# colmap/pycolmap

Measured on AMD Instinct MI355X. Metric: descriptor-pair distances/sec (exhaustive SIFT match: dot + top-2 + ratio + cross-check), higher is better.
Workload: dtype u8 descriptors, int8 MFMA / int32 accumulate; 1 GPU; 500 images x 4096 descriptors, exhaustive match + ratio test + cross-check (BASELINE.json configs[1] at N=1); pairs_total=124750, pairs_per_rank=124750, kernel=auto, matches_rank0=1865611

## Files before the change

include/amc.h:

```cpp
#ifndef AMC_H_
#define AMC_H_

#include <stddef.h>
#include <stdint.h>

#ifdef __cplusplus
extern "C" {
#endif

#define AMC_ABI_VERSION 5
#define AMC_DESC_DIM 128

enum {
    AMC_OK = 0,
    AMC_E_INVALID = -1,
    AMC_E_HIP = -2,
    AMC_E_NOMEM = -3,
    AMC_E_STATE = -4
};

enum { AMC_KERNEL_AUTO = 0, AMC_KERNEL_MFMA = 1, AMC_KERNEL_DOT4 = 2 };

typedef struct amc_ctx amc_ctx;

typedef struct amc_match_opts {
    double max_ratio;
    double max_distance;
    int32_t cross_check;
    int32_t kernel;
} amc_match_opts;

typedef struct amc_match_result {
    size_t npairs;
    uint64_t* offsets;
    uint32_t* matches;
    uint64_t num_distances;
    uint64_t pairs_mfma;
    uint64_t pairs_dot4;
    uint64_t pairs_guided_grid;
    double device_ms;
    double match_kernel_ms;
    double cross_kernel_ms;
    uint32_t match_kernel_launches;
    void* _priv;
} amc_match_result;

const char* amc_last_error(void);
int amc_abi_version(void);

int amc_device_count(void);

int amc_ctx_create(int device_id, amc_ctx** out);
void amc_ctx_destroy(amc_ctx* ctx);

int amc_ctx_set_stream(amc_ctx* ctx, void* hip_stream);

int amc_ctx_trim(amc_ctx* ctx);

int amc_ctx_resident_matches(amc_ctx* ctx, const uint32_t** dev_matches, uint64_t* num_matches);

int amc_upload_matches(amc_ctx* ctx, const uint32_t* matches, uint64_t num_matches);

#define AMC_COMM_ID_BYTES 128
typedef struct amc_comm amc_comm;
int amc_comm_unique_id(void* id);
int amc_comm_create(amc_ctx* ctx, int world_size, int rank, const void* id, amc_comm** out);
void amc_comm_destroy(amc_comm* comm);

typedef struct amc_gathered_tables {
    size_t npairs;
    const uint64_t* offsets;
    const uint32_t* matches;
    const uint32_t* matches_device;
    uint64_t num_matches;
    uint64_t rows_sent, rows_received;
    int32_t world_size, rank;
    double sizes_ms, meta_ms, rows_ms, reorder_ms, download_ms, total_ms;
    void* _priv;
} amc_gathered_tables;

int amc_allgather_match_tables(amc_ctx* ctx, amc_comm* comm, const uint64_t* pair_index, size_t npairs_local,
                               const uint64_t* offsets, const uint32_t* matches, int download,
                               amc_gathered_tables* out);
void amc_gathered_tables_free(amc_gathered_tables* t);

typedef struct amc_gathered_records {
    size_t npairs;
    size_t record_bytes;
    const void* records;
    const void* records_device;
    uint64_t bytes_sent, bytes_received;
    int32_t world_size, rank;
    double total_ms;
    void* _priv;
} amc_gathered_records;
int amc_allgather_pair_records(amc_ctx* ctx, amc_comm* comm, const uint64_t* pair_index, size_t npairs_local,
                               const void* records, size_t record_bytes, int download, amc_gathered_records* out);
void amc_gathered_records_free(amc_gathered_records* r);
int amc_allgather_inlier_tables(amc_ctx* ctx, amc_comm* comm, const uint64_t* pair_index, size_t npairs_local,
                                int download, amc_gathered_tables* out);

int amc_ctx_reserve_slots(amc_ctx* ctx, uint32_t num_slots);
int amc_ctx_grow_slots(amc_ctx* ctx, uint32_t num_slots);

int amc_upload_descriptors(amc_ctx* ctx, uint32_t slot, const uint8_t* host_desc, uint32_t rows);

int amc_upload_descriptors_device(amc_ctx* ctx, uint32_t slot, const void* dev_desc,
                                  uint32_t rows);

int amc_match_pairs(amc_ctx* ctx, const uint32_t* slot1, const uint32_t* slot2, size_t npairs,
                    const amc_match_opts* opts, amc_match_result* out);
void amc_match_result_free(amc_match_result* r);

void amc_match_opts_default(amc_match_opts* opts);

int amc_get_acos_lut(amc_ctx* ctx, float* out);


typedef struct amc_ransac_opts {
    double max_error;
    double min_inlier_ratio;
    double confidence;
    double dyn_num_trials_multiplier;
    int64_t min_num_trials;
    int64_t max_num_trials;
} amc_ransac_opts;

typedef struct amc_tvg_opts {
    int32_t min_num_inliers;
    int32_t detect_watermark;
    int32_t multiple_ignore_watermark;
    int32_t force_H_use;
    int32_t compute_relative_pose;
    int32_t multiple_models;
    double min_E_F_inlier_ratio;
    double max_H_inlier_ratio;
    double watermark_min_inlier_ratio;
    double watermark_border_size;
    amc_ransac_opts ransac;
} amc_tvg_opts;

enum {
    AMC_TVG_UNDEFINED = 0, AMC_TVG_DEGENERATE = 1, AMC_TVG_CALIBRATED = 2, AMC_TVG_UNCALIBRATED = 3,
    AMC_TVG_PLANAR = 4, AMC_TVG_PANORAMIC = 5, AMC_TVG_PLANAR_OR_PANORAMIC = 6, AMC_TVG_WATERMARK = 7,
    AMC_TVG_MULTIPLE = 8
};

enum {
    AMC_CAM_SIMPLE_PINHOLE = 0,
    AMC_CAM_PINHOLE = 1,
    AMC_CAM_SIMPLE_RADIAL = 2,
    AMC_CAM_RADIAL = 3,
    AMC_CAM_OPENCV = 4,
    AMC_CAM_OPENCV_FISHEYE = 5,
    AMC_CAM_FULL_OPENCV = 6,
    AMC_CAM_FOV = 7,
    AMC_CAM_SIMPLE_RADIAL_FISHEYE = 8,
    AMC_CAM_RADIAL_FISHEYE = 9,
    AMC_CAM_THIN_PRISM_FISHEYE = 10
};

typedef struct amc_tvg {
    int32_t config;
    int32_t num_inliers;
    double E[9], F[9], H[9];
    int64_t num_trials[4];
    int64_t model_inliers[3];
} amc_tvg;

typedef struct amc_pose {
    int32_t ok;
    int32_t config;
    double qvec[4];
    double tvec[3];
    double R[9];
    double tri_angle;
    uint32_t num_points3D;
    uint32_t pad_;
} amc_pose;

typedef struct amc_verify_result {
    size_t npairs;
    amc_tvg* tvg;
    uint8_t* inlier_mask;
    double device_ms;
    double kernel_ms;
    uint32_t kernel_launches;
    amc_pose* pose;
    double pose_kernel_ms;
    uint64_t work[12];
    void* _priv;
} amc_verify_result;

void amc_tvg_opts_default(amc_tvg_opts* opts);

int amc_upload_keypoints(amc_ctx* ctx, uint32_t slot, const float* xy, uint32_t rows,
                         uint32_t stride_floats);

int amc_upload_points_f64(amc_ctx* ctx, uint32_t slot, const double* xy, uint32_t rows);

int amc_upload_camera(amc_ctx* ctx, uint32_t slot, int32_t model_id, uint64_t width,
                      uint64_t height, const double* params, int32_t num_params,
                      int32_t has_prior_focal_length);

int amc_cam_from_img(amc_ctx* ctx, int32_t model_id, const double* params, int32_t num_params,
                     const double* xy, size_t n, double* uv);
int amc_img_from_cam(amc_ctx* ctx, int32_t model_id, const double* params, int32_t num_params,
                     const double* uv, size_t n, double* xy);

int amc_verify_pairs(amc_ctx* ctx, const uint32_t* slot1, const uint32_t* slot2, size_t npairs,
                     const uint64_t* match_offsets, const uint32_t* matches,
                     const amc_tvg_opts* opts, uint32_t seed, amc_verify_result* out);
void amc_verify_result_free(amc_verify_result* r);

int amc_match_verify_pairs(amc_ctx* ctx, const uint32_t* slot1, const uint32_t* slot2, size_t npairs,
                           const amc_match_opts* match_opts, const amc_tvg_opts* tvg_opts, uint32_t seed,
                           amc_match_result* match_out, amc_verify_result* verify_out);

int amc_ctx_last_timeline(amc_ctx* ctx, double out_ms[8]);

int amc_pose_pairs(amc_ctx* ctx, const uint32_t* slot1, const uint32_t* slot2, size_t npairs,
                   const uint64_t* match_offsets, const uint32_t* inlier_matches, const amc_tvg* geoms,
                   amc_pose* out);

int amc_match_guided_pairs(amc_ctx* ctx, const uint32_t* slot1, const uint32_t* slot2, size_t npairs,
                           const amc_tvg* geoms, double max_error, const amc_match_opts* opts,
                           amc_match_result* out);

enum { AMC_RANSAC_F = 0, AMC_RANSAC_H = 1, AMC_RANSAC_E = 2 };
typedef struct amc_ransac_report {
    int32_t success;
    int32_t num_inliers;
    int64_t num_trials;
    double model[9];
} amc_ransac_report;
typedef struct amc_ransac_result {
    size_t npairs;
    amc_ransac_report* reports;
    uint8_t* inlier_mask;
    double device_ms;
    void* _priv;
} amc_ransac_result;
int amc_ransac_pairs(amc_ctx* ctx, int kind, const uint32_t* slot1, const uint32_t* slot2, size_t npairs,
                     const uint64_t* match_offsets, const uint32_t* matches,
                     const amc_ransac_opts* opts, uint32_t seed, amc_ransac_result* out);
void amc_ransac_result_free(amc_ransac_result* r);

int amc_squared_sampson_error(amc_ctx* ctx, const double* points1, const double* points2, size_t n,
                              const double E[9], double* out);

int amc_homography_decomposition(amc_ctx* ctx, const double H[9], const double K1[9], const double K2[9],
                                 const double* points1, const double* points2, size_t n, double R[9], double t[3],
                                 double normal[3], double* points3D, uint64_t* num_points3D);

#ifdef __cplusplus
}
#endif
#endif
```

pycolmap_amd/_capi.py:

```python
from __future__ import annotations

import ctypes as C
from pathlib import Path

import numpy as np

_PKG = Path(__file__).resolve().parent
LIB_PATH = _PKG / "libamc.so"

AMC_OK = 0
AMC_E_INVALID, AMC_E_HIP, AMC_E_NOMEM, AMC_E_STATE = -1, -2, -3, -4
KERNEL_AUTO, KERNEL_MFMA, KERNEL_DOT4 = 0, 1, 2
KERNELS = {"auto": KERNEL_AUTO, "mfma": KERNEL_MFMA, "dot4": KERNEL_DOT4}

EXPORTED_SYMBOLS = [
    "amc_last_error", "amc_abi_version", "amc_device_count", "amc_ctx_create", "amc_ctx_destroy",
    "amc_ctx_set_stream", "amc_ctx_reserve_slots", "amc_upload_descriptors",
    "amc_upload_descriptors_device", "amc_match_pairs", "amc_match_result_free",
    "amc_match_opts_default", "amc_get_acos_lut",
    "amc_tvg_opts_default", "amc_upload_keypoints", "amc_upload_camera", "amc_verify_pairs",
    "amc_verify_result_free", "amc_upload_points_f64", "amc_ransac_pairs", "amc_ransac_result_free",
    "amc_squared_sampson_error", "amc_match_guided_pairs", "amc_ctx_grow_slots", "amc_pose_pairs",
    "amc_cam_from_img", "amc_match_verify_pairs", "amc_ctx_trim", "amc_ctx_resident_matches",
    "amc_homography_decomposition", "amc_img_from_cam",
    "amc_comm_unique_id", "amc_comm_create", "amc_comm_destroy", "amc_allgather_match_tables", "amc_gathered_tables_free",
    "amc_allgather_pair_records", "amc_gathered_records_free", "amc_allgather_inlier_tables", "amc_ctx_last_timeline",
    "amc_upload_matches",
    "amc_estimate_rig_absolute_poses", "amc_rigpose_result_free",
    "amc_undistort_opts_default", "amc_undistort_camera", "amc_undistort_points", "amc_undistort_images",
    "amc_ba_opts_default", "amc_bundle_adjust", "amc_bundle_adjust_masked",
    "amc_bacov_opts_default", "amc_ba_covariance", "amc_bacov_result_free",
    "amc_filter_opts_default", "amc_filter_points3d", "amc_filter_result_free",
    "amc_triobs_opts_default", "amc_triangulate_observations", "amc_triobs_result_free",
    "amc_complete_opts_default", "amc_complete_tracks", "amc_complete_result_free",
    "amc_merge_opts_default", "amc_merge_tracks", "amc_merge_result_free",
    "amc_retri_opts_default", "amc_retriangulate_pairs", "amc_retri_result_free",
    "amc_image_visibility", "amc_visibility_result_free",
    "amc_pair_angle_opts_default", "amc_shared_point_angles", "amc_pair_angle_result_free",
    "amc_pair_tri_opts_default", "amc_triangulate_pairs", "amc_pair_tri_result_free",
    "amc_patch_match_opts_default", "amc_patch_match", "amc_patch_match_result_free",
    "amc_fusion_opts_default", "amc_fuse_depth_maps", "amc_fusion_result_free",
]
COMM_ID_BYTES = 128
RANSAC_F, RANSAC_H, RANSAC_E = 0, 1, 2
RANSAC_KINDS = {"F": RANSAC_F, "H": RANSAC_H, "E": RANSAC_E}


class _MatchLease:

    def __init__(self, lib, res):
        self._lib, self._res = lib, res

    def __del__(self):
        try:
            self._lib.amc_match_result_free(C.byref(self._res))
        except Exception:
            pass


class _VerifyLease:

    def __init__(self, lib, res):
        self._lib, self._res = lib, res

    def __del__(self):
        try:
            self._lib.amc_verify_result_free(C.byref(self._res))
        except Exception:
            pass


class _LeasedArray(np.ndarray):

    @staticmethod
    def wrap(arr, lease):
        out = arr.view(_LeasedArray)
        out._lease = lease
        return out

    def __array_finalize__(self, obj):
        self._lease = getattr(obj, "_lease", None)


class AmcError(RuntimeError):
    def __init__(self, code: int, msg: str):
        super().__init__(f"amc error {code}: {msg}")
        self.code = code


class GatheredTables(C.Structure):
    _fields_ = [("npairs", C.c_size_t), ("offsets", C.POINTER(C.c_uint64)), ("matches", C.POINTER(C.c_uint32)),
                ("matches_device", C.c_void_p), ("num_matches", C.c_uint64), ("rows_sent", C.c_uint64),
                ("rows_received", C.c_uint64), ("world_size", C.c_int32), ("rank", C.c_int32),
                ("sizes_ms", C.c_double), ("meta_ms", C.c_double), ("rows_ms", C.c_double), ("reorder_ms", C.c_double),
                ("download_ms", C.c_double), ("total_ms", C.c_double), ("_priv", C.c_void_p)]


class GatheredRecords(C.Structure):
    _fields_ = [("npairs", C.c_size_t), ("record_bytes", C.c_size_t), ("records", C.c_void_p), ("records_device", C.c_void_p),
                ("bytes_sent", C.c_uint64), ("bytes_received", C.c_uint64), ("world_size", C.c_int32), ("rank", C.c_int32),
                ("total_ms", C.c_double), ("_priv", C.c_void_p)]


class MatchOpts(C.Structure):
    _fields_ = [("max_ratio", C.c_double), ("max_distance", C.c_double),
                ("cross_check", C.c_int32), ("kernel", C.c_int32)]


class MatchResult(C.Structure):
    _fields_ = [("npairs", C.c_size_t), ("offsets", C.POINTER(C.c_uint64)),
                ("matches", C.POINTER(C.c_uint32)), ("num_distances", C.c_uint64),
                ("pairs_mfma", C.c_uint64), ("pairs_dot4", C.c_uint64), ("pairs_guided_grid", C.c_uint64),
                ("device_ms", C.c_double), ("match_kernel_ms", C.c_double),
                ("cross_kernel_ms", C.c_double),
                ("match_kernel_launches", C.c_uint32), ("_priv", C.c_void_p)]


class SiftOpts(C.Structure):
    _fields_ = [("first_octave", C.c_int32), ("num_octaves", C.c_int32), ("octave_resolution", C.c_int32),
                ("peak_threshold", C.c_double), ("edge_threshold", C.c_double), ("max_num_orientations", C.c_int32),
                ("upright", C.c_int32), ("normalization", C.c_int32), ("max_num_features", C.c_int32),
                ("max_image_size", C.c_int32)]


class SiftImage(C.Structure):
    _fields_ = [("pixels", C.c_void_p), ("width", C.c_int32), ("height", C.c_int32), ("pitch", C.c_int64)]


class SiftResult(C.Structure):
    _fields_ = [("nimages", C.c_size_t), ("offsets", C.POINTER(C.c_uint64)), ("keypoints", C.POINTER(C.c_float)),
                ("descriptors", C.POINTER(C.c_uint8)), ("device_ms", C.c_double), ("stage_ms", C.c_double * 4),
                ("_priv", C.c_void_p)]


class AbsPoseOpts(C.Structure):
    _fields_ = [("estimate_focal_length", C.c_int32), ("num_focal_length_samples", C.c_int32),
                ("min_focal_length_ratio", C.c_double), ("max_focal_length_ratio", C.c_double),
                ("max_error", C.c_double), ("min_inlier_ratio", C.c_double), ("confidence", C.c_double),
                ("dyn_num_trials_multiplier", C.c_double), ("min_num_trials", C.c_int64),
                ("max_num_trials", C.c_int64)]


class AbsPoseRefineOpts(C.Structure):
    _fields_ = [("gradient_tolerance", C.c_double), ("max_num_iterations", C.c_int64),
                ("loss_function_scale", C.c_double), ("refine_focal_length", C.c_int32),
                ("refine_extra_params", C.c_int32), ("print_summary", C.c_int32)]


class AbsPoseResult(C.Structure):
    _fields_ = [("nqueries", C.c_size_t), ("ncorr", C.c_size_t), ("success", C.POINTER(C.c_uint8)),
                ("qvec", C.POINTER(C.c_double)), ("tvec", C.POINTER(C.c_double)),
                ("num_inliers", C.POINTER(C.c_uint32)), ("num_trials", C.POINTER(C.c_uint64)),
                ("focal_factor", C.POINTER(C.c_double)), ("covariance", C.POINTER(C.c_double)),
                ("inlier_mask", C.POINTER(C.c_uint8)), ("device_ms", C.c_double), ("kernel_ms", C.c_double),
                ("num_batches", C.c_uint32), ("_priv", C.c_void_p)]


def abspose_options(estimation=None, refinement=None):
    eo, ro = AbsPoseOpts(), AbsPoseRefineOpts()
    for k, v in dict(estimate_focal_length=0, num_focal_length_samples=30, min_focal_length_ratio=0.1,
                     max_focal_length_ratio=10.0, max_error=12.0, min_inlier_ratio=0.01, confidence=0.9999,
                     dyn_num_trials_multiplier=3.0, min_num_trials=1000, max_num_trials=100000).items():
        setattr(eo, k, v)
    for k, v in dict(gradient_tolerance=1.0, max_num_iterations=100, loss_function_scale=1.0, refine_focal_length=0,
                     refine_extra_params=0, print_summary=0).items():
        setattr(ro, k, v)
    for o, given in ((eo, estimation or {}), (ro, refinement or {})):
        for k, v in given.items():
            if k not in dict(type(o)._fields_):
                raise ValueError(f"unknown absolute pose option {k!r}")
            setattr(o, k, type(getattr(o, k))(v))
    return eo, ro


def abspose_inputs(offsets, camera_models, camera_params, points2D, points3D):
    off = np.ascontiguousarray(offsets, dtype=np.uint64).reshape(-1)
    if off.size < 1:
        raise ValueError("absolute poses: offsets needs nqueries + 1 entries")
    nq, n = off.size - 1, int(off[-1])
    models = np.ascontiguousarray(camera_models, dtype=np.int32).reshape(-1)
    if models.size != nq or len(camera_params) != nq:
        raise ValueError(f"absolute poses: {nq} queries by offsets, {models.size} camera models, "
                         f"{len(camera_params)} parameter sets")
    prm = np.zeros((nq, 12), np.float64)
    for i, p in enumerate(camera_params):
        p = np.asarray(p, dtype=np.float64).reshape(-1)
        if p.size > 12:
            raise ValueError(f"absolute poses: camera {i} has {p.size} parameters (at most 12)")
        prm[i, :p.size] = p
    p2 = np.ascontiguousarray(points2D, dtype=np.float64).reshape(-1, 2)
    p3 = np.ascontiguousarray(points3D, dtype=np.float64).reshape(-1, 3)
    if p2.shape[0] != n or p3.shape[0] != n:
        raise ValueError(f"absolute poses: {n} correspondences by offsets, {p2.shape[0]} points2D, "
                         f"{p3.shape[0]} points3D")
    return off, models, prm, p2, p3


class BaOpts(C.Structure):
    _fields_ = [("loss_function_type", C.c_int32), ("max_num_iterations", C.c_int32),
                ("max_linear_solver_iterations", C.c_int32), ("max_num_consecutive_invalid_steps", C.c_int32),
                ("loss_function_scale", C.c_double), ("function_tolerance", C.c_double),
                ("gradient_tolerance", C.c_double), ("parameter_tolerance", C.c_double)]


class BaProblem(C.Structure):
    _fields_ = [("num_cameras", C.c_size_t), ("camera_models", C.c_void_p), ("camera_params", C.c_void_p),
                ("camera_const", C.c_void_p), ("num_images", C.c_size_t), ("image_cameras", C.c_void_p),
                ("qvec", C.c_void_p), ("tvec", C.c_void_p), ("pose_const", C.c_void_p), ("num_points", C.c_size_t),
                ("xyz", C.c_void_p), ("num_observations", C.c_size_t), ("obs_image", C.c_void_p),
                ("obs_point", C.c_void_p), ("obs_xy", C.c_void_p)]


class BaResult(C.Structure):
    _fields_ = [("num_images", C.c_uint64), ("num_points", C.c_uint64), ("num_observations", C.c_uint64),
                ("num_variable_parameters", C.c_uint64), ("initial_cost", C.c_double), ("final_cost", C.c_double),
                ("num_successful_steps", C.c_uint32), ("num_unsuccessful_steps", C.c_uint32),
                ("num_pcg_iterations", C.c_uint32), ("num_pcg_stops_residual", C.c_uint32),
                ("num_pcg_stops_cap", C.c_uint32), ("termination", C.c_int32), ("host_ms", C.c_double),
                ("device_ms", C.c_double), ("kernel_ms", C.c_double)]


BA_LOSSES = {"TRIVIAL": 0, "SOFT_L1": 1, "CAUCHY": 2}
BA_TERMINATIONS = ("FUNCTION_TOLERANCE", "PARAMETER_TOLERANCE", "GRADIENT_TOLERANCE", "MAX_ITERATIONS", "MIN_RADIUS",
                   "INVALID_STEPS", "NOTHING_TO_REFINE")
BA_PCG_TOLERANCE = 1e-8


def ba_options(options=None) -> "BaOpts":
    o = BaOpts()
    for k, v in dict(loss_function_type=0, max_num_iterations=100, max_linear_solver_iterations=200,
                     max_num_consecutive_invalid_steps=10, loss_function_scale=1.0, function_tolerance=0.0,
                     gradient_tolerance=0.0, parameter_tolerance=0.0).items():
        setattr(o, k, v)
    for k, v in (options or {}).items():
        if k not in dict(BaOpts._fields_):
            raise ValueError(f"unknown bundle adjustment option {k!r}")
        if k == "loss_function_type" and isinstance(v, str):
            if v.upper() not in BA_LOSSES:
                raise ValueError(f"unknown loss function type {v!r}")
            v = BA_LOSSES[v.upper()]
        setattr(o, k, type(getattr(o, k))(v))
    return o


def ba_inputs(camera_models, camera_params, camera_const, image_cameras, qvec, tvec, pose_const, xyz, obs_image,
              obs_point, obs_xy):
    models = np.array(camera_models, dtype=np.int32).reshape(-1)
    nc = models.size
    if len(camera_params) != nc:
        raise ValueError(f"bundle adjustment: {nc} camera models, {len(camera_params)} parameter sets")
    prm = np.zeros((nc, 12), np.float64)
    for i, p in enumerate(camera_params):
        p = np.asarray(p, dtype=np.float64).reshape(-1)
        if p.size > 12:
            raise ValueError(f"bundle adjustment: camera {i} has {p.size} parameters (at most 12)")
        prm[i, :p.size] = p
    cc = np.ones((nc, 12), np.uint8)
    for i, m in enumerate(camera_const):
        m = np.asarray(m).reshape(-1)
        cc[i, :min(m.size, 12)] = m[:12] != 0
    icam = np.array(image_cameras, dtype=np.int64).reshape(-1)
    ni = icam.size
    q = np.array(qvec, dtype=np.float64).reshape(-1, 4)
    t = np.array(tvec, dtype=np.float64).reshape(-1, 3)
    pc = (np.array(pose_const).reshape(-1, 6) != 0).astype(np.uint8)
    X = np.array(xyz, dtype=np.float64).reshape(-1, 3)
    oi = np.array(obs_image, dtype=np.int64).reshape(-1)
    op = np.array(obs_point, dtype=np.int64).reshape(-1)
    xy = np.array(obs_xy, dtype=np.float64).reshape(-1, 2)
    if q.shape[0] != ni or t.shape[0] != ni or pc.shape[0] != ni or op.size != oi.size or xy.shape[0] != oi.size:
        raise ValueError(f"bundle adjustment: {ni} images by image_cameras, {q.shape[0]} rotations, {t.shape[0]} "
                         f"translations, {pc.shape[0]} pose masks; {oi.size} observations by obs_image, {op.size} "
                         f"point indices, {xy.shape[0]} pixels")
    for name, a in (("image_cameras", icam), ("obs_image", oi), ("obs_point", op)):
        if a.size and (a.min() < 0 or a.max() > 0xffffffff):
            raise ValueError(f"bundle adjustment: {name} has an index outside 0 .. 2^32 - 1")
    return (models, prm, cc, icam.astype(np.uint32), q, t, pc, X, oi.astype(np.uint32), op.astype(np.uint32), xy)


class BacovOpts(C.Structure):
    _fields_ = [("loss_function_type", C.c_int32), ("want_points", C.c_int32), ("want_matrix", C.c_int32),
                ("reserved", C.c_int32), ("loss_function_scale", C.c_double), ("damping", C.c_double)]


class BacovResult(C.Structure):
    _fields_ = [("success", C.c_int32), ("reserved", C.c_int32), ("failed_column", C.c_int64),
                ("num_columns", C.c_uint64), ("num_points", C.c_uint64), ("min_pivot_ratio", C.c_double),
                ("column_owner", C.POINTER(C.c_uint32)), ("column_coord", C.POINTER(C.c_uint32)),
                ("matrix", C.POINTER(C.c_double)), ("point_present", C.POINTER(C.c_uint8)),
                ("point_cov", C.POINTER(C.c_double)), ("host_ms", C.c_double), ("device_ms", C.c_double),
                ("kernel_ms", C.c_double), ("copy_ms", C.c_double), ("phase_ms", C.c_double * 5)]


BACOV_MAX_COLUMNS = 8192
BACOV_PHASES = ("evaluation", "formation", "factor", "inverse", "points")


def bacov_options(options=None) -> "BacovOpts":
    o = BacovOpts(0, 1, 1, 0, 1.0, 1e-8)
    for k, v in (options or {}).items():
        if k not in dict(BacovOpts._fields_) or k == "reserved":
            raise ValueError(f"ba_covariance: unknown option {k!r}")
        if k == "loss_function_type" and isinstance(v, str):
            if v.upper() not in BA_LOSSES:
                raise ValueError(f"ba_covariance: unknown loss function type {v!r}")
            v = BA_LOSSES[v.upper()]
        setattr(o, k, type(getattr(o, k))(v))
    if not 0 <= o.loss_function_type <= 2:
        raise ValueError(f"ba_covariance: loss_function_type {o.loss_function_type} outside 0 .. 2")
    if not (o.loss_function_scale > 0 and np.isfinite(o.loss_function_scale)):
        raise ValueError(f"ba_covariance: loss_function_scale {o.loss_function_scale} is not positive and finite")
    if not (o.damping >= 0 and np.isfinite(o.damping)):
        raise ValueError(f"ba_covariance: damping {o.damping} is not non-negative and finite")
    return o


def bacov_inputs(camera_models, camera_params, camera_const, image_cameras, qvec, tvec, pose_const, xyz, obs_image,
                 obs_point, obs_xy, point_const=None):
    try:
        arrays = ba_inputs(camera_models, camera_params, camera_const, image_cameras, qvec, tvec, pose_const, xyz,
                           obs_image, obs_point, obs_xy)
    except ValueError as e:
        raise ValueError(f"ba_covariance: {e}") from None
    mask = None
    if point_const is not None:
        mask = np.ascontiguousarray(np.asarray(point_const).reshape(-1) != 0, dtype=np.uint8)
        if mask.size != arrays[7].shape[0]:
            raise ValueError(f"ba_covariance: {arrays[7].shape[0]} points, {mask.size} point_const flags")
    return arrays + (mask,)


class FilterOpts(C.Structure):
    _fields_ = [("max_reproj_error", C.c_double), ("min_tri_angle", C.c_double), ("errors_only", C.c_int32),
                ("reserved", C.c_int32)]


class FilterProblem(C.Structure):
    _fields_ = [("num_cameras", C.c_size_t), ("camera_models", C.c_void_p), ("camera_params", C.c_void_p),
                ("num_images", C.c_size_t), ("image_cameras", C.c_void_p), ("qvec", C.c_void_p), ("tvec", C.c_void_p),
                ("num_points", C.c_size_t), ("xyz", C.c_void_p), ("track_offsets", C.c_void_p),
                ("obs_image", C.c_void_p), ("obs_xy", C.c_void_p), ("selected", C.c_void_p)]


class FilterResult(C.Structure):
    _fields_ = [("num_points", C.c_uint64), ("num_observations", C.c_uint64), ("num_filtered", C.c_uint64),
                ("obs_sq_error", C.POINTER(C.c_double)), ("obs_deleted", C.POINTER(C.c_uint8)),
                ("point_verdict", C.POINTER(C.c_uint8)), ("point_error", C.POINTER(C.c_double)),
                ("num_batches", C.c_uint32), ("reserved", C.c_uint32), ("host_ms", C.c_double),
                ("device_ms", C.c_double), ("kernel_ms", C.c_double), ("copy_ms", C.c_double),
                ("alloc_ms", C.c_double)]


FILTER_VERDICTS = ("KEPT", "NOT_SELECTED", "SHORT_TRACK", "REPROJECTION", "ANGLE")


def filter_inputs(camera_models, camera_params, image_cameras, qvec, tvec, xyz, track_offsets, obs_image, obs_xy,
                  selected=None):
    models = np.array(camera_models, dtype=np.int32).reshape(-1)
    if len(camera_params) != models.size:
        raise ValueError(f"filter_points3d: {models.size} camera models, {len(camera_params)} parameter sets")
    prm = np.zeros((models.size, 12), np.float64)
    for i, p in enumerate(camera_params):
        p = np.asarray(p, dtype=np.float64).reshape(-1)
        if p.size > 12:
            raise ValueError(f"filter_points3d: camera {i} has {p.size} parameters (at most 12)")
        prm[i, :p.size] = p
    icam = np.array(image_cameras, dtype=np.int64).reshape(-1)
    q = np.array(qvec, dtype=np.float64).reshape(-1, 4)
    t = np.array(tvec, dtype=np.float64).reshape(-1, 3)
    X = np.array(xyz, dtype=np.float64).reshape(-1, 3)
    off = np.array(track_offsets, dtype=np.int64).reshape(-1)
    oi = np.array(obs_image, dtype=np.int64).reshape(-1)
    xy = np.array(obs_xy, dtype=np.float64).reshape(-1, 2)
    if q.shape[0] != icam.size or t.shape[0] != icam.size or off.size != X.shape[0] + 1 or xy.shape[0] != oi.size:
        raise ValueError(f"filter_points3d: {icam.size} images by image_cameras, {q.shape[0]} rotations, {t.shape[0]} "
                         f"translations; {X.shape[0]} points, {off.size} offsets; {oi.size} observations by obs_image, "
                         f"{xy.shape[0]} pixels")
    if off.min() < 0 or int(off[-1]) != oi.size:
        raise ValueError(f"filter_points3d: track_offsets ends at {int(off[-1])}, {oi.size} observations")
    for name, a in (("image_cameras", icam), ("obs_image", oi)):
        if a.size and (a.min() < 0 or a.max() > 0xffffffff):
            raise ValueError(f"filter_points3d: {name} has an index outside 0 .. 2^32 - 1")
    sel = None
    if selected is not None:
        sel = np.ascontiguousarray(np.asarray(selected).reshape(-1) != 0, dtype=np.uint8)
        if sel.size != X.shape[0]:
            raise ValueError(f"filter_points3d: {X.shape[0]} points, {sel.size} selection flags")
    return models, prm, icam.astype(np.uint32), q, t, X, off.astype(np.uint64), oi.astype(np.uint32), xy, sel


class TriobsOpts(C.Structure):
    _fields_ = [("create_max_angle_error", C.c_double), ("continue_max_angle_error", C.c_double),
                ("min_angle", C.c_double), ("reserved", C.c_double)]


class TriobsProblem(C.Structure):
    _fields_ = [("num_cameras", C.c_size_t), ("camera_models", C.c_void_p), ("camera_params", C.c_void_p),
                ("num_images", C.c_size_t), ("image_cameras", C.c_void_p), ("qvec", C.c_void_p), ("tvec", C.c_void_p),
                ("num_items", C.c_size_t), ("item_offsets", C.c_void_p), ("cand_image", C.c_void_p),
                ("cand_xy", C.c_void_p), ("cand_has_point", C.c_void_p), ("cand_xyz", C.c_void_p),
                ("no_create_two_view", C.c_void_p)]


class TriobsResult(C.Structure):
    _fields_ = [("num_items", C.c_uint64), ("num_candidates", C.c_uint64), ("num_created", C.c_uint64),
                ("num_continued", C.c_uint64), ("continued", C.POINTER(C.c_int32)),
                ("cand_round", C.POINTER(C.c_uint32)), ("round_offsets", C.POINTER(C.c_uint64)),
                ("round_xyz", C.POINTER(C.c_double)), ("num_batches", C.c_uint32), ("reserved", C.c_uint32),
                ("host_ms", C.c_double), ("device_ms", C.c_double), ("kernel_ms", C.c_double), ("copy_ms", C.c_double),
                ("alloc_ms", C.c_double)]


def triobs_inputs(camera_models, camera_params, image_cameras, qvec, tvec, item_offsets, cand_image, cand_xy,
                  cand_has_point, cand_xyz, no_create_two_view=None):
    who = "triangulate_observations"
    models = np.array(camera_models, dtype=np.int32).reshape(-1)
    if len(camera_params) != models.size:
        raise ValueError(f"{who}: {models.size} camera models, {len(camera_params)} parameter sets")
# ... 1375 lines not shown
        ptr = lambda a: a.ctypes.data_as(C.c_void_p)
        pb = TriobsProblem(models.size, ptr(models), ptr(prm), icam.size, ptr(icam), ptr(q), ptr(t), off.size - 1,
                           ptr(off), ptr(ci), ptr(xy), ptr(has), ptr(X), None if two is None else ptr(two))
        res = TriobsResult()
        _check(self._lib.amc_triangulate_observations(self._h, C.byref(pb), C.byref(o), C.byref(res)))
        try:
            nit, n, nr = off.size - 1, ci.size, int(res.num_created)
            a = lambda p, k: np.ctypeslib.as_array(p, (max(k, 1),))[:k].copy()
            out = {"continued": a(res.continued, nit), "cand_round": a(res.cand_round, n),
                   "round_offsets": a(res.round_offsets, nit + 1), "round_xyz": a(res.round_xyz, 3 * nr).reshape(nr, 3),
                   "num_created": nr, "num_continued": int(res.num_continued), "num_batches": int(res.num_batches),
                   "host_ms": res.host_ms, "device_ms": res.device_ms, "kernel_ms": res.kernel_ms,
                   "copy_ms": res.copy_ms, "alloc_ms": res.alloc_ms}
        finally:
            self._lib.amc_triobs_result_free(C.byref(res))
        return out

    def complete_tracks(self, camera_models, camera_params, image_cameras, qvec, tvec, item_xyz, item_offsets, cand_image,
                        cand_xy, complete_max_reproj_error=4.0):
        models, prm, icam, q, t, X, off, ci, xy = complete_inputs(camera_models, camera_params, image_cameras, qvec, tvec,
                                                                  item_xyz, item_offsets, cand_image, cand_xy)
        o = CompleteOpts(float(complete_max_reproj_error), 0.0)
        ptr = lambda a: a.ctypes.data_as(C.c_void_p)
        pb = CompleteProblem(models.size, ptr(models), ptr(prm), icam.size, ptr(icam), ptr(q), ptr(t), off.size - 1,
                             ptr(X), ptr(off), ptr(ci), ptr(xy))
        res = CompleteResult()
        _check(self._lib.amc_complete_tracks(self._h, C.byref(pb), C.byref(o), C.byref(res)))
        try:
            n = ci.size
            a = lambda p, k: np.ctypeslib.as_array(p, (max(k, 1),))[:k].copy()
            out = {"cand_sq_error": a(res.cand_sq_error, n), "cand_pass": a(res.cand_pass, n).astype(bool),
                   "num_passed": int(res.num_passed), "num_batches": int(res.num_batches), "host_ms": res.host_ms,
                   "device_ms": res.device_ms, "kernel_ms": res.kernel_ms, "copy_ms": res.copy_ms,
                   "alloc_ms": res.alloc_ms}
        finally:
            self._lib.amc_complete_result_free(C.byref(res))
        return out

    def merge_tracks(self, camera_models, camera_params, image_cameras, qvec, tvec, comp_point_offsets, comp_root_offsets,
                     roots, point_xyz, point_obs_offsets, obs_image, obs_xy, obs_corr_offsets, corr_obs,
                     merge_max_reproj_error=4.0):
        a = merge_inputs(camera_models, camera_params, image_cameras, qvec, tvec, comp_point_offsets, comp_root_offsets,
                         roots, point_xyz, point_obs_offsets, obs_image, obs_xy, obs_corr_offsets, corr_obs)
        models, prm, icam, q, t, cpo, cro, rt, X, poo, oi, xy, oco, co = a
        o = MergeOpts(float(merge_max_reproj_error), 0.0)
        ptr = lambda v: v.ctypes.data_as(C.c_void_p)
        pb = MergeProblem(models.size, ptr(models), ptr(prm), icam.size, ptr(icam), ptr(q), ptr(t), cpo.size - 1, ptr(cpo),
                          ptr(cro), ptr(rt), ptr(X), ptr(poo), ptr(oi), ptr(xy), ptr(oco), ptr(co))
        res = MergeResult()
        _check(self._lib.amc_merge_tracks(self._h, C.byref(pb), C.byref(o), C.byref(res)))
        try:
            nr, nm = rt.size, int(res.num_merges)
            arr = lambda p, k: np.ctypeslib.as_array(p, (max(k, 1),))[:k].copy()
            out = {"root_return": arr(res.root_return, nr), "root_merge_offsets": arr(res.root_merge_offsets, nr + 1),
                   "merge_current": arr(res.merge_current, nm), "merge_other": arr(res.merge_other, nm),
                   "merge_xyz": arr(res.merge_xyz, 3 * nm).reshape(nm, 3), "num_merges": nm,
                   "num_pairs_tried": int(res.num_pairs_tried), "num_batches": int(res.num_batches),
                   "host_ms": res.host_ms, "device_ms": res.device_ms, "kernel_ms": res.kernel_ms,
                   "copy_ms": res.copy_ms, "alloc_ms": res.alloc_ms}
        finally:
            self._lib.amc_merge_result_free(C.byref(res))
        return out

    def retriangulate_pairs(self, camera_models, camera_params, image_cameras, qvec, tvec, obs_image, obs_xy, obs_point,
                            point_xyz, pair_images, pair_offsets, corr_obs, round_offsets, corr_two_view=None,
                            create_max_angle_error=2.0, re_max_angle_error=5.0, min_angle=1.5, re_min_ratio=0.2):
        a = retri_inputs(camera_models, camera_params, image_cameras, qvec, tvec, obs_image, obs_xy, obs_point, point_xyz,
                         pair_images, pair_offsets, corr_obs, round_offsets, corr_two_view)
        models, prm, icam, q, t, oi, xy, op, X, pi, poff, co, roff, two = a
        o = RetriOpts(float(create_max_angle_error), float(re_max_angle_error), float(min_angle), float(re_min_ratio))
        ptr = lambda v: v.ctypes.data_as(C.c_void_p)
        pb = RetriProblem(models.size, ptr(models), ptr(prm), icam.size, ptr(icam), ptr(q), ptr(t), oi.size, ptr(oi),
                          ptr(xy), ptr(op), X.shape[0], ptr(X), pi.shape[0], ptr(pi), ptr(poff), ptr(co),
                          None if two is None else ptr(two), roff.size - 1, ptr(roff))
        res = RetriResult()
        _check(self._lib.amc_retriangulate_pairs(self._h, C.byref(pb), C.byref(o), C.byref(res)))
        try:
            npairs, nc, made = pi.shape[0], co.shape[0], int(res.num_created)
            arr = lambda p, k: np.ctypeslib.as_array(p, (max(k, 1),))[:k].copy()
            out = {"pair_ran": arr(res.pair_ran, npairs).astype(bool), "pair_num_tri": arr(res.pair_num_tri, npairs),
                   "corr_action": arr(res.corr_action, nc), "created_offsets": arr(res.created_offsets, npairs + 1),
                   "created_xyz": arr(res.created_xyz, 3 * made).reshape(made, 3), "num_pairs_run": int(res.num_pairs_run),
                   "num_continued": int(res.num_continued), "num_created": made, "num_launches": int(res.num_launches),
                   "host_ms": res.host_ms, "device_ms": res.device_ms, "kernel_ms": res.kernel_ms,
                   "copy_ms": res.copy_ms, "alloc_ms": res.alloc_ms}
        finally:
            self._lib.amc_retri_result_free(C.byref(res))
        return out

    def image_visibility(self, image_point_offsets, point2D_point3D, cand_width, cand_height, cand_point_offsets, cand_xy,
                         corr_offsets, corr_image, corr_point2D):
        ipoff, table, cw, ch, cpoff, xy, coff, ci, cp = visibility_inputs(
            image_point_offsets, point2D_point3D, cand_width, cand_height, cand_point_offsets, cand_xy, corr_offsets,
            corr_image, corr_point2D)
        ptr = lambda v: v.ctypes.data_as(C.c_void_p)
        pb = VisibilityProblem(ipoff.size - 1, ptr(ipoff), ptr(table), cw.size, ptr(cw), ptr(ch), ptr(cpoff), ptr(xy),
                               ptr(coff), ptr(ci), ptr(cp))
        res = VisibilityResult()
        _check(self._lib.amc_image_visibility(self._h, C.byref(pb), C.byref(res)))
        try:
            k = cw.size
            arr = lambda p, n: np.ctypeslib.as_array(p, (max(n, 1),))[:n].copy()
            out = {"num_observations": arr(res.num_observations, k), "num_visible_points3D": arr(res.num_visible_points3D, k),
                   "score": arr(res.score, k), "max_score": int(res.max_score), "num_batches": int(res.num_batches),
                   "host_ms": res.host_ms, "device_ms": res.device_ms, "kernel_ms": res.kernel_ms,
                   "copy_ms": res.copy_ms, "alloc_ms": res.alloc_ms}
        finally:
            self._lib.amc_visibility_result_free(C.byref(res))
        return out

    def shared_point_angles(self, qvec, tvec, point_xyz, pair_images, pair_offsets, shared_points, percentile=75.0):
        q, t, X, pi, poff, sp = pair_angle_inputs(qvec, tvec, point_xyz, pair_images, pair_offsets, shared_points)
        ptr = lambda v: v.ctypes.data_as(C.c_void_p)
        o = PairAngleOpts(float(percentile))
        pb = PairAngleProblem(q.shape[0], ptr(q), ptr(t), X.shape[0], ptr(X), pi.shape[0], ptr(pi), ptr(poff), ptr(sp))
        res = PairAngleResult()
        _check(self._lib.amc_shared_point_angles(self._h, C.byref(pb), C.byref(o), C.byref(res)))
        try:
            k = pi.shape[0]
            out = {"angle": np.ctypeslib.as_array(res.angle, (max(k, 1),))[:k].copy(), "num_batches": int(res.num_batches),
                   "host_ms": res.host_ms, "device_ms": res.device_ms, "kernel_ms": res.kernel_ms,
                   "copy_ms": res.copy_ms, "alloc_ms": res.alloc_ms}
        finally:
            self._lib.amc_pair_angle_result_free(C.byref(res))
        return out

    def triangulate_pairs(self, camera_models, camera_params, image_cameras, qvec, tvec, pair_images, pair_offsets, corr_xy1,
                          corr_xy2, min_tri_angle=INITPAIR_DEFAULT_MIN_TRI_ANGLE):
        models, prm, icam, q, t, pi, poff, xy1, xy2 = pair_tri_inputs(camera_models, camera_params, image_cameras, qvec, tvec,
                                                                      pair_images, pair_offsets, corr_xy1, corr_xy2)
        ptr = lambda v: v.ctypes.data_as(C.c_void_p)
        o = PairTriOpts(float(min_tri_angle), 0.0)
        pb = PairTriProblem(models.size, ptr(models), ptr(prm), icam.size, ptr(icam), ptr(q), ptr(t), pi.shape[0], ptr(pi),
                            ptr(poff), ptr(xy1), ptr(xy2))
        res = PairTriResult()
        _check(self._lib.amc_triangulate_pairs(self._h, C.byref(pb), C.byref(o), C.byref(res)))
        try:
            n = xy1.shape[0]
            arr = lambda p, k: np.ctypeslib.as_array(p, (max(k, 1),))[:k].copy()
            out = {"accepted": arr(res.accepted, n).astype(bool), "xyz": arr(res.xyz, 3 * n).reshape(n, 3),
                   "tri_angle": arr(res.tri_angle, n), "num_accepted": int(res.num_accepted),
                   "num_batches": int(res.num_batches), "host_ms": res.host_ms, "device_ms": res.device_ms,
                   "kernel_ms": res.kernel_ms, "copy_ms": res.copy_ms, "alloc_ms": res.alloc_ms}
        finally:
            self._lib.amc_pair_tri_result_free(C.byref(res))
        return out

    def patch_match(self, images, K, R, t, ref_images, src_offsets, src_images, depth_ranges, in_depth=None, in_normal=None,
                    **options):
        o = patch_match_options(**options)
        pb, keep = patch_match_inputs(images, K, R, t, ref_images, src_offsets, src_images, depth_ranges, in_depth, in_normal)
        res = PatchMatchResult()
        _check(self._lib.amc_patch_match(self._h, C.byref(o), C.byref(pb), C.byref(res)))
        try:
            out = patch_match_unpack(keep, res.num_problems, res.map_offsets, res.cost_offsets, res.depth, res.normal,
                                     res.num_consistent, res.costs if o.want_costs else None)
            out.update({"num_batches": int(res.num_batches), "num_launches": int(res.num_launches), "host_ms": res.host_ms,
                        "device_ms": res.device_ms, "kernel_ms": res.kernel_ms, "copy_ms": res.copy_ms,
                        "alloc_ms": res.alloc_ms})
        finally:
            self._lib.amc_patch_match_result_free(C.byref(res))
        return out

    def fuse_depth_maps(self, images, K, R, t, depth_maps, normal_maps, neighbours, **options):
        o = fusion_options(**options)
        pb, keep = fusion_inputs(images, K, R, t, depth_maps, normal_maps, neighbours)
        res = FusionResult()
        _check(self._lib.amc_fuse_depth_maps(self._h, C.byref(o), C.byref(pb), C.byref(res)))
        try:
            out = fusion_unpack(res.num_points, res.xyz, res.normal, res.color, res.seed_image, res.seed_pixel,
                                res.num_fused, res.vis_offsets, res.vis_images)
            out.update({"num_seeds": int(res.num_seeds), "num_truncated": int(res.num_truncated),
                        "num_batches": int(res.num_batches), "num_launches": int(res.num_launches), "host_ms": res.host_ms,
                        "device_ms": res.device_ms, "kernel_ms": res.kernel_ms, "copy_ms": res.copy_ms,
                        "alloc_ms": res.alloc_ms})
        finally:
            self._lib.amc_fusion_result_free(C.byref(res))
        return out

    def estimate_rig_absolute_poses(self, offsets, camera_offsets, camera_models, camera_params, cams_from_rig,
                                    camera_idxs, points2D, points3D, estimation=None, refinement=None,
                                    return_covariance=False):
        off, coff, models, prm, rigs, idx, p2, p3 = rigpose_inputs(offsets, camera_offsets, camera_models,
                                                                   camera_params, cams_from_rig, camera_idxs,
                                                                   points2D, points3D)
        eo, ro = rigpose_options(estimation, refinement)
        nq, n = off.size - 1, int(off[-1])
        res = RigPoseResult()
        ptr = lambda a: a.ctypes.data_as(C.c_void_p)
        _check(self._lib.amc_estimate_rig_absolute_poses(self._h, ptr(off), nq, ptr(coff), ptr(models), ptr(prm),
                                                          ptr(rigs), ptr(idx), ptr(p2), ptr(p3), C.byref(eo),
                                                          C.byref(ro), int(bool(return_covariance)), C.byref(res)))
        try:
            a = lambda p, shape: np.ctypeslib.as_array(p, (max(shape[0], 1),) + shape[1:])[:shape[0]].copy()
            out = {"success": a(res.success, (nq,)).astype(bool), "qvec": a(res.qvec, (nq, 4)),
                   "tvec": a(res.tvec, (nq, 3)), "num_inliers": a(res.num_inliers, (nq,)),
                   "num_all_inliers": a(res.num_all_inliers, (nq,)), "num_trials": a(res.num_trials, (nq,)),
                   "inlier_mask": a(res.inlier_mask, (n,)).astype(bool), "device_ms": res.device_ms,
                   "kernel_ms": res.kernel_ms, "num_batches": int(res.num_batches)}
            if return_covariance:
                out["covariance"] = a(res.covariance, (nq, 36)).reshape(nq, 6, 6)
        finally:
            self._lib.amc_rigpose_result_free(C.byref(res))
        return out

    def triangulate_tracks(self, poses, track_offsets, obs_pose, obs_xy, **opts):
        P = np.ascontiguousarray(poses, dtype=np.float64).reshape(-1, 12)
        off = np.ascontiguousarray(track_offsets, dtype=np.uint64).reshape(-1)
        if off.size < 1:
            raise ValueError("triangulate_tracks: track_offsets needs ntracks + 1 entries")
        nobs = int(off[-1])
        op = np.ascontiguousarray(obs_pose, dtype=np.uint32).reshape(-1)
        xy = np.ascontiguousarray(obs_xy, dtype=np.float64).reshape(-1, 2)
        if op.size != nobs or xy.shape[0] != nobs:
            raise ValueError(f"triangulate_tracks: {nobs} observations by track_offsets, {op.size} pose indices, "
                             f"{xy.shape[0]} points")
        o = TriOpts()
        self._lib.amc_tri_opts_default(C.byref(o))
        for k, v in opts.items():
            if k not in dict(TriOpts._fields_):
                raise ValueError(f"triangulate_tracks: unknown option {k!r}")
            setattr(o, k, type(getattr(o, k))(v))
        nt = off.size - 1
        res = TriResult()
        _check(self._lib.amc_triangulate_tracks(self._h, P.ctypes.data_as(C.c_void_p), P.shape[0],
                                                 off.ctypes.data_as(C.c_void_p), nt, op.ctypes.data_as(C.c_void_p),
                                                 xy.ctypes.data_as(C.c_void_p), C.byref(o), C.byref(res)))
        try:
            xyz = np.ctypeslib.as_array(res.xyz, (max(nt, 1), 3))[:nt].copy()
            ok = np.ctypeslib.as_array(res.success, (max(nt, 1),))[:nt].astype(bool)
            mask = np.ctypeslib.as_array(res.inlier_mask, (max(nobs, 1),))[:nobs].astype(bool)
            stats = {"num_inliers": np.ctypeslib.as_array(res.num_inliers, (max(nt, 1),))[:nt].copy(),
                     "num_trials": np.ctypeslib.as_array(res.num_trials, (max(nt, 1),))[:nt].copy(),
                     "device_ms": res.device_ms, "kernel_ms": res.kernel_ms, "num_batches": int(res.num_batches)}
        finally:
            self._lib.amc_tri_result_free(C.byref(res))
        return xyz, ok, mask, stats

    def undistort_images(self, images, src_cameras, dst_cameras):
        n = len(images)
        if len(src_cameras) != n or len(dst_cameras) != n:
            raise ValueError(f"undistort_images: {n} images, {len(src_cameras)} source and {len(dst_cameras)} target cameras")
        arr = (UndistortImage * max(n, 1))()
        keep, outs = [], []
        for i, im in enumerate(images):
            ok = (isinstance(im, np.ndarray) and im.dtype == np.uint8 and im.ndim in (2, 3) and im.size > 0
                  and (im.ndim == 2 or im.shape[2] in (1, 3)))
            if not ok:
                raise ValueError(f"undistort_images: image {i} must be a non-empty H x W or H x W x 3 uint8 array")
            ch = 1 if im.ndim == 2 else im.shape[2]
            packed = im.strides[-1] == 1 and (im.ndim == 2 or im.strides[1] == ch) and im.strides[0] >= im.shape[1] * ch
            a = im if packed else np.ascontiguousarray(im)
            keep.append(a)
            dc = _undistort_cam(dst_cameras[i])
            out = np.empty((int(dc.height), int(dc.width)) + ((ch,) if im.ndim == 3 else ()), dtype=np.uint8)
            outs.append(out)
            arr[i] = UndistortImage(a.ctypes.data, a.strides[0], ch, 0, _undistort_cam(src_cameras[i]), dc,
                                    out.ctypes.data if out.size else None)
        res = UndistortResult()
        _check(self._lib.amc_undistort_images(self._h, n, C.cast(arr, C.c_void_p), C.byref(res)))
        return outs, {"device_ms": res.device_ms, "kernel_ms": res.kernel_ms, "num_batches": int(res.num_batches),
                      "num_resized": int(res.num_resized)}

    def match_pairs(self, slot1, slot2, max_ratio: float = 0.8, max_distance: float = 0.7,
                    cross_check: bool = True, kernel: str = "auto", copy: bool = True):
        s1 = np.ascontiguousarray(slot1, dtype=np.uint32)
        s2 = np.ascontiguousarray(slot2, dtype=np.uint32)
        if s1.shape != s2.shape or s1.ndim != 1:
            raise ValueError("slot1/slot2 must be equal-length 1-D arrays")
        opts = MatchOpts(max_ratio, max_distance, 1 if cross_check else 0, KERNELS[kernel])
        res = MatchResult()
        self.resident_generation += 1
        _check(self._lib.amc_match_pairs(self._h, s1.ctypes.data_as(C.c_void_p),
                                         s2.ctypes.data_as(C.c_void_p), s1.size, C.byref(opts),
                                         C.byref(res)))
        if not copy:
            return self._unpack_match(res, _MatchLease(self._lib, res))
        try:
            offsets, matches, stats = self._unpack_match(res)
        finally:
            self._lib.amc_match_result_free(C.byref(res))
        return offsets, matches, stats

    @staticmethod
    def _unpack_match(res, lease=None):
        n = int(res.npairs)

        def view(ptr, count, dtype):
            nbytes = count * np.dtype(dtype).itemsize
            return np.frombuffer((C.c_char * nbytes).from_address(C.addressof(ptr.contents)), dtype=dtype)

        offsets = view(res.offsets, n + 1, np.uint64)
        total = int(offsets[-1])
        offsets = offsets.copy() if lease is None else _LeasedArray.wrap(offsets, lease)
        if total:
            matches = view(res.matches, 2 * total, np.uint32).reshape(total, 2)
            matches = matches.copy() if lease is None else _LeasedArray.wrap(matches, lease)
        else:
            matches = np.zeros((0, 2), dtype=np.uint32)
        stats = dict(num_distances=int(res.num_distances), pairs_mfma=int(res.pairs_mfma),
                     pairs_dot4=int(res.pairs_dot4), device_ms=float(res.device_ms),
                     match_kernel_ms=float(res.match_kernel_ms),
                     cross_kernel_ms=float(res.cross_kernel_ms),
                     match_kernel_launches=int(res.match_kernel_launches))
        return offsets, matches, stats

    @staticmethod
    def _unpack_verify(res, total, labelled=False, lease=None):
        n = int(res.npairs)
        assert C.sizeof(Tvg) == TVG_DTYPE.itemsize

        def take(ptr, count, dtype):
            nbytes = count * np.dtype(dtype).itemsize
            if not nbytes:
                return np.zeros(0, dtype=dtype)
            addr = C.cast(ptr, C.c_void_p).value
            a = np.frombuffer((C.c_char * nbytes).from_address(addr), dtype=dtype)
            return a.copy() if lease is None else _LeasedArray.wrap(a, lease)

        tvg = take(res.tvg, n, TVG_DTYPE)
        labels = take(res.inlier_mask, total, np.uint8)
        mask = labels.astype(bool) if labelled else labels.view(np.bool_)
        stats = dict(device_ms=float(res.device_ms), kernel_ms=float(res.kernel_ms), inlier_labels=labels,
                     kernel_launches=int(res.kernel_launches), work=[int(x) for x in res.work])
        stats["pose_kernel_ms"] = float(res.pose_kernel_ms)
        if res.pose:
            assert C.sizeof(Pose) == POSE_DTYPE.itemsize
            stats["pose"] = take(res.pose, n, POSE_DTYPE)
        return tvg, mask, stats

    def match_verify_pairs(self, slot1, slot2, opts: TvgOpts | None = None, seed: int = 0, max_ratio: float = 0.8,
                           max_distance: float = 0.7, cross_check: bool = True, kernel: str = "auto", copy: bool = True):
        s1 = np.ascontiguousarray(slot1, dtype=np.uint32)
        s2 = np.ascontiguousarray(slot2, dtype=np.uint32)
        if s1.shape != s2.shape or s1.ndim != 1:
            raise ValueError("slot1/slot2 must be equal-length 1-D arrays")
        mo = MatchOpts(max_ratio, max_distance, 1 if cross_check else 0, KERNELS[kernel])
        o = opts or tvg_options()
        mres, vres = MatchResult(), VerifyResult()
        self.resident_generation += 1
        _check(self._lib.amc_match_verify_pairs(self._h, s1.ctypes.data_as(C.c_void_p), s2.ctypes.data_as(C.c_void_p),
                                                s1.size, C.byref(mo), C.byref(o), seed, C.byref(mres), C.byref(vres)))
        if not copy:
            offsets, matches, mstats = self._unpack_match(mres, _MatchLease(self._lib, mres))
            tvg, mask, vstats = self._unpack_verify(vres, matches.shape[0], bool(o.multiple_models),
                                                    _VerifyLease(self._lib, vres))
            return offsets, matches, mstats, tvg, mask, vstats
        try:
            offsets, matches, mstats = self._unpack_match(mres)
            tvg, mask, vstats = self._unpack_verify(vres, matches.shape[0], bool(o.multiple_models))
        finally:
            self._lib.amc_match_result_free(C.byref(mres))
            self._lib.amc_verify_result_free(C.byref(vres))
        return offsets, matches, mstats, tvg, mask, vstats

    def match_guided_pairs(self, slot1, slot2, tvg, max_error: float, max_ratio: float = 0.8,
                           max_distance: float = 0.7, cross_check: bool = True):
        s1 = np.ascontiguousarray(slot1, dtype=np.uint32)
        s2 = np.ascontiguousarray(slot2, dtype=np.uint32)
        g = np.ascontiguousarray(tvg, dtype=TVG_DTYPE)
        if s1.shape != s2.shape or s1.ndim != 1 or g.shape != s1.shape:
            raise ValueError("slot1/slot2/tvg must be equal-length 1-D arrays")
        assert C.sizeof(Tvg) == TVG_DTYPE.itemsize
        opts = MatchOpts(max_ratio, max_distance, 1 if cross_check else 0, KERNEL_AUTO)
        res = MatchResult()
        self.resident_generation += 1
        _check(self._lib.amc_match_guided_pairs(self._h, s1.ctypes.data_as(C.c_void_p),
                                                s2.ctypes.data_as(C.c_void_p), s1.size,
                                                g.ctypes.data_as(C.c_void_p), float(max_error), C.byref(opts),
                                                C.byref(res)))
        try:
            n = int(res.npairs)
            offsets = np.ctypeslib.as_array(res.offsets, shape=(n + 1,)).copy()
            total = int(offsets[-1])
            matches = (np.ctypeslib.as_array(res.matches, shape=(total, 2)).copy() if total
                       else np.zeros((0, 2), dtype=np.uint32))
            stats = dict(num_distances=int(res.num_distances), pairs_dot4=int(res.pairs_dot4),
                         pairs_guided_grid=int(res.pairs_guided_grid),
                         device_ms=float(res.device_ms))
        finally:
            self._lib.amc_match_result_free(C.byref(res))
        return offsets, matches, stats

    def upload_keypoints(self, slot: int, kp: np.ndarray) -> None:
        k = np.ascontiguousarray(kp, dtype=np.float32)
        if k.size and (k.ndim != 2 or k.shape[1] < 2):
            raise ValueError(f"keypoints must be N x (>=2) float32, got {k.shape}")
        rows = k.shape[0] if k.ndim == 2 else 0
        stride = k.shape[1] if k.ndim == 2 and rows else 2
        _check(self._lib.amc_upload_keypoints(self._h, slot, k.ctypes.data_as(C.c_void_p), rows, stride))

    def upload_points_f64(self, slot: int, pts: np.ndarray) -> None:
        k = np.ascontiguousarray(pts, dtype=np.float64)
        if k.size and (k.ndim != 2 or k.shape[1] != 2):
            raise ValueError(f"points must be N x 2 float64, got {k.shape}")
        rows = k.shape[0] if k.ndim == 2 else 0
        _check(self._lib.amc_upload_points_f64(self._h, slot, k.ctypes.data_as(C.c_void_p), rows))

    def ransac_pairs(self, kind, slot1, slot2, match_offsets, matches, ransac: dict | RansacOpts | None = None,
                     seed: int = 0):
        s1 = np.ascontiguousarray(slot1, dtype=np.uint32)
        s2 = np.ascontiguousarray(slot2, dtype=np.uint32)
        off = np.ascontiguousarray(match_offsets, dtype=np.uint64)
        m = np.ascontiguousarray(matches, dtype=np.uint32).reshape(-1, 2)
        if off.shape != (s1.size + 1,) or s1.shape != s2.shape:
            raise ValueError("match_offsets must have npairs + 1 entries")
        if int(off[-1]) != m.shape[0]:
            raise ValueError("match_offsets[-1] must equal the number of matches")
        if isinstance(ransac, RansacOpts):
            ro = ransac
        else:
            ro = tvg_options(ransac=ransac or {}).ransac
        k = RANSAC_KINDS[kind] if isinstance(kind, str) else int(kind)
        res = RansacResult()
        _check(self._lib.amc_ransac_pairs(self._h, k, s1.ctypes.data_as(C.c_void_p), s2.ctypes.data_as(C.c_void_p),
                                          s1.size, off.ctypes.data_as(C.c_void_p), m.ctypes.data_as(C.c_void_p),
                                          C.byref(ro), seed, C.byref(res)))
        try:
            n = int(res.npairs)
            assert C.sizeof(RansacReport) == RANSAC_DTYPE.itemsize
            rep = (np.frombuffer(C.string_at(res.reports, n * C.sizeof(RansacReport)), dtype=RANSAC_DTYPE).copy()
                   if n else np.zeros(0, dtype=RANSAC_DTYPE))
            total = m.shape[0]
            mask = (np.ctypeslib.as_array(res.inlier_mask, shape=(total,)).astype(bool) if total
                    else np.zeros(0, dtype=bool))
        finally:
            self._lib.amc_ransac_result_free(C.byref(res))
        return rep, mask

    def squared_sampson_error(self, points1, points2, E) -> np.ndarray:
        p1 = np.ascontiguousarray(points1, dtype=np.float64).reshape(-1, 2)
        p2 = np.ascontiguousarray(points2, dtype=np.float64).reshape(-1, 2)
        if p1.shape != p2.shape:
            raise ValueError("points1 and points2 must have the same shape")
        e = np.ascontiguousarray(E, dtype=np.float64).reshape(9)
        out = np.empty(p1.shape[0], dtype=np.float64)
        _check(self._lib.amc_squared_sampson_error(self._h, p1.ctypes.data_as(C.c_void_p),
                                                   p2.ctypes.data_as(C.c_void_p), p1.shape[0],
                                                   e.ctypes.data_as(C.c_void_p), out.ctypes.data_as(C.c_void_p)))
        return out

    def homography_decomposition(self, H, K1, K2, points1, points2) -> dict:
        p1 = np.ascontiguousarray(points1, dtype=np.float64).reshape(-1, 2)
        p2 = np.ascontiguousarray(points2, dtype=np.float64).reshape(-1, 2)
        if p1.shape != p2.shape:
            raise ValueError("points1 and points2 must have the same shape")
        mats = [np.ascontiguousarray(a, dtype=np.float64).reshape(9) for a in (H, K1, K2)]
        R, t, n = np.empty(9), np.empty(3), np.empty(3)
        X = np.empty((max(1, len(p1)), 3))
        m = C.c_uint64(0)
        v = lambda a: a.ctypes.data_as(C.c_void_p)
        _check(self._lib.amc_homography_decomposition(self._h, v(mats[0]), v(mats[1]), v(mats[2]), v(p1), v(p2), len(p1),
                                                      v(R), v(t), v(n), v(X), C.cast(C.byref(m), C.c_void_p)))
        return dict(R=R.reshape(3, 3), t=t, n=n, points3D=X[:m.value].copy())

    def cam_from_img(self, model: str | int, params, points) -> np.ndarray:
        p = np.ascontiguousarray(params, dtype=np.float64)
        xy = np.ascontiguousarray(points, dtype=np.float64).reshape(-1, 2)
        mid = CAMERA_MODELS[model] if isinstance(model, str) else int(model)
        out = np.empty_like(xy)
        _check(self._lib.amc_cam_from_img(self._h, mid, p.ctypes.data_as(C.c_void_p), p.size,
                                          xy.ctypes.data_as(C.c_void_p), xy.shape[0], out.ctypes.data_as(C.c_void_p)))
        return out

    def img_from_cam(self, model: str | int, params, points) -> np.ndarray:
        p = np.ascontiguousarray(params, dtype=np.float64)
        uv = np.ascontiguousarray(points, dtype=np.float64).reshape(-1, 2)
        mid = CAMERA_MODELS[model] if isinstance(model, str) else int(model)
        out = np.empty_like(uv)
        _check(self._lib.amc_img_from_cam(self._h, mid, p.ctypes.data_as(C.c_void_p), p.size, uv.ctypes.data_as(C.c_void_p),
                                          uv.shape[0], out.ctypes.data_as(C.c_void_p)))
        return out

    def upload_camera(self, slot: int, model: str | int, width: int, height: int, params,
                      has_prior_focal_length: bool = False) -> None:
        p = np.ascontiguousarray(params, dtype=np.float64)
        mid = CAMERA_MODELS[model] if isinstance(model, str) else int(model)
        _check(self._lib.amc_upload_camera(self._h, slot, mid, width, height,
                                           p.ctypes.data_as(C.c_void_p), p.size,
                                           int(has_prior_focal_length)))

    def verify_pairs(self, slot1, slot2, match_offsets, matches, opts: TvgOpts | None = None, seed: int = 0,
                     copy: bool = True):
        s1 = np.ascontiguousarray(slot1, dtype=np.uint32)
        s2 = np.ascontiguousarray(slot2, dtype=np.uint32)
        off = np.ascontiguousarray(match_offsets, dtype=np.uint64)
        if off.shape != (s1.size + 1,) or s1.shape != s2.shape:
            raise ValueError("match_offsets must have npairs + 1 entries")
        if matches is None:
            m, nrows = None, int(off[-1]) if off.size else 0
        else:
            m = np.ascontiguousarray(matches, dtype=np.uint32).reshape(-1, 2)
            nrows = m.shape[0]
            if int(off[-1]) != nrows:
                raise ValueError("match_offsets[-1] must equal the number of matches")
        o = opts if opts is not None else tvg_options()
        res = VerifyResult()
        _check(self._lib.amc_verify_pairs(self._h, s1.ctypes.data_as(C.c_void_p), s2.ctypes.data_as(C.c_void_p),
                                          s1.size, off.ctypes.data_as(C.c_void_p),
                                          m.ctypes.data_as(C.c_void_p) if m is not None else None,
                                          C.byref(o), seed, C.byref(res)))
        if not copy:
            return self._unpack_verify(res, nrows, bool(o.multiple_models), _VerifyLease(self._lib, res))
        try:
            tvg, mask, stats = self._unpack_verify(res, nrows, bool(o.multiple_models))
        finally:
            self._lib.amc_verify_result_free(C.byref(res))
        return tvg, mask, stats

    def pose_pairs(self, slot1, slot2, match_offsets, inlier_matches, config, E=None, H=None) -> np.ndarray:
        s1 = np.ascontiguousarray(slot1, dtype=np.uint32)
        s2 = np.ascontiguousarray(slot2, dtype=np.uint32)
        off = np.ascontiguousarray(match_offsets, dtype=np.uint64)
        m = np.ascontiguousarray(inlier_matches, dtype=np.uint32).reshape(-1, 2)
        if off.shape != (s1.size + 1,) or s1.shape != s2.shape:
            raise ValueError("match_offsets must have npairs + 1 entries")
        if int(off[-1]) != m.shape[0]:
            raise ValueError("match_offsets[-1] must equal the number of matches")
        n = s1.size
        geoms = np.zeros(n, dtype=TVG_DTYPE)
        geoms["config"] = np.asarray(config, dtype=np.int32).reshape(n)
        if E is not None:
            geoms["E"] = np.asarray(E, dtype=np.float64).reshape(n, 3, 3)
        if H is not None:
            geoms["H"] = np.asarray(H, dtype=np.float64).reshape(n, 3, 3)
        out = np.zeros(n, dtype=POSE_DTYPE)
        assert C.sizeof(Pose) == POSE_DTYPE.itemsize and C.sizeof(Tvg) == TVG_DTYPE.itemsize
        _check(self._lib.amc_pose_pairs(self._h, s1.ctypes.data_as(C.c_void_p), s2.ctypes.data_as(C.c_void_p),
                                        C.c_size_t(n), off.ctypes.data_as(C.c_void_p),
                                        m.ctypes.data_as(C.c_void_p), geoms.ctypes.data_as(C.c_void_p),
                                        out.ctypes.data_as(C.c_void_p)))
        return out

    def acos_lut(self) -> np.ndarray:
        out = np.empty(262145, dtype=np.float32)
        _check(self._lib.amc_get_acos_lut(self._h, out.ctypes.data_as(C.c_void_p)))
        return out
```

pycolmap_amd/csrc/amc_ctx.h:

```cpp
#pragma once

#include <functional>
#include <map>
#include <memory>
#include <mutex>
#include <vector>

#include "amc_internal.h"
#include "slot_arena.h"
#include "scan_accept.h"

namespace amc {

inline uint32_t round_up(uint32_t x, uint32_t m) { return (x + m - 1) / m * m; }

struct Slot {
    void* base = nullptr;
    ImageDev dev{};
    uint32_t maxsq = 0;
    bool valid = false;
    float* kp = nullptr;
    double* kp64 = nullptr;
    double* kpn = nullptr;
    bool kpn_valid = false;
    uint32_t kp_rows = 0;
    bool has_kp = false, has_cam = false;
    CameraDev cam{};
    void* grid_base = nullptr;
    GridDev grid{};
};

struct HipRaw {
    static int alloc(void** p, size_t bytes) { return (int)hipMalloc(p, bytes); }
    static void free(void* p) { (void)hipFree(p); }
    static void clear_error() { (void)hipGetLastError(); }
};
struct SlotArena : amc::SlotArenaT<HipRaw> {
    template <class T>
    hipError_t alloc(T** out, size_t bytes) {
        return (hipError_t)amc::SlotArenaT<HipRaw>::alloc(out, bytes);
    }
};

struct PinnedPool {
    static constexpr size_t kMaxIdleBytes = (size_t)3 << 29;
    std::mutex mu;
    std::vector<PinBuf<uint32_t>> idle;
    PinBuf<uint32_t> acquire(size_t want = 0) {
        std::lock_guard<std::mutex> lock(mu);
        if (idle.empty()) return PinBuf<uint32_t>();
        auto better = [&](const PinBuf<uint32_t>& a, const PinBuf<uint32_t>& b) {
            const bool fa = a.cap >= want, fb = b.cap >= want;
            if (want && fa != fb) return fa;
            if (want && fa) return a.cap < b.cap;
            return a.cap > b.cap;
        };
        size_t best = 0;
        for (size_t i = 1; i < idle.size(); ++i)
            if (better(idle[i], idle[best])) best = i;
        PinBuf<uint32_t> b = std::move(idle[best]);
        idle.erase(idle.begin() + best);
        return b;
    }
    void give_back(PinBuf<uint32_t> b) {
        if (!b.p) return;
        std::lock_guard<std::mutex> lock(mu);
        idle.push_back(std::move(b));
        auto total = [&] {
            size_t t = 0;
            for (auto& x : idle) t += x.cap * sizeof(uint32_t);
            return t;
        };
        while (!idle.empty() && (idle.size() > 3 || total() > kMaxIdleBytes)) {
            size_t small = 0;
            for (size_t i = 1; i < idle.size(); ++i)
                if (idle[i].cap < idle[small].cap) small = i;
            idle.erase(idle.begin() + small);
        }
    }
    void trim() {
        std::lock_guard<std::mutex> lock(mu);
        idle.clear();
    }
};

struct VerifyClassSlot {
    PinBuf<TvgPair> h_pairs, h_pairs_e;
    DevBuf<TvgPair> pairs, pairs_e;
    DevBuf<double> ws, ws_e;
    DevBuf<uint8_t> maskws;
    void release() { pairs.release(); pairs_e.release(); ws.release(); ws_e.release(); maskws.release(); h_pairs.release(); h_pairs_e.release(); }
};
struct VerifySliceBufs {
    PinBuf<uint32_t> h_tabs;
    DevBuf<uint32_t> tabs;
    DevBuf<uint8_t> outmask, emask;
    VerifyClassSlot cls[4];
    hipEvent_t ev[4] = {nullptr, nullptr, nullptr, nullptr};
    hipEvent_t ev_e_done = nullptr, ev_aux_done = nullptr;
    bool aux_pending = false;
    void release() {
        tabs.release(); outmask.release(); emask.release(); h_tabs.release();
        for (auto& k : cls) k.release();
    }
    ~VerifySliceBufs() {
        for (auto& e : ev)
            if (e) (void)hipEventDestroy(e);
        if (ev_e_done) (void)hipEventDestroy(ev_e_done);
        if (ev_aux_done) (void)hipEventDestroy(ev_aux_done);
    }
};
constexpr size_t kVScalarWords = 128;
constexpr size_t kMaxStreamWords = (size_t)1 << 28;

struct TrialTabKey {
    uint32_t M;
    double confidence, multiplier;
    bool operator<(const TrialTabKey& o) const {
        if (M != o.M) return M < o.M;
        if (confidence != o.confidence) return confidence < o.confidence;
        return multiplier < o.multiplier;
    }
};
constexpr size_t kTrialTabCacheWords = size_t(64) << 20;

}

using namespace amc;

struct amc_ctx {
    int device = 0;
    hipStream_t own_stream = nullptr;
    hipStream_t stream = nullptr;
    hipStream_t copy_stream = nullptr;
    hipEvent_t cev[2] = {nullptr, nullptr};
    hipStream_t aux_stream = nullptr;
    hipEvent_t aev[2] = {nullptr, nullptr};
    std::vector<Slot> slots;
    bool table_dirty = true;
    DevBuf<ImageDev> d_imgs;
    DevBuf<GridDev> d_grids;
    float* d_lut = nullptr;
    std::vector<float> h_lut;
    ScanAccept* d_accept = nullptr;
    ScanAccept h_accept{};
    float accept_ratio = 0.f, accept_distance = 0.f;
    bool accept_valid = false;
    uint32_t* d_scalars = nullptr;
    struct MatchScratch {
        DevBuf<PairDev> d_pairs;
        DevBuf<Dot4Work> d_work;
        DevBuf<uint32_t> d_order, d_order2;
        DevBuf<uint32_t> d_grp, d_grp2, d_seg_base, d_grp_segs, d_grp_item_base;
        DevBuf<SegDesc> d_segs;
        DevBuf<Top2> d_rowbuf, d_colbuf;
        DevBuf<uint32_t> d_accmask;
        DevBuf<GuidedDev> d_guided;
        DevBuf<uint32_t> d_pair_off, d_pair_cnt, d_matches, d_cand_cnt, d_candbuf;
        DevBuf<uint32_t> d_live, d_live_fwd, d_live_all, d_live_rev, d_live_scan;
        void release_all() {
            d_pairs.release(); d_work.release(); d_order.release(); d_order2.release();
            d_grp.release(); d_grp2.release(); d_seg_base.release(); d_grp_segs.release();
            d_grp_item_base.release(); d_segs.release();
            d_rowbuf.release(); d_colbuf.release(); d_accmask.release(); d_guided.release();
            d_pair_off.release(); d_pair_cnt.release(); d_matches.release();
            d_cand_cnt.release(); d_candbuf.release();
            d_live.release(); d_live_fwd.release(); d_live_all.release(); d_live_rev.release();
            d_live_scan.release();
        }
        void release_large() {
            d_rowbuf.release(); d_colbuf.release(); d_accmask.release(); d_matches.release(); d_candbuf.release();
            d_segs.release(); d_seg_base.release();
        }
    };
    MatchScratch ms;
    DevBuf<uint32_t> d_keep;
    DevBuf<uint64_t> d_csr;
    uint64_t resident_matches = 0;
    PinBuf<uint64_t> h_csr[2];
    std::shared_ptr<PinnedPool> result_pool = std::make_shared<PinnedPool>();
    SlotArena arena;
    PinBuf<PairDev> h_pairs[2];
    PinBuf<Dot4Work> h_work[2];
    PinBuf<uint32_t> h_order[2], h_order2[2], h_pair_off[2], h_pair_cnt[2], h_matches[2], h_bscalars[2];
    PinBuf<uint32_t> h_grp[2], h_grp2[2];
    PinBuf<uint32_t> h_scalars;
    hipEvent_t ev[6] = {nullptr, nullptr, nullptr, nullptr, nullptr, nullptr};
    hipEvent_t bev[2][5] = {{nullptr, nullptr, nullptr, nullptr, nullptr},
                            {nullptr, nullptr, nullptr, nullptr, nullptr}};
    DevBuf<TvgImage> d_timgs;
    DevBuf<uint32_t> d_tmatches;
    DevBuf<TvgEState> d_estate;
    std::vector<std::unique_ptr<VerifySliceBufs>> vslices;
    hipStream_t vstream = nullptr;
    hipEvent_t vev_setup = nullptr, vev_matches = nullptr;
    uint32_t* d_vscalars = nullptr;
    std::vector<double> wm_cut_cache;
    double wm_cut_conf = 0.0, wm_cut_mult = 0.0;
    bool wm_cut_on_device = false;
    PinBuf<TvgImage> h_timgs;
    std::vector<TvgImage> timgs_on_device;
    PinBuf<TvgPair> h_tp;
    PinBuf<uint64_t> h_moff;
    DevBuf<uint32_t> d_stream;
    uint32_t stream_seed = 0;
    size_t stream_len = 0;
    DevBuf<double> d_wmcut;
    DevBuf<TvgOut> d_tout;
    DevBuf<amc_tvg> d_tvg_packed;
    DevBuf<uint8_t> d_mask_packed;
    DevBuf<uint64_t> d_moff;
    DevBuf<TvgPair> d_tp_all;
    DevBuf<unsigned long long> d_worksum;
    amc::VerifyResident vres;
    double timeline[8] = {0, 0, 0, 0, 0, 0, 0, 0};
    double last_hook_ms = 0.0;
    std::shared_ptr<PinnedPool> verify_pool = std::make_shared<PinnedPool>();
    PinBuf<TvgOut> h_tout;
    PinBuf<uint8_t> h_tmask;
    std::map<TrialTabKey, std::vector<uint32_t>> trial_tabs;
    size_t trial_tab_words = 0;
    DevBuf<PosePair> d_ppairs;
    DevBuf<uint32_t> d_pmatches;
    DevBuf<double> d_pcos;
    DevBuf<PoseOut> d_pout;
    PinBuf<PosePair> h_ppairs;
    PinBuf<PoseOut> h_pout;
};

namespace amc {

using BatchHook = std::function<int(size_t begin, size_t end, const uint64_t* offsets, const uint64_t* keep_off)>;
int match_impl(amc_ctx* c, const uint32_t* slot1, const uint32_t* slot2, size_t npairs, const amc_match_opts* opts_in,
               const amc_tvg* geoms, double max_error, amc_match_result* out, std::vector<uint64_t>* keep_off = nullptr,
               const BatchHook* batch_hook = nullptr);

int ensure_normalized(amc_ctx* c, uint32_t slot);
void fill_tvg_images(const amc_ctx* c, std::vector<TvgImage>& timgs);

}
```

pycolmap_amd/csrc/amc_internal.h:

```cpp
#pragma once

#include <hip/hip_runtime.h>
#include <stdint.h>

#include <algorithm>
#include <cstdlib>
#include <type_traits>
#include <vector>

#include "../../include/amc.h"
#include "guided_region.h"

namespace amc {

constexpr int kDim = AMC_DESC_DIM;
constexpr int kRowPad = 256;
constexpr int kAcosLutSize = 262145;

__host__ __device__ __forceinline__ constexpr uint32_t arena_swizzle(uint32_t row) {
    return ((row >> 1) & 1u) | (((row >> 5) & 3u) << 1);
}

struct ImageDev {
    const uint8_t* raw;
// ... 12 lines not shown
    float max_residual;
    float m[9];
    int32_t grid_ok;
    double bound[2];
    double minv[9];
};

using guided::kGridDim;
struct GridDev {
    const float* sxy;
    const uint32_t* sidx;
    const uint32_t* cell_start;
    float x0, y0, inv_cw, inv_ch;
    float cw, ch;
    float bx1, by1;
    uint32_t n;
    uint32_t pad_;
};
using guided::grid_cell;
#if defined(__HIPCC__)
__device__ __forceinline__ bool guided_rejects(const GuidedDev& g, float x1, float y1, float x2, float y2) {
    const float* m = g.m;
    if (g.kind == kGuidedF) {
        const float Fx1_0 = m[0] * x1 + m[1] * y1 + m[2] * 1.0f;
        const float Fx1_1 = m[3] * x1 + m[4] * y1 + m[5] * 1.0f;
        const float Fx1_2 = m[6] * x1 + m[7] * y1 + m[8] * 1.0f;
        const float Ftx2_0 = m[0] * x2 + m[3] * y2 + m[6] * 1.0f;
        const float Ftx2_1 = m[1] * x2 + m[4] * y2 + m[7] * 1.0f;
        const float x2tFx1 = x2 * Fx1_0 + y2 * Fx1_1 + 1.0f * Fx1_2;
        return x2tFx1 * x2tFx1 / (Fx1_0 * Fx1_0 + Fx1_1 * Fx1_1 + Ftx2_0 * Ftx2_0 + Ftx2_1 * Ftx2_1) > g.max_residual;
    }
    const float Hp_0 = m[0] * x1 + m[1] * y1 + m[2] * 1.0f;
    const float Hp_1 = m[3] * x1 + m[4] * y1 + m[5] * 1.0f;
    const float Hp_2 = m[6] * x1 + m[7] * y1 + m[8] * 1.0f;
    const float e0 = Hp_0 / Hp_2 - x2;
    const float e1 = Hp_1 / Hp_2 - y2;
    return e0 * e0 + e1 * e1 > g.max_residual;
}
#endif

struct Top2 {
    uint32_t best_v;
    uint32_t best_idx;
    uint32_t second_v;
    uint32_t pad;
};

struct PairDev {
    uint32_t slot1, slot2;
    uint32_t mode;
    uint32_t pad;
    uint64_t row_off;
    uint64_t col_off;
};

struct Dot4Work {
    uint32_t pair;
    uint32_t dir;
    uint32_t rb;
};

struct FinalizeParams {
    float max_ratio;
    float max_distance;
    int cross_check;
    int reserved;
};

int api_fail(int code, const char* fmt, ...) __attribute__((format(printf, 2, 3)));

constexpr const char* hipchk_who = nullptr;
#define HIPCHK(expr)                                                                                                   \
    do {                                                                                                               \
        const hipError_t e_ = (expr);                                                                                  \
        if (e_ != hipSuccess)                                                                                          \
            return ::amc::api_fail(AMC_E_HIP, "%s%s%s:%d: %s -> %s", hipchk_who ? hipchk_who : "",                    \
                                   hipchk_who ? ": " : "", __FILE__, __LINE__, #expr, hipGetErrorString(e_));        \
    } while (0)

inline bool env_flag(const char* name) { return std::getenv(name) != nullptr; }
inline long long env_int(const char* name, long long dflt, long long lo, long long hi) {
    const char* e = std::getenv(name);
    return e ? std::min(hi, std::max(lo, std::atoll(e))) : dflt;
}

template <typename T, bool kPinned>
struct GrowBuf {
    T* p = nullptr;
    size_t cap = 0;

    GrowBuf() = default;
    GrowBuf(GrowBuf&& o) noexcept : p(o.p), cap(o.cap) {
        o.p = nullptr;
        o.cap = 0;
    }
    GrowBuf& operator=(GrowBuf&& o) noexcept {
        if (this != &o) {
            release();
            p = o.p;
            cap = o.cap;
            o.p = nullptr;
            o.cap = 0;
        }
        return *this;
    }
    ~GrowBuf() { release(); }

    hipError_t ensure(size_t n) {
        if (n <= cap) return hipSuccess;
        release();
        const size_t want = std::max(n, std::is_void<T>::value ? (size_t)256 : (size_t)16);
        const size_t bytes = want * sizeof(typename std::conditional<std::is_void<T>::value, char, T>::type);
        void* q = nullptr;
        const hipError_t e = kPinned ? hipHostMalloc(&q, bytes, 0) : hipMalloc(&q, bytes);
        if (e == hipSuccess) {
            p = static_cast<T*>(q);
            cap = want;
        }
        return e;
    }
    void release() {
        if (p) (void)(kPinned ? hipHostFree(p) : hipFree(p));
        p = nullptr;
        cap = 0;
    }
};
template <typename T>
using DevBuf = GrowBuf<T, false>;
template <typename T>
using PinBuf = GrowBuf<T, true>;

inline size_t align256(size_t x) { return (x + 255) & ~(size_t)255; }

class DevParts {
  public:
    template <typename T>
    DevParts& part(T** ptr, size_t n) {
        parts_.push_back({ptr, align256(n * sizeof(T)), [](void* q, char* at) { *static_cast<T**>(q) = reinterpret_cast<T*>(at); }});
        return *this;
    }
    hipError_t carve(DevBuf<void>& buf) const {
        size_t total = 0;
        for (const Part& q : parts_) total += q.bytes;
        const hipError_t e = buf.ensure(total);
        if (e != hipSuccess) return e;
        char* at = static_cast<char*>(buf.p);
        for (const Part& q : parts_) {
            q.set(q.ptr, at);
            at += q.bytes;
        }
        return hipSuccess;
    }

  private:
    struct Part {
        void* ptr;
        size_t bytes;
        void (*set)(void* ptr, char* at);
    };
    std::vector<Part> parts_;
};

inline hipError_t create_events(hipEvent_t* ev, int n, const unsigned* flags = nullptr) {
    for (int i = 0; i < n; ++i) {
        const hipError_t e = hipEventCreateWithFlags(&ev[i], flags ? flags[i] : hipEventDefault);
        if (e != hipSuccess) {
            for (int j = 0; j < i; ++j) (void)hipEventDestroy(ev[j]);
            std::fill(ev, ev + n, nullptr);
            return e;
        }
    }
    return hipSuccess;
}

class StreamTimer {
  public:
    explicit StreamTimer(hipStream_t s) : s_(s), made_(create_events(ab_, 2)) {}
    StreamTimer(const StreamTimer&) = delete;
    StreamTimer& operator=(const StreamTimer&) = delete;
    ~StreamTimer() {
        for (hipEvent_t e : ab_)
            if (e) (void)hipEventDestroy(e);
        for (hipEvent_t e : spans_) (void)hipEventDestroy(e);
    }

    hipError_t start() { return made_ != hipSuccess ? made_ : hipEventRecord(ab_[0], s_); }
    hipError_t stop(double& ms) {
        hipError_t e = hipEventRecord(ab_[1], s_);
        if (e == hipSuccess) e = hipEventSynchronize(ab_[1]);
        return e == hipSuccess ? add_elapsed(ab_[0], ab_[1], ms) : e;
    }
    hipError_t span_begin() {
        hipEvent_t two[2];
        if (const hipError_t e = create_events(two, 2)) return e;
        spans_.insert(spans_.end(), two, two + 2);
        return hipEventRecord(two[0], s_);
    }
    hipError_t span_end() { return hipEventRecord(spans_.back(), s_); }
    hipError_t spans(double& ms) const {
        for (size_t i = 0; i + 1 < spans_.size(); i += 2)
            if (const hipError_t e = add_elapsed(spans_[i], spans_[i + 1], ms)) return e;
        return hipSuccess;
    }

  private:
    static hipError_t add_elapsed(hipEvent_t a, hipEvent_t b, double& ms) {
        float f = 0.f;
        const hipError_t e = hipEventElapsedTime(&f, a, b);
        if (e == hipSuccess) ms += f;
        return e;
    }
    hipStream_t s_;
    hipEvent_t ab_[2] = {nullptr, nullptr};
    hipError_t made_;
    std::vector<hipEvent_t> spans_;
};

struct Batches {
    std::vector<size_t> start{0};
    uint64_t most_items = 0, most_elems = 0;
    size_t count() const { return start.size() - 1; }
};
inline Batches split_batches(const uint64_t* offsets, size_t n, uint64_t max_items, uint64_t max_elems,
                             uint64_t factor = 1) {
    Batches b;
    for (size_t i = 0; i < n;) {
        size_t j = i + 1;
        while (j < n && j - i < max_items && (offsets[j + 1] - offsets[i]) * factor <= max_elems) ++j;
        b.most_items = std::max<uint64_t>(b.most_items, j - i);
        b.most_elems = std::max<uint64_t>(b.most_elems, offsets[j] - offsets[i]);
        b.start.push_back(j);
        i = j;
    }
    return b;
}

struct CtxView {
    int device;
    hipStream_t stream;
    const uint32_t* resident;
    uint64_t resident_rows;
};
CtxView ctx_view(amc_ctx* c);
struct TvgPair;
struct VerifyResident {
    size_t npairs = 0;
    uint64_t total = 0;
    const amc_tvg* tvg = nullptr;
    const uint8_t* mask = nullptr;
    const uint64_t* moff = nullptr;
    const TvgPair* tp = nullptr;
    const uint32_t* matches = nullptr;
};
VerifyResident verify_resident(amc_ctx* c);

hipError_t memset_async(void* p, int value, size_t bytes, hipStream_t s);
hipError_t memcpy_async(void* dst, const void* src, size_t bytes, hipMemcpyKind kind, hipStream_t s);

hipError_t launch_prep(const uint8_t* raw, uint8_t* prep, int32_t* rs128, uint32_t rows_pad,
                 uint32_t* maxsq_out, hipStream_t s);

hipError_t launch_match_dot4(const ImageDev* imgs, const PairDev* pairs, const Dot4Work* work,
                       uint32_t nwork, Top2* rowbuf, Top2* colbuf, const GuidedDev* guided, hipStream_t s);
hipError_t launch_match_guided_grid(const ImageDev* imgs, const GridDev* grids, const PairDev* pairs, const Dot4Work* work,
                              uint32_t nwork, Top2* rowbuf, Top2* colbuf, const GuidedDev* guided, hipStream_t s);

constexpr int kSegRows = 128;
constexpr int kSegsPerItem = 4;
struct alignas(64) SegDesc {
    const uint8_t* xprep;
    const int32_t* xrs;
    Top2* out;
    const uint32_t* list;
    const uint8_t* yprep;
    const int32_t* yrs;
    uint32_t cnt;
    uint32_t accword;
    uint32_t yrows;
    uint32_t pad_;
};
__device__ __forceinline__ bool one_way_accepts(const Top2 t, const float* __restrict__ lut,
                                                float max_ratio, float max_distance) {
    if (t.best_v == 0u) return false;
    const float a_best = lut[min(t.best_v, 262144u)];
    if (a_best > max_distance) return false;
    const float a_second = lut[min(t.second_v, 262144u)];
    if (a_best >= max_ratio * a_second) return false;
    return true;
}

hipError_t launch_build_segments(int mode, const ImageDev* imgs, const PairDev* pairs, const uint32_t* order,
                           const uint32_t* grp_start, uint32_t ngroups, const uint32_t* cand_cnt,
                           const uint32_t* candbuf, Top2* outbuf, uint32_t* seg_base, uint32_t* grp_segs,
                           uint32_t* grp_item_base, SegDesc* segs, uint32_t* nitems_dev, hipStream_t s);
struct ScanAccept;
struct CopyJob {
    const void* src = nullptr;
    void* dst = nullptr;
    unsigned long long n16 = 0;
    uint32_t parts = 0, pad_ = 0;
};
hipError_t launch_match_mfma(int mode, const SegDesc* segs, const uint32_t* nitems_dev, uint32_t max_items,
                       uint32_t* queue_head, uint32_t* accmask, const ScanAccept* accept_dev, hipStream_t s,
                       const CopyJob& job = CopyJob(), uint32_t* copy_head = nullptr);

size_t live_scratch_words(size_t npairs);
hipError_t launch_live_pairs(const ImageDev* imgs, const PairDev* pairs, uint32_t npairs, const uint32_t* accmask,
                             const uint32_t* order, uint32_t norder, uint32_t* live, uint32_t* live_fwd,
                             uint32_t* live_all, uint32_t* nlive, uint32_t* cand_cnt, uint32_t* pair_cnt,
                             uint32_t* pair_off, uint32_t* scratch, hipStream_t s);
hipError_t launch_compact_order(const uint32_t* order, uint32_t norder, uint32_t npairs, const uint32_t* key, uint32_t* list,
                                uint32_t* nlist, uint32_t* scratch, hipStream_t s);

hipError_t launch_resolve_index(int side, const ImageDev* imgs, const PairDev* pairs,
                          Top2* table, uint32_t* accmask, const float* acos_lut, FinalizeParams fp,
                          const uint32_t* cand_cnt, const uint32_t* candbuf, uint32_t* err_count,
                          bool grouped, const uint32_t* order, const uint32_t* nlist, uint32_t max_list, hipStream_t s);
uint32_t resolve_grouped_max_rows();
constexpr uint32_t kSelectMaxCols = 1u << 20;

hipError_t launch_select_candidates(const ImageDev* imgs, const PairDev* pairs, uint32_t npairs, uint32_t max_cols,
                              const Top2* rowbuf, const uint32_t* accmask, const float* acos_lut,
                              FinalizeParams fp, uint32_t* cand_cnt, uint32_t* candbuf, const uint32_t* list,
                              const uint32_t* nlist, hipStream_t s);

hipError_t launch_finalize(const ImageDev* imgs, const PairDev* pairs, uint32_t npairs, const uint32_t* list,
                     const uint32_t* nlist, const Top2* rowbuf, const Top2* colbuf, uint32_t* accmask,
                     const float* acos_lut, FinalizeParams fp, uint32_t* cursor, uint32_t capacity,
                     uint32_t* pair_off, uint32_t* pair_cnt, uint32_t* matches, hipStream_t s);

hipError_t launch_host_copy(void* dst_pinned, const void* src_dev, size_t bytes, hipStream_t s);
hipError_t launch_reorder_matches(const uint32_t* src_off, const uint32_t* cnt, const uint64_t* dst_off, uint32_t npairs,
                            const uint32_t* src, uint32_t* dst, hipStream_t s);

struct CameraDev {
    int32_t model_id;
    int32_t has_prior;
    uint64_t width, height;
    double params[12];
};
struct TvgImage {
    const float* kp;
    const double* kp64;
    const double* kpn;
    uint32_t rows;
    uint32_t pad;
    CameraDev cam;
};
hipError_t launch_undistort(const float* kp, const double* kp64, uint32_t rows, const CameraDev& cam, double* kpn,
                            hipStream_t s);
hipError_t launch_project(const double* uv, uint32_t n, const CameraDev& cam, double* xy, hipStream_t s);
struct TvgPair {
    uint32_t slot1, slot2;
    uint64_t match_off;
    uint64_t mask_off;
    uint32_t M;
    uint32_t tab_off[3];
    uint32_t orig;
};
struct PosePair {
    uint32_t slot1, slot2;
    uint64_t match_off;
    uint64_t mask_off;
    uint64_t ws_off;
    uint32_t M;
    int32_t config;
    double E[9], H[9];
};
struct alignas(128) PoseOut {
    int32_t ok;
    int32_t t_is_zero;
    uint32_t num_points3D;
    uint32_t pad;
    double R[9], t[3], q[4], cmed[2];
};
hipError_t launch_pose(const TvgImage* imgs, const PosePair* pairs, uint32_t npairs, const uint32_t* matches,
                       const uint8_t* mask, double* cosine_ws, PoseOut* out, hipStream_t s);

struct alignas(128) TvgOut {
    amc_tvg g;
    unsigned long long prof[8];
    unsigned long long work[12];
};
struct TvgParams {
    int32_t min_num_inliers, detect_watermark, force_H_use, min_num_trials;
    int32_t max_trials[4];
    double min_E_F_inlier_ratio, max_H_inlier_ratio, watermark_min_inlier_ratio,
        watermark_border_size, max_error;
    int32_t force_slow_sampler;
    int32_t no_fast_count;
    int32_t no_fast32;
    int32_t mode;
    uint32_t* bad_index_count;
    const double* wm_cut;
    const uint32_t* stream;
    uint32_t stream_len;
    uint32_t* stream_err;
};
struct alignas(64) TvgEState {
    double model[9];
    double sum;
    int32_t cnt, success, num_trials;
    uint32_t soff;
};
void tvg_diag_report();
void tvg_diag_report_e();
size_t tvg_ws_doubles_host(uint32_t mcap);
size_t tvg_ws_doubles_e_host(uint32_t mcap);
size_t tvg_ws_mask_bytes_host(uint32_t mcap);
constexpr int kTvgEWavesPerSimd = 2;
constexpr int kTvgFhWavesPerSimd = 4;
size_t tvg_lds_bytes(uint32_t mcap, int waves);
size_t tvg_lds_bytes_e(uint32_t mcap, int waves);
hipError_t launch_pack_verify(const TvgOut* out, const TvgPair* tp, uint32_t npairs, const uint8_t* mask_src,
                              const uint64_t* moff, amc_tvg* tvg_dst, uint8_t* mask_dst, unsigned long long* work,
                              int32_t trivial_below, hipStream_t s);
hipError_t launch_homography_decomposition(const double* in27, const double* p1, const double* p2, uint32_t n, double* out16,
                                           double* points3D, hipStream_t s);
hipError_t launch_sampson(const double* p1, const double* p2, size_t n, const double* E9, double* out,
                          hipStream_t s);
hipError_t launch_tvg_e(const TvgImage* imgs, const TvgPair* pairs, uint32_t npairs, const uint32_t* matches,
                        const uint32_t* trial_tabs, const TvgParams& P, double* ws, uint32_t mcap, uint32_t num_waves,
                        int waves_per_block, uint32_t* queue_head, TvgEState* estate, uint8_t* emask, TvgOut* out,
                        uint8_t* out_mask, hipStream_t s);
hipError_t launch_tvg_fh(const TvgImage* imgs, const TvgPair* pairs, uint32_t npairs, const uint32_t* matches,
                         const uint32_t* trial_tabs, const TvgParams& P, double* ws, uint8_t* mask_ws, uint32_t mcap,
                         uint32_t num_waves, int waves_per_block, uint32_t* queue_head, const TvgEState* estate,
                         const uint8_t* emask, TvgOut* out, uint8_t* out_mask, hipStream_t s);

size_t tvg_big_lds_bytes(int waves);
size_t tvg_big_lds_bytes_e(int waves);
size_t tvg_big_idx_doubles_host(uint32_t mcap);
hipError_t launch_tvg_e_big(const TvgImage* imgs, const TvgPair* pairs, uint32_t npairs, const uint32_t* matches,
                            const uint32_t* trial_tabs, const TvgParams& P, double* ws, uint32_t mcap, uint32_t num_waves,
                            int waves_per_block, uint32_t* queue_head, TvgEState* estate, uint8_t* emask, TvgOut* out,
                            uint8_t* out_mask, hipStream_t s);
hipError_t launch_tvg_fh_big(const TvgImage* imgs, const TvgPair* pairs, uint32_t npairs, const uint32_t* matches,
                             const uint32_t* trial_tabs, const TvgParams& P, double* ws, uint8_t* mask_ws, uint32_t mcap,
                             uint32_t num_waves, int waves_per_block, uint32_t* queue_head, const TvgEState* estate,
                             const uint8_t* emask, TvgOut* out, uint8_t* out_mask, hipStream_t s);

}
```

pycolmap_amd/csrc/amc_match.hip:

```cpp
#include <algorithm>
#include <chrono>
#include <cstdio>
#include <cstdlib>
#include <cstring>
#include <limits>
#include <memory>
#include <new>
#include <vector>

#include "amc_ctx.h"

using namespace amc;

namespace {

struct ResultPriv {
    std::vector<uint64_t> offsets;
    PinBuf<uint32_t> matches;
    std::shared_ptr<PinnedPool> pool;
    ~ResultPriv() {
        if (pool) pool->give_back(std::move(matches));
    }
};

constexpr size_t kMaxTop2Entries = (size_t)256 << 20;
constexpr size_t kMaxMatchCap = (size_t)256 << 20;

}

static void guided_grid_setup(GuidedDev& g, const GridDev& g1, const GridDev& g2, bool dense_only) {
    g.grid_ok = 0;
    g.bound[0] = g.bound[1] = 0.0;
    for (int k = 0; k < 9; ++k) g.minv[k] = 0.0;
    if (dense_only || g1.n == 0 || g2.n == 0) return;
    const float box1[4] = {g1.x0, g1.y0, g1.bx1, g1.by1}, box2[4] = {g2.x0, g2.y0, g2.bx1, g2.by1};
    g.grid_ok = guided::guided_pair_setup(g.kind, g.m, g.max_residual, box1, box2, g.bound, g.minv) ? 1 : 0;
}

int amc::match_impl(amc_ctx* c, const uint32_t* slot1, const uint32_t* slot2, size_t npairs,
                    const amc_match_opts* opts_in, const amc_tvg* geoms, double max_error,
                    amc_match_result* out, std::vector<uint64_t>* keep_off, const BatchHook* batch_hook) {
    if (!c || !out) return api_fail(AMC_E_INVALID, "amc_match_pairs: NULL ctx/out");
    std::memset(out, 0, sizeof *out);
    if (npairs > 0 && (!slot1 || !slot2))
        return api_fail(AMC_E_INVALID, "amc_match_pairs: NULL pair arrays");
    const bool prof = env_flag("AMC_MATCH_PROFILE");
    const bool guided_dense_only = env_flag("AMC_GUIDED_DENSE");
    const bool accept_trivial = env_flag("AMC_SCAN_ACCEPT_TRIVIAL");
    const bool resolve_ungrouped = env_flag("AMC_RESOLVE_UNGROUPED");
    const size_t batch_entries = (size_t)env_int("AMC_MATCH_BATCH_ENTRIES", 0, 0, (long long)kMaxTop2Entries);
    const char* const d2h_env = std::getenv("AMC_D2H");
    const size_t fuse_min_bytes = (size_t)env_int("AMC_D2H_FUSE_MIN_BYTES", 1 << 20, 0, std::numeric_limits<long long>::max());
    const int hook_split_mode = (int)env_int("AMC_HOOK_SPLIT", 1, 0, 2);
    const auto wall0 = std::chrono::steady_clock::now();
    double t_prepare = 0.0, t_collect = 0.0, t_enqueue = 0.0, t_scatter = 0.0;
    auto since = [](std::chrono::steady_clock::time_point t) {
        return std::chrono::duration<double, std::milli>(std::chrono::steady_clock::now() - t).count();
    };
    amc_match_opts o;
    if (opts_in) o = *opts_in; else amc_match_opts_default(&o);
    if (o.kernel != AMC_KERNEL_AUTO && o.kernel != AMC_KERNEL_MFMA && o.kernel != AMC_KERNEL_DOT4)
        return api_fail(AMC_E_INVALID, "amc_match_pairs: unknown kernel %d", o.kernel);
    uint64_t rows_total = 0;
    for (size_t i = 0; i < npairs; ++i) {
        if (slot1[i] >= c->slots.size() || slot2[i] >= c->slots.size())
            return api_fail(AMC_E_INVALID, "amc_match_pairs: pair %zu references slot out of range", i);
        if (!c->slots[slot1[i]].valid || !c->slots[slot2[i]].valid)
            return api_fail(AMC_E_STATE, "amc_match_pairs: pair %zu references a slot with no "
                            "descriptors uploaded", i);
        rows_total += c->slots[slot1[i]].dev.rows_pad;
    }
    std::vector<GuidedDev> h_guided;
    if (geoms) {
        h_guided.resize(npairs);
        for (size_t i = 0; i < npairs; ++i) {
            const int cfg = geoms[i].config;
            GuidedDev& g = h_guided[i];
            g.kind = (cfg == AMC_TVG_CALIBRATED || cfg == AMC_TVG_UNCALIBRATED) ? kGuidedF
                     : (cfg == AMC_TVG_PLANAR || cfg == AMC_TVG_PANORAMIC || cfg == AMC_TVG_PLANAR_OR_PANORAMIC)
                         ? kGuidedH : kGuidedNone;
            if (g.kind == kGuidedNone)
                return api_fail(AMC_E_INVALID, "amc_match_guided_pairs: pair %zu: configuration %d has no guided "
                                "matching (COLMAP keeps the inlier matches it has)", i, cfg);
            const double* m = g.kind == kGuidedF ? geoms[i].F : geoms[i].H;
            for (int k = 0; k < 9; ++k) g.m[k] = (float)m[k];
            g.max_residual = (float)(max_error * max_error);
            const Slot& a = c->slots[slot1[i]];
            const Slot& b = c->slots[slot2[i]];
            if (!a.kp || !b.kp || a.kp_rows < a.dev.rows || b.kp_rows < b.dev.rows)
                return api_fail(AMC_E_STATE, "amc_match_guided_pairs: pair %zu: float32 keypoints (one per descriptor) "
                                "must be uploaded for both images", i);
            guided_grid_setup(g, a.grid, b.grid, guided_dense_only);
        }
    }
    HIPCHK(hipSetDevice(c->device));
    hipStream_t st = c->stream;

    if (c->table_dirty) {
        HIPCHK(c->d_imgs.ensure(c->slots.size()));
        std::vector<ImageDev> t(c->slots.size());
        for (size_t i = 0; i < t.size(); ++i) t[i] = c->slots[i].dev;
        if (!t.empty())
            HIPCHK(hipMemcpy(c->d_imgs.p, t.data(), t.size() * sizeof(ImageDev),
                             hipMemcpyHostToDevice));
        HIPCHK(c->d_grids.ensure(c->slots.size()));
        std::vector<GridDev> gt(c->slots.size());
        for (size_t i = 0; i < gt.size(); ++i) gt[i] = c->slots[i].grid;
        if (!gt.empty())
            HIPCHK(hipMemcpy(c->d_grids.p, gt.data(), gt.size() * sizeof(GridDev), hipMemcpyHostToDevice));
        c->table_dirty = false;
    }

    const float max_ratio_f = (float)o.max_ratio;
    FinalizeParams fp;
    fp.max_ratio = max_ratio_f;
    fp.max_distance = (float)o.max_distance;
    fp.cross_check = o.cross_check ? 1 : 0;
    fp.reserved = 0;

    if (!c->accept_valid || std::memcmp(&c->accept_ratio, &fp.max_ratio, sizeof(float)) != 0 ||
        std::memcmp(&c->accept_distance, &fp.max_distance, sizeof(float)) != 0) {
        c->h_accept = build_scan_accept(c->h_lut.data(), (uint32_t)c->h_lut.size(), fp.max_ratio, fp.max_distance);
        if (accept_trivial) c->h_accept.trivial = 1;
        if (!c->d_accept) HIPCHK(hipMalloc(reinterpret_cast<void**>(&c->d_accept), sizeof(ScanAccept)));
        HIPCHK(hipStreamSynchronize(st));
        HIPCHK(hipMemcpy(c->d_accept, &c->h_accept, sizeof(ScanAccept), hipMemcpyHostToDevice));
        c->accept_ratio = fp.max_ratio;
        c->accept_distance = fp.max_distance;
        c->accept_valid = true;
    }
    HIPCHK(hipEventRecord(c->ev[0], st));
    ResultPriv* priv = new (std::nothrow) ResultPriv();
    if (!priv) return api_fail(AMC_E_NOMEM, "amc_match_pairs: out of host memory");
    priv->offsets.assign(npairs + 1, 0);
    priv->pool = c->result_pool;
    priv->matches = c->result_pool->acquire();
    size_t keep_used = 0;
    c->resident_matches = 0;
    c->vres = amc::VerifyResident{};
    if (keep_off) keep_off->assign(npairs, 0);

    const size_t mfma_max_cols = kSelectMaxCols;

    uint64_t num_dist = 0, n_mfma = 0, n_dot4 = 0, n_grid = 0;
    double kernel_ms = 0.0, cross_ms = 0.0;
    uint32_t kernel_launches = 0;

    int rc = AMC_OK;
    auto hc = [&](hipError_t e, const char* what) {
        if (e != hipSuccess && rc == AMC_OK)
            rc = api_fail(AMC_E_HIP, "amc_match_pairs: %s: %s", what, hipGetErrorString(e));
        return e == hipSuccess;
    };
    const size_t max_entries = batch_entries ? batch_entries : kMaxTop2Entries;

    struct Batch {
        size_t begin = 0, end = 0, nb = 0, top_rows = 0, top_cols = 0, cap = 0;
        size_t row_off = 0, nwork = 0, nord = 0, nwork_grid = 0;
        uint32_t max_cols = 0;
        size_t ngrp = 0, ngrp2 = 0, seg_cap = 0;
        int set = 0;
        uint32_t total = 0;
        bool grouped_resolve = true;
    };
    uint64_t rows_carved = 0, rows_collected = 0;
    const int d2h_mode = !d2h_env ? 0 : (std::strcmp(d2h_env, "memcpy") == 0 ? 2 : (std::strcmp(d2h_env, "stream") == 0 ? 1 : 0));
    struct PendingCopy {
        void* dst = nullptr;
        const void* src = nullptr;
        size_t bytes = 0;
        int set = -1;
    } pending;
    constexpr uint32_t kCopyParts = 64 / kSegsPerItem;
    auto sync_batch_streams = [&](const char* what) { return hc(hipStreamSynchronize(st), what); };
    const bool hook_split = batch_hook && hook_split_mode != 0;
    const size_t hook_split_min_pairs = hook_split_mode == 2 ? 2 : 4096;
    auto carve = [&](size_t begin, int set) {
        Batch b;
        b.begin = b.end = begin;
        b.set = set;
        size_t limit = max_entries;
        const uint64_t rows_left = rows_total - rows_carved;
        if (begin > 0 && rows_left <= max_entries && rows_left > max_entries / 4)
            limit = (size_t)(rows_left - max_entries / 4);
        if (begin == 0 && hook_split && rows_total <= max_entries && npairs >= hook_split_min_pairs)
            limit = (size_t)(rows_total * 6 / 10);
        while (b.end < npairs) {
            const Slot& x = c->slots[slot1[b.end]];
            const Slot& y = c->slots[slot2[b.end]];
            const size_t nr = x.dev.rows_pad, nc = y.dev.rows_pad;
            const size_t mc = o.cross_check ? std::min(x.dev.rows, y.dev.rows) : x.dev.rows;
            if (b.end > b.begin && (b.top_rows + nr > limit || b.top_cols + nc > max_entries ||
                                    b.cap + mc > kMaxMatchCap || b.end - b.begin >= (1u << 24)))
                break;
            b.top_rows += nr; b.top_cols += nc; b.cap += mc; ++b.end;
        }
        b.nb = b.end - b.begin;
        rows_carved += b.top_rows;
        return b;
    };
    auto build_reverse_order = [&](Batch& b) {
        const int k = b.set;
        const size_t nord = b.nord;
        if (!nord || !o.cross_check) return;
        const PairDev* hp = c->h_pairs[k].p;
        const size_t nslots = c->slots.size();
        std::vector<uint32_t> cnt(nslots + 1), tmp(nord);
        auto by_slot = [&](const uint32_t* src, uint32_t* dst, bool key_is_slot2) {
            std::fill(cnt.begin(), cnt.end(), 0u);
            for (size_t q = 0; q < nord; ++q) ++cnt[(key_is_slot2 ? hp[src[q]].slot2 : hp[src[q]].slot1) + 1];
            for (size_t v = 0; v < nslots; ++v) cnt[v + 1] += cnt[v];
            for (size_t q = 0; q < nord; ++q) dst[cnt[key_is_slot2 ? hp[src[q]].slot2 : hp[src[q]].slot1]++] = src[q];
        };
        uint32_t* ord2 = c->h_order2[k].p;
        by_slot(c->h_order[k].p, tmp.data(), true);
        by_slot(tmp.data(), ord2, false);
        size_t ngrp2 = 0;
        for (size_t q = 0; q < nord; ++q)
            if (q == 0 || hp[ord2[q]].slot1 != hp[ord2[q - 1]].slot1) c->h_grp2[k].p[ngrp2++] = (uint32_t)q;
        c->h_grp2[k].p[ngrp2] = (uint32_t)nord;
    };
    auto prepare = [&](Batch& b, bool defer_reverse) {
        const int k = b.set;
        const size_t nb = b.nb, begin = b.begin;
        if (!hc(c->h_pairs[k].ensure(nb), "pinned pairs") || !hc(c->h_order[k].ensure(nb), "pinned order") ||
            !hc(c->h_order2[k].ensure(nb), "pinned order2") || !hc(c->h_pair_off[k].ensure(nb), "pinned pair_off") ||
            !hc(c->h_pair_cnt[k].ensure(nb), "pinned pair_cnt") || !hc(c->h_bscalars[k].ensure(16), "pinned scalars"))
            return false;
        std::vector<uint8_t> want_mfma(nb, 0);
        for (size_t i = 0; i < nb; ++i) {
            const Slot& x = c->slots[slot1[begin + i]];
            const Slot& y = c->slots[slot2[begin + i]];
            const bool nonempty = x.dev.rows > 0 && y.dev.rows > 0;
            want_mfma[i] = nonempty && o.kernel != AMC_KERNEL_DOT4 && !geoms &&
                           (!o.cross_check || y.dev.rows_pad <= mfma_max_cols);
        }
        PairDev* hp = c->h_pairs[k].p;
        size_t row_off = 0, col_off = 0, nwork = 0, nord = 0, nimg1 = 0;
        std::vector<uint8_t> seen1(c->slots.size(), 0);
        b.grouped_resolve = !resolve_ungrouped;
        for (size_t i = 0; i < nb; ++i) {
            const Slot& x = c->slots[slot1[begin + i]];
            const Slot& y = c->slots[slot2[begin + i]];
            const bool nonempty = x.dev.rows > 0 && y.dev.rows > 0;
            if (o.kernel == AMC_KERNEL_MFMA && nonempty && !want_mfma[i]) {
                rc = api_fail(AMC_E_INVALID,
                              "amc_match_pairs: kernel=MFMA forced but pair %zu is not eligible "
                              "(rows_pad=%u, cols_pad=%u > %zu)", begin + i, x.dev.rows_pad,
                              y.dev.rows_pad, mfma_max_cols);
                return false;
            }
            PairDev& pd = hp[i];
            pd.slot1 = slot1[begin + i];
            pd.slot2 = slot2[begin + i];
            pd.mode = want_mfma[i] ? 1u : 0u;
            pd.pad = 0;
            pd.row_off = row_off;
            pd.col_off = col_off;
            row_off += x.dev.rows_pad;
            col_off += y.dev.rows_pad;
            num_dist += (uint64_t)x.dev.rows * y.dev.rows;
            if (!nonempty) continue;
            if (want_mfma[i]) {
                c->h_order[k].p[nord++] = (uint32_t)i;
                if (!seen1[pd.slot1]) { seen1[pd.slot1] = 1; ++nimg1; }
                ++n_mfma;
                b.max_cols = std::max(b.max_cols, y.dev.rows);
                if (std::max(x.dev.rows_pad, y.dev.rows_pad) > resolve_grouped_max_rows()) b.grouped_resolve = false;
            } else {
                nwork += (x.dev.rows + 63) / 64;
                if (o.cross_check) nwork += (y.dev.rows + 63) / 64;
                if (geoms && h_guided[begin + i].grid_ok) ++n_grid; else ++n_dot4;
            }
        }
        if (nord) {
            const size_t nslots = c->slots.size();
            std::vector<uint32_t> cnt(nslots + 1), tmp(nord);
            auto by_slot = [&](const uint32_t* src, uint32_t* dst, bool key_is_slot2) {
                std::fill(cnt.begin(), cnt.end(), 0u);
                for (size_t q = 0; q < nord; ++q) ++cnt[(key_is_slot2 ? hp[src[q]].slot2 : hp[src[q]].slot1) + 1];
                for (size_t v = 0; v < nslots; ++v) cnt[v + 1] += cnt[v];
                for (size_t q = 0; q < nord; ++q) dst[cnt[key_is_slot2 ? hp[src[q]].slot2 : hp[src[q]].slot1]++] = src[q];
            };
            uint32_t* ord = c->h_order[k].p;
            by_slot(ord, tmp.data(), false);
            by_slot(tmp.data(), ord, true);
        }
        b.ngrp = b.ngrp2 = 0;
        b.seg_cap = 0;
        if (nord) {
            if (!hc(c->h_grp[k].ensure(nord + 1), "pinned group cuts") ||
                (o.cross_check && !hc(c->h_grp2[k].ensure(nord + 1), "pinned group cuts")))
                return false;
            size_t seg1 = 0, seg2 = 0;
            for (size_t q = 0; q < nord; ++q) {
                const PairDev& pq = hp[c->h_order[k].p[q]];
                if (q == 0 || pq.slot2 != hp[c->h_order[k].p[q - 1]].slot2) c->h_grp[k].p[b.ngrp++] = (uint32_t)q;
                seg1 += (c->slots[pq.slot1].dev.rows + kSegRows - 1) / kSegRows;
                seg2 += (c->slots[pq.slot2].dev.rows + kSegRows - 1) / kSegRows;
            }
            c->h_grp[k].p[b.ngrp] = (uint32_t)nord;
            if (o.cross_check) b.ngrp2 = nimg1;
            b.seg_cap = std::max(seg1 + kSegsPerItem * b.ngrp, o.cross_check ? seg2 + kSegsPerItem * b.ngrp2 : 0);
        }
        b.nwork_grid = 0;
        if (nwork) {
            if (!hc(c->h_work[k].ensure(nwork), "pinned work")) return false;
            size_t w = 0;
            for (int pass = geoms ? 0 : 1; pass < 2; ++pass) {
                for (size_t i = 0; i < nb; ++i) {
                    if (hp[i].mode) continue;
                    if (geoms && (h_guided[begin + i].grid_ok != 0) != (pass == 0)) continue;
                    const Slot& x = c->slots[slot1[begin + i]];
                    const Slot& y = c->slots[slot2[begin + i]];
                    if (x.dev.rows == 0 || y.dev.rows == 0) continue;
                    for (uint32_t rb = 0; rb < (x.dev.rows + 63) / 64; ++rb)
                        c->h_work[k].p[w++] = Dot4Work{(uint32_t)i, 0u, rb};
                    if (o.cross_check)
                        for (uint32_t rb = 0; rb < (y.dev.rows + 63) / 64; ++rb)
                            c->h_work[k].p[w++] = Dot4Work{(uint32_t)i, 1u, rb};
                }
                if (pass == 0) b.nwork_grid = w;
            }
        }
        b.row_off = row_off;
        b.nwork = nwork;
        b.nord = nord;
        if (!defer_reverse) build_reverse_order(b);
        return true;
    };
    auto enqueue_scan = [&](Batch& b) {
        const int k = b.set;
        amc_ctx::MatchScratch& S = c->ms;
        const size_t nb = b.nb, nord = b.nord, nwork = b.nwork;
        const bool grow = S.d_pairs.cap < nb || S.d_order.cap < nb || S.d_order2.cap < nb ||
                          S.d_rowbuf.cap < b.top_rows || S.d_colbuf.cap < b.top_cols ||
                          S.d_accmask.cap < b.top_rows / 32 + 8 || S.d_pair_off.cap < nb || S.d_pair_cnt.cap < nb ||
                          S.d_matches.cap < 2 * b.cap || S.d_cand_cnt.cap < nb || S.d_candbuf.cap < b.top_cols ||
                          S.d_live.cap < nb || S.d_live_fwd.cap < nb || S.d_live_all.cap < nb || S.d_live_rev.cap < nb ||
                          S.d_live_scan.cap < live_scratch_words(nb) ||
                          S.d_work.cap < nwork || (geoms && S.d_guided.cap < nb) || S.d_segs.cap < b.seg_cap ||
                          S.d_seg_base.cap < nord || S.d_grp.cap < b.ngrp + 1 || S.d_grp2.cap < b.ngrp2 + 1 ||
                          S.d_grp_segs.cap < std::max(b.ngrp, b.ngrp2) || S.d_grp_item_base.cap < std::max(b.ngrp, b.ngrp2);
        if (grow && !sync_batch_streams("sync before growing device scratch")) return false;
        if (!hc(S.d_pairs.ensure(nb), "dev pairs") || !hc(S.d_order.ensure(nb), "dev order") ||
            !hc(S.d_order2.ensure(nb), "dev order2") ||
            !hc(S.d_rowbuf.ensure(b.top_rows), "row top2") || !hc(S.d_colbuf.ensure(b.top_cols), "col top2") ||
            !hc(S.d_accmask.ensure(b.top_rows / 32 + 8), "accept mask") ||
            !hc(S.d_pair_off.ensure(nb), "pair_off") || !hc(S.d_pair_cnt.ensure(nb), "pair_cnt") ||
            !hc(S.d_matches.ensure(2 * b.cap), "dev matches") ||
            !hc(S.d_cand_cnt.ensure(nb), "cand_cnt") || !hc(S.d_candbuf.ensure(b.top_cols), "candbuf") ||
            !hc(S.d_live.ensure(nb), "live flags") || !hc(S.d_live_fwd.ensure(nb), "live list (forward)") ||
            !hc(S.d_live_all.ensure(nb), "live list") || !hc(S.d_live_rev.ensure(nb), "live list (reverse)") ||
            !hc(S.d_live_scan.ensure(live_scratch_words(nb)), "live list scratch") ||
            (nwork && !hc(S.d_work.ensure(nwork), "dev work")) || (geoms && !hc(S.d_guided.ensure(nb), "dev guided")) ||
            !hc(S.d_segs.ensure(b.seg_cap), "segment descriptors") || !hc(S.d_seg_base.ensure(nord), "segment bases") ||
            !hc(S.d_grp.ensure(b.ngrp + 1), "group cuts") || !hc(S.d_grp2.ensure(b.ngrp2 + 1), "group cuts") ||
            !hc(S.d_grp_segs.ensure(std::max(b.ngrp, b.ngrp2)), "group segments") ||
            !hc(S.d_grp_item_base.ensure(std::max(b.ngrp, b.ngrp2)), "group items"))
            return false;
        bool okq = hc(hipMemcpyAsync(S.d_pairs.p, c->h_pairs[k].p, nb * sizeof(PairDev),
                                     hipMemcpyHostToDevice, st), "H2D pairs") &&
                   hc(memset_async(c->d_scalars, 0, 2 * sizeof(uint32_t), st), "memset cursor") &&
                   hc(memset_async(c->d_scalars + 3, 0, sizeof(uint32_t), st), "memset errcount");
        if (okq && nord)
            okq = hc(hipMemcpyAsync(S.d_order.p, c->h_order[k].p, nord * sizeof(uint32_t),
                                    hipMemcpyHostToDevice, st), "H2D order") &&
                  hc(hipMemcpyAsync(S.d_grp.p, c->h_grp[k].p, (b.ngrp + 1) * sizeof(uint32_t),
                                    hipMemcpyHostToDevice, st), "H2D group cuts") &&
                  hc(memset_async(S.d_accmask.p, 0, (b.row_off / 32 + 8) * sizeof(uint32_t), st), "memset accmask");
        if (okq && nwork)
            okq = hc(hipMemcpyAsync(S.d_work.p, c->h_work[k].p, nwork * sizeof(Dot4Work),
                                    hipMemcpyHostToDevice, st), "H2D work");
        if (okq && geoms)
            okq = hc(hipMemcpyAsync(S.d_guided.p, h_guided.data() + b.begin, nb * sizeof(GuidedDev),
                                    hipMemcpyHostToDevice, st), "H2D guided");
        if (!okq) return false;
        if (nord &&
            !hc(launch_build_segments(0, c->d_imgs.p, S.d_pairs.p, S.d_order.p, S.d_grp.p, (uint32_t)b.ngrp,
                                      S.d_cand_cnt.p, S.d_candbuf.p, S.d_rowbuf.p, S.d_seg_base.p, S.d_grp_segs.p,
                                      S.d_grp_item_base.p, S.d_segs.p, c->d_scalars + 5, st), "segment packing"))
            return false;
        if (!hc(hipEventRecord(c->bev[k][0], st), "event record")) return false;
        if (nord) {
            CopyJob job;
            const uintptr_t ps = reinterpret_cast<uintptr_t>(pending.src), pd = reinterpret_cast<uintptr_t>(pending.dst);
            const bool take = pending.set >= 0 && d2h_mode == 0 && b.seg_cap > 0 && pending.bytes >= fuse_min_bytes &&
                              (ps & 15) == (pd & 15);
            int done_set = -1;
            if (take) {
                const size_t head = (ps & 15) ? 16 - (ps & 15) : 0, n16 = (pending.bytes - head) / 16;
                const size_t tail = pending.bytes - head - n16 * 16;
                if (head && !hc(memcpy_async(pending.dst, pending.src, head, hipMemcpyDeviceToHost, st), "D2H matches (head)"))
                    return false;
                if (tail && !hc(memcpy_async(static_cast<char*>(pending.dst) + head + n16 * 16,
                                             static_cast<const char*>(pending.src) + head + n16 * 16, tail,
                                             hipMemcpyDeviceToHost, st), "D2H matches (tail)"))
                    return false;
                job.src = static_cast<const char*>(pending.src) + head;
                job.dst = static_cast<char*>(pending.dst) + head;
                job.n16 = n16;
                job.parts = kCopyParts;
                done_set = pending.set;
                pending.set = -1;
            }
            if (!hc(launch_match_mfma(0, S.d_segs.p, c->d_scalars + 5, (uint32_t)std::min<size_t>(b.seg_cap, 0xFFFFFFFFu),
                                      c->d_scalars + 1, S.d_accmask.p, c->d_accept, st, job, c->d_scalars + 7), "forward scan"))
                return false;
            if (done_set >= 0 && !hc(hipEventRecord(c->bev[done_set][4], st), "event record")) return false;
        }
        if (b.nwork_grid &&
            !hc(launch_match_guided_grid(c->d_imgs.p, c->d_grids.p, S.d_pairs.p, S.d_work.p, (uint32_t)b.nwork_grid,
                                         S.d_rowbuf.p, S.d_colbuf.p, S.d_guided.p, st), "guided scan"))
            return false;
        if (nwork > b.nwork_grid &&
            !hc(launch_match_dot4(c->d_imgs.p, S.d_pairs.p, S.d_work.p + b.nwork_grid, (uint32_t)(nwork - b.nwork_grid),
                                  S.d_rowbuf.p, S.d_colbuf.p, geoms ? S.d_guided.p : nullptr, st), "dot4 scan"))
            return false;
        kernel_launches += (nord ? 1 : 0) + (b.nwork_grid ? 1 : 0) + (nwork > b.nwork_grid ? 1 : 0);
        return hc(hipEventRecord(c->bev[k][1], st), "event record");
    };
    auto enqueue_chain = [&](Batch& b) {
        const int k = b.set;
        amc_ctx::MatchScratch& S = c->ms;
        const size_t nb = b.nb, nord = b.nord;
        uint32_t* const nlive = c->d_scalars + 8;
        if (!hc(launch_live_pairs(c->d_imgs.p, S.d_pairs.p, (uint32_t)nb, S.d_accmask.p, S.d_order.p, (uint32_t)nord,
                                  S.d_live.p, S.d_live_fwd.p, S.d_live_all.p, nlive, S.d_cand_cnt.p, S.d_pair_cnt.p,
                                  S.d_pair_off.p, S.d_live_scan.p, st), "live pairs"))
            return false;
        if (nord &&
            !hc(launch_resolve_index(0, c->d_imgs.p, S.d_pairs.p, S.d_rowbuf.p, S.d_accmask.p, c->d_lut,
                                     fp, S.d_cand_cnt.p, S.d_candbuf.p, c->d_scalars + 3, b.grouped_resolve,
                                     S.d_live_fwd.p, nlive, (uint32_t)nord, st), "resolve (rows)"))
            return false;
        if (nord && o.cross_check) {
            if (!hc(launch_select_candidates(c->d_imgs.p, S.d_pairs.p, (uint32_t)nb, b.max_cols, S.d_rowbuf.p,
                                             S.d_accmask.p, c->d_lut, fp, S.d_cand_cnt.p, S.d_candbuf.p,
                                             S.d_live_all.p, nlive + 1, st),
                    "candidate selection"))
                return false;
            if (!hc(hipMemcpyAsync(S.d_order2.p, c->h_order2[k].p, nord * sizeof(uint32_t),
                                   hipMemcpyHostToDevice, st), "H2D order2") ||
                !hc(hipMemcpyAsync(S.d_grp2.p, c->h_grp2[k].p, (b.ngrp2 + 1) * sizeof(uint32_t),
                                   hipMemcpyHostToDevice, st), "H2D group cuts"))
                return false;
            if (!hc(launch_compact_order(S.d_order2.p, (uint32_t)nord, (uint32_t)nb, S.d_cand_cnt.p, S.d_live_rev.p, nlive + 2,
                                         S.d_live_scan.p, st),
                    "live pairs (reverse)") ||
                !hc(launch_build_segments(1, c->d_imgs.p, S.d_pairs.p, S.d_order2.p, S.d_grp2.p, (uint32_t)b.ngrp2,
                                          S.d_cand_cnt.p, S.d_candbuf.p, S.d_colbuf.p, S.d_seg_base.p, S.d_grp_segs.p,
                                          S.d_grp_item_base.p, S.d_segs.p, c->d_scalars + 5, st), "segment packing (reverse)") ||
                !hc(launch_match_mfma(1, S.d_segs.p, c->d_scalars + 5, (uint32_t)std::min<size_t>(b.seg_cap, 0xFFFFFFFFu),
                                      c->d_scalars + 1, S.d_accmask.p, c->d_accept, st), "reverse scan") ||
                !hc(launch_resolve_index(1, c->d_imgs.p, S.d_pairs.p, S.d_colbuf.p, S.d_accmask.p, c->d_lut,
                                         fp, S.d_cand_cnt.p, S.d_candbuf.p, c->d_scalars + 3, b.grouped_resolve,
                                         S.d_live_rev.p, nlive + 2, (uint32_t)nord, st), "resolve (columns)"))
                return false;
        }
        if (!hc(hipEventRecord(c->bev[k][2], st), "event record") ||
            !hc(launch_finalize(c->d_imgs.p, S.d_pairs.p, (uint32_t)nb, S.d_live_all.p, nlive + 1, S.d_rowbuf.p, S.d_colbuf.p,
                                S.d_accmask.p, c->d_lut, fp, c->d_scalars, (uint32_t)std::min(b.cap, (size_t)0xFFFFFFFFu),
                                S.d_pair_off.p, S.d_pair_cnt.p, S.d_matches.p, st), "finalize"))
            return false;
        return hc(hipMemcpyAsync(c->h_bscalars[k].p, c->d_scalars, 4 * sizeof(uint32_t),
                                 hipMemcpyDeviceToHost, st), "D2H cursor") &&
               hc(hipMemcpyAsync(c->h_pair_off[k].p, S.d_pair_off.p, nb * sizeof(uint32_t),
                                 hipMemcpyDeviceToHost, st), "D2H pair_off") &&
               hc(hipMemcpyAsync(c->h_pair_cnt[k].p, S.d_pair_cnt.p, nb * sizeof(uint32_t),
                                 hipMemcpyDeviceToHost, st), "D2H pair_cnt") &&
               hc(hipEventRecord(c->bev[k][3], st), "event record");
    };
    auto collect = [&](Batch& b) {
        const int k = b.set;
        amc_ctx::MatchScratch& S = c->ms;
        if (!hc(hipEventSynchronize(c->bev[k][3]), "wait for the batch")) return false;
        b.total = c->h_bscalars[k].p[0];
        if (c->h_bscalars[k].p[3] != 0) {
            rc = api_fail(AMC_E_HIP, "amc_match_pairs: internal: %u accepted rows could not be resolved "
                          "to an index (scan/recompute mismatch)", c->h_bscalars[k].p[3]);
            return false;
        }
        if (b.total > b.cap) {
            rc = api_fail(AMC_E_HIP, "amc_match_pairs: internal: %u matches exceed capacity %zu", b.total, b.cap);
            return false;
        }
        if (!hc(c->h_csr[k].ensure(b.nb), "pinned csr")) return false;
        uint64_t run = keep_used;
        for (size_t i = 0; i < b.nb; ++i) {
            c->h_csr[k].p[i] = run;
            if (keep_off) (*keep_off)[b.begin + i] = run;
            run += c->h_pair_cnt[k].p[i];
            priv->offsets[b.begin + i + 1] = run;
        }
        if (run - keep_used != b.total) {
            rc = api_fail(AMC_E_HIP, "amc_match_pairs: internal: pair counts (%llu) disagree with the cursor (%u)",
                          (unsigned long long)(run - keep_used), b.total);
            return false;
        }
        rows_collected += b.top_rows;
        if (b.total) {
            const auto tgrow = std::chrono::steady_clock::now();
            const size_t need = 2 * (keep_used + (size_t)b.total);
            size_t want = need;
            if (rows_collected > 0 && rows_collected < rows_total) {
                const double est = std::min((double)need * ((double)rows_total / (double)rows_collected) * 1.1, 4.0 * (double)need);
                want = std::max(need, (size_t)est / 2 * 2);
            }
            if (need > c->d_keep.cap) {
                DevBuf<uint32_t> bigger;
                if (bigger.ensure(std::max(want, 2 * c->d_keep.cap)) != hipSuccess) {
                    (void)hipGetLastError();
                    if (!hc(bigger.ensure(need), "resident match table")) return false;
                }
                if (keep_used &&
                    !hc(hipMemcpyAsync(bigger.p, c->d_keep.p, 2 * keep_used * sizeof(uint32_t), hipMemcpyDeviceToDevice, st),
                        "move resident match table"))
                    return false;
                if (!sync_batch_streams("sync before freeing the old resident table") ||
                    !hc(hipStreamSynchronize(c->copy_stream), "sync before freeing the old resident table"))
                    return false;
                c->d_keep = std::move(bigger);
            }
            if (need > priv->matches.cap) {
                if (!sync_batch_streams("sync before growing the result buffer") ||
                    !hc(hipStreamSynchronize(c->copy_stream), "sync before growing the result buffer"))
                    return false;
                PinBuf<uint32_t> bigger;
                if (bigger.ensure(std::max(want, 2 * priv->matches.cap)) != hipSuccess) {
                    (void)hipGetLastError();
                    if (prof) std::fprintf(stderr, "[amc match profile] pinned result: %zu words refused, asking for %zu\n", want, need);
                    if (!hc(bigger.ensure(need), "pinned result")) return false;
                }
                if (keep_used) std::memcpy(bigger.p, priv->matches.p, 2 * keep_used * sizeof(uint32_t));
                priv->matches = std::move(bigger);
            }
            if (prof && since(tgrow) > 5.0)
                std::fprintf(stderr, "[amc match profile] batch of %zu pairs: %.1f ms growing the result tables to %zu words\n", b.nb,
                             since(tgrow), priv->matches.cap);
            if (!hc(c->d_csr.ensure(b.nb), "dev csr") ||
                !hc(hipMemcpyAsync(c->d_csr.p, c->h_csr[k].p, b.nb * sizeof(uint64_t), hipMemcpyHostToDevice, st), "H2D csr"))
                return false;
            if (!hc(launch_reorder_matches(S.d_pair_off.p, S.d_pair_cnt.p, c->d_csr.p, (uint32_t)b.nb, S.d_matches.p,
                                           c->d_keep.p, st), "reorder launch"))
                return false;
            pending.dst = priv->matches.p + 2 * keep_used;
            pending.src = c->d_keep.p + 2 * keep_used;
            pending.bytes = (size_t)b.total * 2 * sizeof(uint32_t);
            pending.set = k;
            keep_used += b.total;
            return true;
        }
        return hc(hipEventRecord(c->bev[k][4], st), "event record");
    };
    double t_hook = 0.0;
    auto run_hook = [&](const Batch& b) {
        if (!batch_hook) return true;
        const auto th = std::chrono::steady_clock::now();
        const int hrc = (*batch_hook)(b.begin, b.end, priv->offsets.data(), keep_off ? keep_off->data() : nullptr);
        t_hook += since(th);
        if (hrc != AMC_OK && rc == AMC_OK) rc = hrc;
        return hrc == AMC_OK;
    };
    auto flush_copy = [&]() {
        if (pending.set < 0) return true;
        const int k = pending.set;
        pending.set = -1;
        if (!hc(hipEventRecord(c->cev[k], st), "event record") || !hc(hipStreamWaitEvent(c->copy_stream, c->cev[k], 0), "stream wait"))
            return false;
        if (d2h_mode == 2) {
            if (!hc(hipMemcpyAsync(pending.dst, pending.src, pending.bytes, hipMemcpyDeviceToHost, c->copy_stream), "D2H matches"))
                return false;
        } else {
            if (!hc(launch_host_copy(pending.dst, pending.src, pending.bytes, c->copy_stream), "D2H matches")) return false;
        }
        return hc(hipEventRecord(c->bev[k][4], c->copy_stream), "event record");
    };
    auto scatter = [&](Batch& b) {
        const int k = b.set;
        if (!hc(hipEventSynchronize(c->bev[k][4]), "wait for the matches")) return false;
        float ms = 0.f;
        if (hipEventElapsedTime(&ms, c->bev[k][0], c->bev[k][1]) == hipSuccess) kernel_ms += ms;
        if (hipEventElapsedTime(&ms, c->bev[k][1], c->bev[k][2]) == hipSuccess) cross_ms += ms;
        return true;
    };

    if (npairs > 0) {
        Batch cur = carve(0, 0);
        auto tp = std::chrono::steady_clock::now();
        bool ok = prepare(cur, true);
        t_prepare += since(tp);
        tp = std::chrono::steady_clock::now();
        ok = ok && enqueue_scan(cur);
        if (ok) build_reverse_order(cur);
        ok = ok && enqueue_chain(cur);
        t_enqueue += since(tp);
        Batch prev;
        bool have_prev = false;
        while (ok) {
            Batch next;
            const bool have_next = cur.end < npairs;
            if (have_next) {
                tp = std::chrono::steady_clock::now();
                next = carve(cur.end, cur.set ^ 1);
                ok = prepare(next, false);
                t_prepare += since(tp);
            }
            tp = std::chrono::steady_clock::now();
            if (ok && have_prev) ok = scatter(prev);
            t_scatter += since(tp);
            tp = std::chrono::steady_clock::now();
            ok = ok && collect(cur);
            t_collect += since(tp);
            tp = std::chrono::steady_clock::now();
            if (ok && have_next) ok = enqueue_scan(next) && enqueue_chain(next);
            ok = ok && flush_copy();
            t_enqueue += since(tp);
            ok = ok && run_hook(cur);
            if (!have_next) {
                tp = std::chrono::steady_clock::now();
                ok = ok && scatter(cur);
                t_scatter += since(tp);
                break;
            }
            prev = cur;
            have_prev = true;
            cur = next;
        }
        if (!ok && rc == AMC_OK) rc = api_fail(AMC_E_HIP, "amc_match_pairs: batch failed");
        if (rc != AMC_OK) {
            (void)hipStreamSynchronize(st);
            (void)hipStreamSynchronize(c->copy_stream);
        }
    }
    if (rc == AMC_OK && npairs > 0 &&
        hc(hipEventRecord(c->cev[0], c->copy_stream), "event record"))
        hc(hipStreamWaitEvent(st, c->cev[0], 0), "stream wait");
    if (rc == AMC_OK && hc(hipEventRecord(c->ev[1], st), "event record")) hc(hipEventSynchronize(c->ev[1]), "wait for the call");
    if (rc != AMC_OK) {
        delete priv;
        return rc;
    }
    float total_ms = 0.f;
    (void)hipEventElapsedTime(&total_ms, c->ev[0], c->ev[1]);

    out->npairs = npairs;
    c->resident_matches = keep_used;
    out->offsets = priv->offsets.data();
    out->matches = priv->offsets[npairs] ? priv->matches.p : nullptr;
    out->num_distances = num_dist;
    out->pairs_mfma = n_mfma;
    out->pairs_dot4 = n_dot4;
    out->pairs_guided_grid = n_grid;
    out->device_ms = total_ms;
    out->match_kernel_ms = kernel_ms;
    out->match_kernel_launches = kernel_launches;
    out->cross_kernel_ms = cross_ms;
    out->_priv = priv;
    c->last_hook_ms = t_hook;
    if (prof)
        std::fprintf(stderr, "[amc match profile] pairs=%zu wall=%.1f ms: prepare %.1f, enqueue %.1f, collect(wait+reorder+D2H enqueue) %.1f, "
                     "scatter(wait) %.1f, batch hook %.1f; device events %.1f ms (scan %.1f, cross %.1f)\n", npairs, since(wall0), t_prepare,
                     t_enqueue, t_collect, t_scatter, t_hook, (double)total_ms, kernel_ms, cross_ms);
    return AMC_OK;
}

extern "C" {

int amc_match_pairs(amc_ctx* c, const uint32_t* slot1, const uint32_t* slot2, size_t npairs,
                    const amc_match_opts* opts_in, amc_match_result* out) {
    return match_impl(c, slot1, slot2, npairs, opts_in, nullptr, 0.0, out);
}

int amc_match_guided_pairs(amc_ctx* c, const uint32_t* slot1, const uint32_t* slot2, size_t npairs,
                           const amc_tvg* geoms, double max_error, const amc_match_opts* opts_in,
                           amc_match_result* out) {
    if (npairs > 0 && !geoms) {
        if (out) std::memset(out, 0, sizeof *out);
        return api_fail(AMC_E_INVALID, "amc_match_guided_pairs: NULL geometries");
    }
    if (!(max_error >= 0.0)) {
        if (out) std::memset(out, 0, sizeof *out);
        return api_fail(AMC_E_INVALID, "amc_match_guided_pairs: max_error must be >= 0");
    }
    static const amc_tvg kNone{};
    return match_impl(c, slot1, slot2, npairs, opts_in, npairs ? geoms : &kNone, max_error, out);
}

void amc_match_result_free(amc_match_result* r) {
    if (!r) return;
    delete static_cast<ResultPriv*>(r->_priv);
    std::memset(r, 0, sizeof *r);
}

}
```

pycolmap_amd/csrc/match_mfma.hip:

```cpp
#include <cstdlib>

#include "amc_internal.h"
#include "scan_accept.h"

namespace amc {

typedef int i32x4 __attribute__((ext_vector_type(4)));
typedef __attribute__((address_space(1))) const void gvoid_t;
typedef __attribute__((address_space(3))) void lvoid_t;

constexpr int kBN = 128;
constexpr int kYS = kBN / 32;
constexpr int kUR = 128;
constexpr int kSPB = kUR / 32;
constexpr int kChunkBytes = kBN * kDim;
constexpr int kW = kSegsPerItem;
constexpr int kWGPerCU = 2;
constexpr int kXT = kSegRows / 16;
constexpr int kKeyShift = 7, kKeyCarried = 127;

constexpr int kNB = 4;
constexpr int kOffRs = 0;
constexpr int kOffQ = kOffRs + kNB * kBN * 4;
constexpr int kOffB = kOffQ + 16;
constexpr int kLdsBytes = kOffB + kNB * kChunkBytes;
static_assert(kRowPad % kBN == 0, "a chunk divides the row padding: every chunk that holds a row lies inside the padded image");
static_assert(kUR == 128 && kSPB == 4 && kBN == kUR, "a lane quarter's rows of a block are one 32-row tile; the loop body is one block, which is one chunk");
static_assert(kRowPad % kSegRows == 0 && kSegRows % 32 == 0, "segments tile the padded rows");
static_assert((kNB & (kNB - 1)) == 0, "the ring position is taken modulo kNB with a mask");
static_assert(kWGPerCU * kLdsBytes <= 160 * 1024, "LDS of one CU holds two workgroups");
static_assert(kW == 4, "one wave of a workgroup per SIMD");
static_assert(sizeof(SegDesc) == 64, "a descriptor is 16 dwords: one per lane of a quarter wave");

enum : int { kDXprep = 0, kDXrs = 2, kDOut = 4, kDList = 6, kDYprep = 8, kDYrs = 10, kDCnt = 12, kDAccword = 13,
             kDYrows = 14 };

__device__ __forceinline__ void mfma_first(i32x4& d, const i32x4& a, const i32x4& b, const i32x4& c) {
    asm volatile("v_mfma_i32_16x16x64_i8 %0, %1, %2, %3" : "=&v"(d) : "v"(a), "v"(b), "v"(c));
}
__device__ __forceinline__ void mfma_acc(i32x4& d, const i32x4& a, const i32x4& b) {
    asm volatile("v_mfma_i32_16x16x64_i8 %0, %1, %2, %0" : "+v"(d) : "v"(a), "v"(b));
}

struct YFrag {
    i32x4 f[2][2];
    i32x4 ci[2];
};

#ifdef AMC_SCAN_STAMPS
constexpr int kStampMaxWG = 1024;
__device__ uint32_t g_scan_stamps[2 * kStampMaxWG * kSegsPerItem * 8];
#define AMC_STAMP() ((uint32_t)__builtin_amdgcn_s_memtime())
#endif

__device__ __noinline__ __attribute__((used)) void copy_part(const uint4* __restrict__ src, uint4* __restrict__ dst,
                                                             unsigned long long b, unsigned long long e, int tid,
                                                             int nthreads) {
    __builtin_assume(tid >= 0 && tid < 1024 && nthreads >= 256 && nthreads <= 512);
    unsigned long long i = b + (unsigned long long)tid;
    const unsigned long long st = (unsigned long long)nthreads;
    for (; i + 3 * st < e; i += 4 * st) {
        const uint4 v0 = src[i], v1 = src[i + st], v2 = src[i + 2 * st], v3 = src[i + 3 * st];
        dst[i] = v0; dst[i + st] = v1; dst[i + 2 * st] = v2; dst[i + 3 * st] = v3;
    }
    for (; i < e; i += st) dst[i] = src[i];
}

template <int MODE>
__global__ __launch_bounds__(64 * kW) __attribute__((amdgpu_waves_per_eu(kWGPerCU, kWGPerCU)))
void match_mfma_kernel(const SegDesc* __restrict__ segs, const uint32_t* __restrict__ nitems_p,
                       uint32_t* __restrict__ queue_head, uint32_t* __restrict__ accmask,
                       const ScanAccept* __restrict__ accept, CopyJob job, uint32_t* __restrict__ copy_head) {
    static_assert(kChunkBytes / 1024 == kW * kYS, "a chunk splits into 1 KiB DMA pieces, one per wave and step");
    static_assert(kBN * 4 == 512, "a chunk's rs128 block is half a wave's DMA");
    __shared__ __attribute__((aligned(16))) char smem[kLdsBytes];

    const int tid = threadIdx.x;
    const int lane = tid & 63;
    const int wid = __builtin_amdgcn_readfirstlane(tid >> 6);
    const int l15 = lane & 15, lq = lane >> 4;
    volatile uint32_t* s_q = reinterpret_cast<volatile uint32_t*>(smem + kOffQ);
    if constexpr (MODE == 0) {
        if (job.parts) {
            volatile uint32_t* s_part = reinterpret_cast<volatile uint32_t*>(smem + kOffQ + 4);
            if (tid == 0) *s_part = atomicAdd(copy_head, 1u);
            __syncthreads();
            const uint32_t part = *s_part;
            if (part < job.parts)
                copy_part(static_cast<const uint4*>(job.src), static_cast<uint4*>(job.dst), job.n16 * part / job.parts,
                          job.n16 * (part + 1) / job.parts, tid, 64 * kW);
        }
    }
    const uint32_t nitems = *nitems_p;
    const ScanAccept sa = *accept;

    auto load_desc = [&](uint32_t q) -> int {
        int v = 0;
        if (q < nitems && lane < 16) v = reinterpret_cast<const int*>(segs + (size_t)q * kSegsPerItem + wid)[lane];
        return v;
    };
    auto dword = [&](int dv, int f) -> int { return __builtin_amdgcn_readlane(dv, f); };
    auto dptr = [&](int dv, int f) -> const char* {
        const uint64_t lo = (uint32_t)__builtin_amdgcn_readlane(dv, f);
        const uint64_t hi = (uint32_t)__builtin_amdgcn_readlane(dv, f + 1);
        return reinterpret_cast<const char*>(lo | (hi << 32));
    };

    constexpr int kPW = kChunkBytes / 1024 / kW;
    uint32_t lane16 = (uint32_t)lane * 16u;
    auto lane_off = [&]() __attribute__((always_inline)) -> uint32_t {
        asm volatile("" : "+v"(lane16));
        return lane16;
    };
    auto stage_piece = [&](const char* yprep, int c, int buf, int ps) __attribute__((always_inline)) {
        const int piece = ps * kW + wid;
        const char* src = yprep + ((size_t)c * kChunkBytes + piece * 1024);
        __builtin_amdgcn_global_load_lds((gvoid_t*)(src + lane_off()),
                                         (lvoid_t*)(smem + kOffB + buf * kChunkBytes + piece * 1024), 16, 0, 0);
    };
    auto stage_rs = [&](const char* yrs, int c, int buf) __attribute__((always_inline)) {
        const char* src = yrs + (size_t)c * kBN * 4;
        if (wid == 0 && lane < kBN / 4)
            __builtin_amdgcn_global_load_lds((gvoid_t*)(src + lane_off()), (lvoid_t*)(smem + kOffRs + buf * kBN * 4), 16, 0,
                                             0);
    };
    auto stage = [&](const char* yprep, const char* yrs, int c, int buf) __attribute__((always_inline)) {
#pragma unroll
        for (int ps = 0; ps < kPW; ++ps) stage_piece(yprep, c, buf, ps);
        stage_rs(yrs, c, buf);
    };
    auto stage_head = [&](int dv) __attribute__((always_inline)) {
        const char* yprep = dptr(dv, kDYprep);
        const char* yrs = dptr(dv, kDYrs);
        const int yrows = dword(dv, kDYrows);
        stage(yprep, yrs, 0, 0);
#pragma unroll
        for (int c = 1; c < kNB - 1; ++c)
            if (yrows > c * kBN) stage(yprep, yrs, c, c);
    };

    const int yrow_lane = (kUR / 4) * (l15 >> 2) + (l15 & 3);
    const int ysw_lane = arena_swizzle(yrow_lane);
    int yb0 = kOffB + yrow_lane * kDim + ((lq ^ ysw_lane) * 16);
    int yb1 = kOffB + yrow_lane * kDim + (((4 + lq) ^ ysw_lane) * 16);
    int cbs = kOffRs + (kUR / 4) * lq * 4;
    auto load_y_part = [&](YFrag& y, int ys, int part) __attribute__((always_inline)) {
        if (part < 2) {
            y.ci[part] = *reinterpret_cast<const i32x4*>(smem + cbs + (8 * ys * 4 + 16 * part));
        } else {
            const int tt = (part - 2) >> 1, s = (part - 2) & 1;
            y.f[tt][s] = *reinterpret_cast<const i32x4*>(smem + (s ? yb1 : yb0) + (8 * ys + tt * 4) * kDim);
        }
    };
    auto load_y = [&](YFrag& y, int ys) __attribute__((always_inline)) {
#pragma unroll
        for (int part = 0; part < 6; ++part) load_y_part(y, ys, part);
    };
    auto advance = [&](int cb) __attribute__((always_inline)) {
        const int k = cb == kNB - 1 ? -(kNB - 1) : 1;
        asm volatile("v_add_u32 %0, %3, %0\n\tv_add_u32 %1, %3, %1\n\tv_add_u32 %2, %4, %2"
                     : "+v"(yb0), "+v"(yb1), "+v"(cbs) : "s"(k * kChunkBytes), "s"(k * kBN * 4));
    };

    i32x4 xf[kXT][2];
    int best[kXT], sec[kXT], btile[kXT], xterm[kXT], part[kXT];
    auto load_x = [&](int dv) __attribute__((always_inline)) {
        const int cnt = dword(dv, kDCnt);
        const char* xprep = dptr(dv, kDXprep);
        const int* xrs = reinterpret_cast<const int*>(dptr(dv, kDXrs));
#pragma unroll
        for (int xt = 0; xt < kXT; ++xt) {
            const int kl = xt * 16 + l15;
            int row;
            if (MODE == 0) {
                row = kl;
            } else {
                const uint32_t* list = reinterpret_cast<const uint32_t*>(dptr(dv, kDList));
                row = cnt > 0 ? (int)list[min(kl, cnt - 1)] : 0;
            }
            const char* rp = xprep + (size_t)row * kDim;
            const int sw = arena_swizzle(row);
#pragma unroll
            for (int s = 0; s < 2; ++s) xf[xt][s] = *reinterpret_cast<const i32x4*>(rp + (((4 * s + lq) ^ sw) * 16));
            xterm[xt] = xrs[row] - (1 << 21);
            best[xt] = ((-xterm[xt]) << kKeyShift) | kKeyCarried;
            sec[xt] = best[xt];
            btile[xt] = -1;
        }
    };

#ifdef AMC_SCAN_STAMPS
    uint32_t st_a = 0, st_first = 0, st_end = 0, st_sum[5] = {0, 0, 0, 0, 0};
    bool st_prev = false, st_prev_active = false;
    uint32_t* const st_slot = g_scan_stamps + ((size_t)(MODE * kStampMaxWG + min((int)blockIdx.x, kStampMaxWG - 1)) * kW + wid) * 8;
#endif
    if (tid == 0) *s_q = atomicAdd(queue_head, 1u);
    __syncthreads();
    uint32_t q = *s_q;
    int dv = load_desc(q);
    if (q < nitems) {
        stage_head(dv);
        if (dword(dv, kDCnt) > 0) load_x(dv);
    }
    __syncthreads();

    while (q < nitems) {
        const char* yprep = dptr(dv, kDYprep);
        const char* yrs = dptr(dv, kDYrs);
        const int nchunks = (dword(dv, kDYrows) + kBN - 1) / kBN;
        const bool active = dword(dv, kDCnt) > 0;
        if (tid == 0) *s_q = atomicAdd(queue_head, 1u);

        i32x4 acc[2][2];
        auto insert = [&](int xt, int code) __attribute__((always_inline)) {
            asm volatile(
                "v_lshl_or_b32 %2, %2, 7, %3\n\t"
                "v_med3_i32 %1, %0, %1, %2\n\t"
                "v_max_i32 %0, %0, %2"
                : "+v"(best[xt]), "+v"(sec[xt]), "+v"(part[xt])
                : "s"(code));
        };
        auto flush = [&](int sb) __attribute__((always_inline)) {
#pragma unroll
            for (int xt = 0; xt < kXT; ++xt) {
                const int c = best[xt] & 127;
                btile[xt] = c != kKeyCarried ? sb * 64 + (126 - c) : btile[xt];
                best[xt] |= kKeyCarried;
            }
        };
        auto phase = [&](i32x4 (&an)[2], const YFrag& y, int xtn, const i32x4 (&ac)[2], int xtc, int sp, int gb)
                         __attribute__((always_inline)) {
            mfma_first(an[0], y.f[0][0], xf[xtn][0], y.ci[0]);
            mfma_first(an[1], y.f[1][0], xf[xtn][0], y.ci[1]);
            __builtin_amdgcn_sched_barrier(0);
            if (xtc == 0 ? sp == 0 : sp == kSPB - 1) {
                insert((xtc + kXT - 1) % kXT, 126 - ((xtc == 0 ? gb - 1 : gb) & 63));
                if (xtc == 0 && gb != 0 && (gb & 63) == 0) flush((gb >> 6) - 1);
                __builtin_amdgcn_sched_barrier(0);
            }
            mfma_acc(an[0], y.f[0][1], xf[xtn][1]);
            mfma_acc(an[1], y.f[1][1], xf[xtn][1]);
            __builtin_amdgcn_sched_barrier(0);
            int t0, t1;
            if (sp == 0)
                asm volatile(
                    "v_max3_i32 %0, %3, %4, %5\n\t"
                    "v_max3_i32 %1, %6, %7, %8\n\t"
                    "v_max3_i32 %0, %0, %9, %10\n\t"
                    "v_max_i32 %2, %0, %1"
                    : "=&v"(t0), "=&v"(t1), "=&v"(part[xtc])
                    : "v"(ac[0][0]), "v"(ac[0][1]), "v"(ac[0][2]), "v"(ac[0][3]), "v"(ac[1][0]), "v"(ac[1][1]),
                      "v"(ac[1][2]), "v"(ac[1][3]));
            else
                asm volatile(
                    "v_max3_i32 %0, %3, %4, %5\n\t"
                    "v_max3_i32 %1, %6, %7, %8\n\t"
                    "v_max3_i32 %0, %0, %9, %10\n\t"
                    "v_max3_i32 %2, %0, %1, %2"
                    : "=&v"(t0), "=&v"(t1), "+v"(part[xtc])
                    : "v"(ac[0][0]), "v"(ac[0][1]), "v"(ac[0][2]), "v"(ac[0][3]), "v"(ac[1][0]), "v"(ac[1][1]),
                      "v"(ac[1][2]), "v"(ac[1][3]));
            __builtin_amdgcn_sched_barrier(0);
        };

        YFrag y0, y1;
        asm volatile("s_waitcnt vmcnt(0)" ::: "memory");
        __syncthreads();
        const uint32_t qn = *s_q;
        const int dvn = load_desc(qn);
#ifdef AMC_SCAN_STAMPS
        {
            const uint32_t now = AMC_STAMP();
            if (st_prev) {
                st_sum[0] += st_a;
                st_sum[1] += now - st_end;
                st_sum[2] += now - st_first;
                st_sum[3] += 1;
                st_sum[4] += st_prev_active ? 1 : 0;
                if (lane == 0) {
#pragma unroll
                    for (int k = 0; k < 5; ++k) st_slot[k] = st_sum[k];
                }
            }
            st_a = 0;
            st_first = now;
        }
#endif
        static_assert(kPW == kYS, "one DMA piece per wave and step");
        static_assert(kNB == 4, "the counted waits below are written out for three chunks ahead");
        auto crossing = [&](bool steady, int rem) __attribute__((always_inline)) {
#ifdef AMC_SCAN_STAMPS
            const uint32_t st_t = AMC_STAMP();
#endif
            if (steady) {
                if (wid == 0) asm volatile("s_waitcnt vmcnt(%0)" ::"n"(2 * kPW + 2) : "memory");
                else asm volatile("s_waitcnt vmcnt(%0)" ::"n"(2 * kPW) : "memory");
            } else if (rem >= 2) {
                if (wid == 0) asm volatile("s_waitcnt vmcnt(%0)" ::"n"(kPW + 1) : "memory");
                else asm volatile("s_waitcnt vmcnt(%0)" ::"n"(kPW) : "memory");
            } else {
                asm volatile("s_waitcnt vmcnt(0)" ::: "memory");
            }
            asm volatile("s_barrier" ::: "memory");
#ifdef AMC_SCAN_STAMPS
            st_a += AMC_STAMP() - st_t;
#endif
        };
        auto fetch = [&](int c, int cb, int ys) __attribute__((always_inline)) {
            const int fb = (cb + kNB - 1) & (kNB - 1);
            stage_piece(yprep, c + kNB - 1, fb, ys);
            if (ys == 0) stage_rs(yrs, c + kNB - 1, fb);
        };
        int c = 0, cb = 0;
        if (active) {
            load_y(y0, 0);
            mfma_first(acc[0][0], y0.f[0][0], xf[0][0], y0.ci[0]);
            mfma_first(acc[0][1], y0.f[1][0], xf[0][0], y0.ci[1]);
            mfma_acc(acc[0][0], y0.f[0][1], xf[0][1]);
            mfma_acc(acc[0][1], y0.f[1][1], xf[0][1]);
            part[kXT - 1] = -(1 << 24);
            __builtin_amdgcn_sched_barrier(0);
            auto step = [&](YFrag& yc, YFrag& yn, int ys, bool steady) __attribute__((always_inline)) {
                if (steady) fetch(c, cb, ys);
                if (ys == kYS - 1) {
                    const int rem = nchunks - 1 - c;
                    if (steady || rem >= 1) crossing(steady, rem);
                    advance(cb);
                }
                const int nys = ys == kYS - 1 ? 0 : ys + 1;
#pragma unroll
                for (int xt = 0; xt < kXT; ++xt) {
                    if (xt + 1 < kXT)
                        phase(acc[(xt + 1) & 1], yc, xt + 1, acc[xt & 1], xt, ys, c);
                    else
                        phase(acc[0], yn, 0, acc[xt & 1], xt, ys, c);
                    if (xt < 6) {
                        load_y_part(yn, nys, xt);
                        __builtin_amdgcn_sched_barrier(0);
                    }
                }
            };
#pragma unroll 1
            for (; c + kNB - 1 < nchunks; ++c, cb = (cb + 1) & (kNB - 1)) {
                step(y0, y1, 0, true);
                step(y1, y0, 1, true);
                step(y0, y1, 2, true);
                step(y1, y0, 3, true);
            }
#pragma unroll 1
            for (; c < nchunks; ++c, cb = (cb + 1) & (kNB - 1)) {
                step(y0, y1, 0, false);
                step(y1, y0, 1, false);
                step(y0, y1, 2, false);
                step(y1, y0, 3, false);
            }
            yb0 -= cb * kChunkBytes;
            yb1 -= cb * kChunkBytes;
            cbs -= cb * kBN * 4;
            const int lastb = nchunks - 1;
            insert(kXT - 1, 126 - (lastb & 63));
            flush(lastb >> 6);
#pragma unroll
            for (int xt = 0; xt < kXT; ++xt) {
                best[xt] >>= kKeyShift;
                sec[xt] >>= kKeyShift;
            }
        } else {
#pragma unroll 1
            for (; c + kNB - 1 < nchunks; ++c, cb = (cb + 1) & (kNB - 1)) {
#pragma unroll
                for (int ys = 0; ys < kYS; ++ys) fetch(c, cb, ys);
                crossing(true, kNB - 1);
            }
#pragma unroll 1
            for (; c + 1 < nchunks; ++c) crossing(false, nchunks - 1 - c);
        }
        __syncthreads();
#ifdef AMC_SCAN_STAMPS
        st_end = AMC_STAMP();
        st_prev = true;
        st_prev_active = active;
#endif

        int eb[kXT], es[kXT], et[kXT], ex[kXT];
#pragma unroll
        for (int xt = 0; xt < kXT; ++xt) {
            asm volatile("v_mov_b32 %0, %1" : "=v"(eb[xt]) : "v"(best[xt]));
            asm volatile("v_mov_b32 %0, %1" : "=v"(es[xt]) : "v"(sec[xt]));
            asm volatile("v_mov_b32 %0, %1" : "=v"(et[xt]) : "v"(btile[xt]));
            ex[xt] = xterm[xt];
        }
        if (qn < nitems) {
            stage_head(dvn);
            if (dword(dvn, kDCnt) > 0) load_x(dvn);
        }
        if (active) {
            const int cnt = dword(dv, kDCnt);
            uint32_t bits_lo = 0;
#pragma unroll
            for (int xt = 0; xt < kXT; ++xt) {
                const int kl = xt * 16 + l15;
                int b = eb[xt], s = es[xt], t = et[xt] < 0 ? -1 : et[xt] * kSPB + lq;
#pragma unroll
                for (int m = 16; m <= 32; m <<= 1) {
                    const int ob = __shfl_xor(b, m);
                    const int os = __shfl_xor(s, m);
                    const int ot = __shfl_xor(t, m);
                    const bool ow = (ob > b) || (ob == b && (unsigned)ot < (unsigned)t);
                    s = max(max(s, os), ow ? b : ob);
                    t = ow ? ot : t;
                    b = ow ? ob : b;
                }
                bool acc_bit = false;
                const bool live = lq == 0 && kl < cnt;
                Top2 o;
                o.best_v = (uint32_t)(b + ex[xt]);
                o.best_idx = o.best_v ? (uint32_t)t : 0xFFFFFFFFu;
                o.second_v = (uint32_t)(s + ex[xt]);
                o.pad = 0;
                if (MODE == 0) acc_bit = live && scan_may_accept(sa, o.best_v, o.second_v);
                const uint32_t bits = MODE == 0 ? (uint32_t)__ballot(acc_bit) : 0u;
                if (live && (MODE == 1 || bits != 0)) {
                    Top2* out = reinterpret_cast<Top2*>(const_cast<char*>(dptr(dv, kDOut)));
                    int row = kl;
                    if (MODE == 1) row = (int)reinterpret_cast<const uint32_t*>(dptr(dv, kDList))[kl];
                    out[row] = o;
                }
                if (MODE == 0) {
                    if (xt & 1) {
                        const uint32_t word = bits_lo | (bits << 16);
                        if (lane == 0 && word != 0) accmask[(uint32_t)dword(dv, kDAccword) + (xt >> 1)] = word;
                    } else {
                        bits_lo = bits;
                    }
                }
            }
        }
#ifdef AMC_SCAN_STAMPS
        if (qn >= nitems && lane == 0) {
            st_slot[5] = st_a;
            st_slot[6] = AMC_STAMP() - st_first;
            st_slot[7] = 1;
        }
#endif
        q = qn;
        dv = dvn;
    }
}

__device__ __forceinline__ uint32_t pair_segments(int mode, const ImageDev* imgs, const PairDev& p, uint32_t pi,
                                                  const uint32_t* cand_cnt, uint32_t* nrows_out) {
    const uint32_t nx = mode == 0 ? imgs[p.slot1].rows : cand_cnt[pi];
    const uint32_t ny = imgs[mode == 0 ? p.slot2 : p.slot1].rows;
    *nrows_out = nx;
    return ny ? (nx + kSegRows - 1) / kSegRows : 0u;
}

__global__ __launch_bounds__(256) void seg_count_kernel(int mode, const ImageDev* __restrict__ imgs,
                                                        const PairDev* __restrict__ pairs,
                                                        const uint32_t* __restrict__ order,
                                                        const uint32_t* __restrict__ grp_start,
                                                        const uint32_t* __restrict__ cand_cnt,
                                                        uint32_t* __restrict__ seg_base, uint32_t* __restrict__ grp_segs) {
    __shared__ uint32_t wsum[4];
    const uint32_t g = blockIdx.x, tid = threadIdx.x, lane = tid & 63, wid = tid >> 6;
    const uint32_t i0 = grp_start[g], i1 = grp_start[g + 1];
    uint32_t running = 0;
    for (uint32_t base = i0; base < i1; base += 256) {
        const uint32_t i = base + tid;
        uint32_t s = 0, nr;
        if (i < i1) {
            const uint32_t pi = order[i];
            s = pair_segments(mode, imgs, pairs[pi], pi, cand_cnt, &nr);
        }
        uint32_t inc = s;
#pragma unroll
        for (int m = 1; m < 64; m <<= 1) {
            const uint32_t o = __shfl_up(inc, m);
            if (lane >= (uint32_t)m) inc += o;
        }
        if (lane == 63) wsum[wid] = inc;
        __syncthreads();
        uint32_t wbase = 0, total = 0;
        for (uint32_t k = 0; k < 4; ++k) {
            if (k < wid) wbase += wsum[k];
            total += wsum[k];
        }
        if (i < i1) seg_base[i] = running + wbase + inc - s;
        running += total;
        __syncthreads();
    }
    if (tid == 0) grp_segs[g] = running;
}

__global__ __launch_bounds__(1024) void seg_scan_kernel(const uint32_t* __restrict__ grp_segs, uint32_t ngroups,
                                                        uint32_t* __restrict__ grp_item_base,
                                                        uint32_t* __restrict__ nitems_out) {
    __shared__ uint32_t wsum[16];
    const uint32_t tid = threadIdx.x, lane = tid & 63, wid = tid >> 6;
    uint32_t running = 0;
    for (uint32_t base = 0; base < ngroups; base += 1024) {
        const uint32_t g = base + tid;
        const uint32_t s = g < ngroups ? (grp_segs[g] + kSegsPerItem - 1) / kSegsPerItem : 0u;
        uint32_t inc = s;
#pragma unroll
        for (int m = 1; m < 64; m <<= 1) {
            const uint32_t o = __shfl_up(inc, m);
            if (lane >= (uint32_t)m) inc += o;
        }
        if (lane == 63) wsum[wid] = inc;
        __syncthreads();
        uint32_t wbase = 0, total = 0;
        for (uint32_t k = 0; k < 16; ++k) {
            if (k < wid) wbase += wsum[k];
            total += wsum[k];
        }
        if (g < ngroups) grp_item_base[g] = running + wbase + inc - s;
        running += total;
        __syncthreads();
    }
    if (tid == 0) *nitems_out = running;
}

constexpr uint32_t kFillY = 8;
__global__ __launch_bounds__(256) void seg_fill_kernel(int mode, const ImageDev* __restrict__ imgs,
                                                       const PairDev* __restrict__ pairs,
                                                       const uint32_t* __restrict__ order,
                                                       const uint32_t* __restrict__ grp_start,
                                                       const uint32_t* __restrict__ cand_cnt,
                                                       const uint32_t* __restrict__ candbuf,
                                                       const uint32_t* __restrict__ seg_base,
                                                       const uint32_t* __restrict__ grp_segs,
                                                       const uint32_t* __restrict__ grp_item_base,
                                                       Top2* __restrict__ outbuf, SegDesc* __restrict__ segs) {
    const uint32_t g = blockIdx.x, tid = threadIdx.x, lane = tid & 63, wid = blockIdx.y * 4 + (tid >> 6);
    const uint32_t i0 = grp_start[g], i1 = grp_start[g + 1];
    if (i0 >= i1) return;
    const uint32_t total = grp_segs[g];
    if (total == 0) return;
    SegDesc* gs = segs + (size_t)grp_item_base[g] * kSegsPerItem;
    const PairDev p0 = pairs[order[i0]];
    const ImageDev Y = imgs[mode == 0 ? p0.slot2 : p0.slot1];
    for (uint32_t i = i0 + wid; i < i1; i += 4 * kFillY) {
        const uint32_t pi = order[i];
        const PairDev p = pairs[pi];
        uint32_t nx;
        const uint32_t ns = pair_segments(mode, imgs, p, pi, cand_cnt, &nx);
        const ImageDev X = imgs[mode == 0 ? p.slot1 : p.slot2];
        const uint32_t sb = seg_base[i];
        for (uint32_t k = lane; k < ns; k += 64) {
            const uint32_t row0 = k * kSegRows;
            SegDesc d;
            d.yprep = Y.prep;
            d.yrs = Y.rs128;
            d.yrows = Y.rows;
            d.cnt = min(nx - row0, (uint32_t)kSegRows);
            d.pad_ = 0;
            if (mode == 0) {
                d.xprep = X.prep + (size_t)row0 * kDim;
                d.xrs = X.rs128 + row0;
                d.out = outbuf + p.row_off + row0;
                d.list = nullptr;
                d.accword = (uint32_t)((p.row_off + row0) >> 5);
            } else {
                d.xprep = X.prep;
                d.xrs = X.rs128;
                d.out = outbuf + p.col_off;
                d.list = candbuf + p.col_off + row0;
                d.accword = 0;
            }
            gs[sb + k] = d;
        }
    }
    const uint32_t padded = (total + kSegsPerItem - 1) / kSegsPerItem * kSegsPerItem;
    if (blockIdx.y == 0 && tid < padded - total) {
        SegDesc d;
        d.xprep = Y.prep;
        d.xrs = Y.rs128;
        d.out = nullptr;
        d.list = nullptr;
        d.yprep = Y.prep;
        d.yrs = Y.rs128;
        d.cnt = 0;
        d.accword = 0;
        d.yrows = Y.rows;
        d.pad_ = 0;
        gs[total + tid] = d;
    }
}

hipError_t launch_build_segments(int mode, const ImageDev* imgs, const PairDev* pairs, const uint32_t* order,
                                 const uint32_t* grp_start, uint32_t ngroups, const uint32_t* cand_cnt,
                                 const uint32_t* candbuf, Top2* outbuf, uint32_t* seg_base, uint32_t* grp_segs,
                                 uint32_t* grp_item_base, SegDesc* segs, uint32_t* nitems_dev, hipStream_t s) {
    if (ngroups == 0) return memset_async(nitems_dev, 0, sizeof(uint32_t), s);
    hipLaunchKernelGGL(seg_count_kernel, dim3(ngroups), dim3(256), 0, s, mode, imgs, pairs, order, grp_start,
                       cand_cnt, seg_base, grp_segs);
    hipLaunchKernelGGL(seg_scan_kernel, dim3(1), dim3(1024), 0, s, grp_segs, ngroups, grp_item_base, nitems_dev);
    hipLaunchKernelGGL(seg_fill_kernel, dim3(ngroups, kFillY), dim3(256), 0, s, mode, imgs, pairs, order, grp_start,
                       cand_cnt, candbuf, seg_base, grp_segs, grp_item_base, outbuf, segs);
    return hipGetLastError();
}

hipError_t launch_match_mfma(int mode, const SegDesc* segs, const uint32_t* nitems_dev, uint32_t max_items,
                             uint32_t* queue_head, uint32_t* accmask, const ScanAccept* accept_dev, hipStream_t s,
                             const CopyJob& job_in, uint32_t* copy_head) {
    if (max_items == 0) return hipSuccess;
    CopyJob job = (mode == 0 && copy_head) ? job_in : CopyJob();
    hipError_t e = job.parts ? memset_async(copy_head, 0, sizeof(uint32_t), s) : hipSuccess;
    if (e != hipSuccess) return e;
    int dev = 0, cus = 256;
    if ((e = hipGetDevice(&dev)) != hipSuccess) return e;
    if ((e = hipDeviceGetAttribute(&cus, hipDeviceAttributeMultiprocessorCount, dev)) != hipSuccess) return e;
    static const hipError_t occupancy = [] {
        int n0 = 0, n1 = 0;
        hipError_t oe = hipOccupancyMaxActiveBlocksPerMultiprocessor(&n0, match_mfma_kernel<0>, 64 * kW, 0);
        if (oe == hipSuccess) oe = hipOccupancyMaxActiveBlocksPerMultiprocessor(&n1, match_mfma_kernel<1>, 64 * kW, 0);
        if (oe != hipSuccess) return oe;
        return n0 >= kWGPerCU && n1 >= kWGPerCU ? hipSuccess : hipErrorLaunchOutOfResources;
    }();
    if (occupancy != hipSuccess) return occupancy;
    int wgs = kWGPerCU * cus;
    static const int grid_cap = [] {
        const char* e = std::getenv("AMC_SCAN_GRID");
        return e ? std::atoi(e) : 0;
    }();
    if (grid_cap > 0 && grid_cap < wgs) wgs = grid_cap;
    const uint32_t grid = max_items < (uint32_t)wgs ? max_items : (uint32_t)wgs;
    if (job.parts > grid) job.parts = grid;
    if ((e = memset_async(queue_head, 0, sizeof(uint32_t), s)) != hipSuccess) return e;
    if (mode == 0)
        hipLaunchKernelGGL((match_mfma_kernel<0>), dim3(grid), dim3(64 * kW), 0, s, segs, nitems_dev, queue_head,
                           accmask, accept_dev, job, copy_head);
    else
        hipLaunchKernelGGL((match_mfma_kernel<1>), dim3(grid), dim3(64 * kW), 0, s, segs, nitems_dev, queue_head,
                           accmask, accept_dev, job, copy_head);
    return hipGetLastError();
}

}
```

Measured before the change: 13630 billion distances/s.

## Batch scan work items into runs that reuse loaded X tiles across groups

Adds a run table that packs up to R work items from consecutive groups into a single queue ticket. Within a run, items that share the same X descriptor segment are flagged so the MFMA scan kernel keeps the loaded X tile and running top-2 state instead of reloading them. The goal is to cut redundant X loads and per-item atomic queue traffic. A host heuristic enables R=4 automatically when groups line up by slot1 and there is enough work per workgroup, at the cost of two extra build kernels, padded run entries and more complex control flow in the kernel.

```diff
diff --git a/include/amc.h b/include/amc.h
--- a/include/amc.h
+++ b/include/amc.h
@@ -42,6 +42,7 @@
     double match_kernel_ms;
     double cross_kernel_ms;
     uint32_t match_kernel_launches;
+    uint32_t scan_run;
     void* _priv;
 } amc_match_result;
 
diff --git a/profiles/chain/recipes/pick_summary.py b/profiles/chain/recipes/pick_summary.py
--- /dev/null
+++ b/profiles/chain/recipes/pick_summary.py
@@ -0,0 +1,4 @@
+import glob, json, os, sys
+for f in sorted(glob.glob(os.path.join(sys.argv[1], "*.json"))):
+    j = [json.loads(l) for l in open(f) if l.startswith("{")][-1]
+    print(os.path.basename(f), j["ms_per_step"], j["roofline"]["avg_kernel_ms"], j["config"]["matches_rank0"])
diff --git a/pycolmap_amd/_capi.py b/pycolmap_amd/_capi.py
--- a/pycolmap_amd/_capi.py
+++ b/pycolmap_amd/_capi.py
@@ -113,7 +113,7 @@
                 ("pairs_mfma", C.c_uint64), ("pairs_dot4", C.c_uint64), ("pairs_guided_grid", C.c_uint64),
                 ("device_ms", C.c_double), ("match_kernel_ms", C.c_double),
                 ("cross_kernel_ms", C.c_double),
-                ("match_kernel_launches", C.c_uint32), ("_priv", C.c_void_p)]
+                ("match_kernel_launches", C.c_uint32), ("scan_run", C.c_uint32), ("_priv", C.c_void_p)]
 
 
 class SiftOpts(C.Structure):
@@ -2095,7 +2095,7 @@
                      pairs_dot4=int(res.pairs_dot4), device_ms=float(res.device_ms),
                      match_kernel_ms=float(res.match_kernel_ms),
                      cross_kernel_ms=float(res.cross_kernel_ms),
-                     match_kernel_launches=int(res.match_kernel_launches))
+                     match_kernel_launches=int(res.match_kernel_launches), scan_run=int(res.scan_run))
         return offsets, matches, stats
 
     @staticmethod
diff --git a/pycolmap_amd/csrc/amc_ctx.h b/pycolmap_amd/csrc/amc_ctx.h
--- a/pycolmap_amd/csrc/amc_ctx.h
+++ b/pycolmap_amd/csrc/amc_ctx.h
@@ -153,6 +153,7 @@
         DevBuf<uint32_t> d_order, d_order2;
         DevBuf<uint32_t> d_grp, d_grp2, d_seg_base, d_grp_segs, d_grp_item_base;
         DevBuf<SegDesc> d_segs;
+        DevBuf<uint32_t> d_run_base, d_run_items;
         DevBuf<Top2> d_rowbuf, d_colbuf;
         DevBuf<uint32_t> d_accmask;
         DevBuf<GuidedDev> d_guided;
@@ -161,7 +162,7 @@
         void release_all() {
             d_pairs.release(); d_work.release(); d_order.release(); d_order2.release();
             d_grp.release(); d_grp2.release(); d_seg_base.release(); d_grp_segs.release();
-            d_grp_item_base.release(); d_segs.release();
+            d_grp_item_base.release(); d_segs.release(); d_run_base.release(); d_run_items.release();
             d_rowbuf.release(); d_colbuf.release(); d_accmask.release(); d_guided.release();
             d_pair_off.release(); d_pair_cnt.release(); d_matches.release();
             d_cand_cnt.release(); d_candbuf.release();
@@ -170,7 +171,7 @@
         }
         void release_large() {
             d_rowbuf.release(); d_colbuf.release(); d_accmask.release(); d_matches.release(); d_candbuf.release();
-            d_segs.release(); d_seg_base.release();
+            d_segs.release(); d_seg_base.release(); d_run_items.release();
         }
     };
     MatchScratch ms;
diff --git a/pycolmap_amd/csrc/amc_internal.h b/pycolmap_amd/csrc/amc_internal.h
--- a/pycolmap_amd/csrc/amc_internal.h
+++ b/pycolmap_amd/csrc/amc_internal.h
@@ -338,7 +338,10 @@
 };
 hipError_t launch_match_mfma(int mode, const SegDesc* segs, const uint32_t* nitems_dev, uint32_t max_items,
                        uint32_t* queue_head, uint32_t* accmask, const ScanAccept* accept_dev, hipStream_t s,
-                       const CopyJob& job = CopyJob(), uint32_t* copy_head = nullptr);
+                       const CopyJob& job = CopyJob(), uint32_t* copy_head = nullptr,
+                       const uint32_t* run_items = nullptr, uint32_t run_len = 1, const uint32_t* nruns_dev = nullptr);
+hipError_t launch_build_runs(const SegDesc* segs, const uint32_t* grp_segs, const uint32_t* grp_item_base, uint32_t ngroups,
+                       uint32_t R, uint32_t* run_base, uint32_t* run_items, uint32_t* nruns_dev, hipStream_t s);
 
 size_t live_scratch_words(size_t npairs);
 hipError_t launch_live_pairs(const ImageDev* imgs, const PairDev* pairs, uint32_t npairs, const uint32_t* accmask,
diff --git a/pycolmap_amd/csrc/amc_match.hip b/pycolmap_amd/csrc/amc_match.hip
--- a/pycolmap_amd/csrc/amc_match.hip
+++ b/pycolmap_amd/csrc/amc_match.hip
@@ -9,6 +9,7 @@
 #include <vector>
 
 #include "amc_ctx.h"
+#include "scan_run.h"
 
 using namespace amc;
 
@@ -51,6 +52,7 @@
     const size_t batch_entries = (size_t)env_int("AMC_MATCH_BATCH_ENTRIES", 0, 0, (long long)kMaxTop2Entries);
     const char* const d2h_env = std::getenv("AMC_D2H");
     const size_t fuse_min_bytes = (size_t)env_int("AMC_D2H_FUSE_MIN_BYTES", 1 << 20, 0, std::numeric_limits<long long>::max());
+    const int scan_run_env = (int)env_int("AMC_SCAN_RUN", 0, 0, 8);
     const int hook_split_mode = (int)env_int("AMC_HOOK_SPLIT", 1, 0, 2);
     const auto wall0 = std::chrono::steady_clock::now();
     double t_prepare = 0.0, t_collect = 0.0, t_enqueue = 0.0, t_scatter = 0.0;
@@ -144,7 +146,10 @@
 
     uint64_t num_dist = 0, n_mfma = 0, n_dot4 = 0, n_grid = 0;
     double kernel_ms = 0.0, cross_ms = 0.0;
-    uint32_t kernel_launches = 0;
+    uint32_t kernel_launches = 0, scan_run_max = 0;
+    int cus = 256;
+    (void)hipDeviceGetAttribute(&cus, hipDeviceAttributeMultiprocessorCount, c->device);
+    const size_t scan_workgroups = 2 * (size_t)cus;
 
     int rc = AMC_OK;
     auto hc = [&](hipError_t e, const char* what) {
@@ -162,6 +167,7 @@
         int set = 0;
         uint32_t total = 0;
         bool grouped_resolve = true;
+        int run = 1;
     };
     uint64_t rows_carved = 0, rows_collected = 0;
     const int d2h_mode = !d2h_env ? 0 : (std::strcmp(d2h_env, "memcpy") == 0 ? 2 : (std::strcmp(d2h_env, "stream") == 0 ? 1 : 0));
@@ -302,6 +308,10 @@
             c->h_grp[k].p[b.ngrp] = (uint32_t)nord;
             if (o.cross_check) b.ngrp2 = nimg1;
             b.seg_cap = std::max(seg1 + kSegsPerItem * b.ngrp, o.cross_check ? seg2 + kSegsPerItem * b.ngrp2 : 0);
+            const uint32_t* ord = c->h_order[k].p;
+            b.run = choose_scan_run_by([hp, ord](size_t q) { return hp[ord[q]].slot1; }, c->h_grp[k].p, b.ngrp,
+                                       seg1 / kSegsPerItem, scan_workgroups, scan_run_env);
+            scan_run_max = std::max(scan_run_max, (uint32_t)b.run);
         }
         b.nwork_grid = 0;
         if (nwork) {
@@ -333,6 +343,8 @@
         const int k = b.set;
         amc_ctx::MatchScratch& S = c->ms;
         const size_t nb = b.nb, nord = b.nord, nwork = b.nwork;
+        const size_t run_blocks = b.run > 1 ? (b.ngrp + b.run - 1) / b.run : 0;
+        const size_t run_entries = b.run > 1 ? (b.seg_cap / kSegsPerItem + 1) * b.run : 0;
         const bool grow = S.d_pairs.cap < nb || S.d_order.cap < nb || S.d_order2.cap < nb ||
                           S.d_rowbuf.cap < b.top_rows || S.d_colbuf.cap < b.top_cols ||
                           S.d_accmask.cap < b.top_rows / 32 + 8 || S.d_pair_off.cap < nb || S.d_pair_cnt.cap < nb ||
@@ -341,7 +353,8 @@
                           S.d_live_scan.cap < live_scratch_words(nb) ||
                           S.d_work.cap < nwork || (geoms && S.d_guided.cap < nb) || S.d_segs.cap < b.seg_cap ||
                           S.d_seg_base.cap < nord || S.d_grp.cap < b.ngrp + 1 || S.d_grp2.cap < b.ngrp2 + 1 ||
-                          S.d_grp_segs.cap < std::max(b.ngrp, b.ngrp2) || S.d_grp_item_base.cap < std::max(b.ngrp, b.ngrp2);
+                          S.d_grp_segs.cap < std::max(b.ngrp, b.ngrp2) || S.d_grp_item_base.cap < std::max(b.ngrp, b.ngrp2) ||
+                          S.d_run_base.cap < run_blocks || S.d_run_items.cap < run_entries;
         if (grow && !sync_batch_streams("sync before growing device scratch")) return false;
         if (!hc(S.d_pairs.ensure(nb), "dev pairs") || !hc(S.d_order.ensure(nb), "dev order") ||
             !hc(S.d_order2.ensure(nb), "dev order2") ||
@@ -357,7 +370,8 @@
             !hc(S.d_segs.ensure(b.seg_cap), "segment descriptors") || !hc(S.d_seg_base.ensure(nord), "segment bases") ||
             !hc(S.d_grp.ensure(b.ngrp + 1), "group cuts") || !hc(S.d_grp2.ensure(b.ngrp2 + 1), "group cuts") ||
             !hc(S.d_grp_segs.ensure(std::max(b.ngrp, b.ngrp2)), "group segments") ||
-            !hc(S.d_grp_item_base.ensure(std::max(b.ngrp, b.ngrp2)), "group items"))
+            !hc(S.d_grp_item_base.ensure(std::max(b.ngrp, b.ngrp2)), "group items") ||
+            !hc(S.d_run_base.ensure(run_blocks), "run bases") || !hc(S.d_run_items.ensure(run_entries), "run table"))
             return false;
         bool okq = hc(hipMemcpyAsync(S.d_pairs.p, c->h_pairs[k].p, nb * sizeof(PairDev),
                                      hipMemcpyHostToDevice, st), "H2D pairs") &&
@@ -380,6 +394,10 @@
             !hc(launch_build_segments(0, c->d_imgs.p, S.d_pairs.p, S.d_order.p, S.d_grp.p, (uint32_t)b.ngrp,
                                       S.d_cand_cnt.p, S.d_candbuf.p, S.d_rowbuf.p, S.d_seg_base.p, S.d_grp_segs.p,
                                       S.d_grp_item_base.p, S.d_segs.p, c->d_scalars + 5, st), "segment packing"))
+            return false;
+        if (nord && b.run > 1 &&
+            !hc(launch_build_runs(S.d_segs.p, S.d_grp_segs.p, S.d_grp_item_base.p, (uint32_t)b.ngrp, (uint32_t)b.run,
+                                  S.d_run_base.p, S.d_run_items.p, c->d_scalars + 6, st), "run packing"))
             return false;
         if (!hc(hipEventRecord(c->bev[k][0], st), "event record")) return false;
         if (nord) {
@@ -405,7 +423,8 @@
                 pending.set = -1;
             }
             if (!hc(launch_match_mfma(0, S.d_segs.p, c->d_scalars + 5, (uint32_t)std::min<size_t>(b.seg_cap, 0xFFFFFFFFu),
-                                      c->d_scalars + 1, S.d_accmask.p, c->d_accept, st, job, c->d_scalars + 7), "forward scan"))
+                                      c->d_scalars + 1, S.d_accmask.p, c->d_accept, st, job, c->d_scalars + 7,
+                                      b.run > 1 ? S.d_run_items.p : nullptr, (uint32_t)b.run, c->d_scalars + 6), "forward scan"))
                 return false;
             if (done_set >= 0 && !hc(hipEventRecord(c->bev[done_set][4], st), "event record")) return false;
         }
@@ -655,6 +674,7 @@
     out->device_ms = total_ms;
     out->match_kernel_ms = kernel_ms;
     out->match_kernel_launches = kernel_launches;
+    out->scan_run = scan_run_max;
     out->cross_kernel_ms = cross_ms;
     out->_priv = priv;
     c->last_hook_ms = t_hook;
diff --git a/pycolmap_amd/csrc/match_mfma.hip b/pycolmap_amd/csrc/match_mfma.hip
--- a/pycolmap_amd/csrc/match_mfma.hip
+++ b/pycolmap_amd/csrc/match_mfma.hip
@@ -18,6 +18,7 @@
 constexpr int kWGPerCU = 2;
 constexpr int kXT = kSegRows / 16;
 constexpr int kKeyShift = 7, kKeyCarried = 127;
+constexpr uint32_t kRunSameX = 0x80000000u, kRunNone = 0xFFFFFFFFu;
 
 constexpr int kNB = 4;
 constexpr int kOffRs = 0;
@@ -48,8 +49,8 @@
 };
 
 #ifdef AMC_SCAN_STAMPS
-constexpr int kStampMaxWG = 1024;
-__device__ uint32_t g_scan_stamps[2 * kStampMaxWG * kSegsPerItem * 8];
+constexpr int kStampMaxWG = 1024, kStampDwords = 12;
+__device__ uint32_t g_scan_stamps[2 * kStampMaxWG * kSegsPerItem * kStampDwords];
 #define AMC_STAMP() ((uint32_t)__builtin_amdgcn_s_memtime())
 #endif
 
@@ -68,9 +69,10 @@
 
 template <int MODE>
 __global__ __launch_bounds__(64 * kW) __attribute__((amdgpu_waves_per_eu(kWGPerCU, kWGPerCU)))
-void match_mfma_kernel(const SegDesc* __restrict__ segs, const uint32_t* __restrict__ nitems_p,
+void match_mfma_kernel(const SegDesc* __restrict__ segs, const uint32_t* __restrict__ nruns_p,
                        uint32_t* __restrict__ queue_head, uint32_t* __restrict__ accmask,
-                       const ScanAccept* __restrict__ accept, CopyJob job, uint32_t* __restrict__ copy_head) {
+                       const ScanAccept* __restrict__ accept, CopyJob job, uint32_t* __restrict__ copy_head,
+                       const uint32_t* __restrict__ run_items, int run_len) {
     static_assert(kChunkBytes / 1024 == kW * kYS, "a chunk splits into 1 KiB DMA pieces, one per wave and step");
     static_assert(kBN * 4 == 512, "a chunk's rs128 block is half a wave's DMA");
     __shared__ __attribute__((aligned(16))) char smem[kLdsBytes];
@@ -91,12 +93,28 @@
                           job.n16 * (part + 1) / job.parts, tid, 64 * kW);
         }
     }
-    const uint32_t nitems = *nitems_p;
+    const uint32_t nruns = *nruns_p;
     const ScanAccept sa = *accept;
 
-    auto load_desc = [&](uint32_t q) -> int {
+    auto load_run = [&](uint32_t r) -> uint32_t {
+        uint32_t v = kRunNone;
+        if (r < nruns) {
+            if (run_items) {
+                if (lane < run_len) v = run_items[(size_t)r * run_len + lane];
+            } else if (lane == 0) {
+                v = r;
+            }
+        }
+        return v;
+    };
+    auto next_entry = [&](uint32_t rv, int after) -> int {
+        const unsigned long long m = __ballot(rv != kRunNone) & (~0ull << (after + 1));
+        return m ? __builtin_ctzll(m) : -1;
+    };
+    auto load_desc = [&](uint32_t e) -> int {
         int v = 0;
-        if (q < nitems && lane < 16) v = reinterpret_cast<const int*>(segs + (size_t)q * kSegsPerItem + wid)[lane];
+        if (e != kRunNone && lane < 16)
+            v = reinterpret_cast<const int*>(segs + (size_t)(e & ~kRunSameX) * kSegsPerItem + wid)[lane];
         return v;
     };
     auto dword = [&](int dv, int f) -> int { return __builtin_amdgcn_readlane(dv, f); };
@@ -188,28 +206,47 @@
             btile[xt] = -1;
         }
     };
+    auto reset_x = [&]() __attribute__((always_inline)) {
+#pragma unroll
+        for (int xt = 0; xt < kXT; ++xt) {
+            best[xt] = ((-xterm[xt]) << kKeyShift) | kKeyCarried;
+            sec[xt] = best[xt];
+            btile[xt] = -1;
+        }
+    };
 
 #ifdef AMC_SCAN_STAMPS
-    uint32_t st_a = 0, st_first = 0, st_end = 0, st_sum[5] = {0, 0, 0, 0, 0};
-    bool st_prev = false, st_prev_active = false;
-    uint32_t* const st_slot = g_scan_stamps + ((size_t)(MODE * kStampMaxWG + min((int)blockIdx.x, kStampMaxWG - 1)) * kW + wid) * 8;
+    uint32_t st_a = 0, st_first = 0, st_end = 0, st_sum[5] = {0, 0, 0, 0, 0}, st_kept[2] = {0, 0};
+    bool st_prev = false, st_prev_active = false, st_keep_x = false;
+    uint32_t* const st_slot = g_scan_stamps + ((size_t)(MODE * kStampMaxWG + min((int)blockIdx.x, kStampMaxWG - 1)) * kW + wid) * kStampDwords;
 #endif
+    const bool table = MODE == 0 && run_items != nullptr;
+    uint32_t rv = kRunNone, rvn, rvn2 = kRunNone;
     if (tid == 0) *s_q = atomicAdd(queue_head, 1u);
     __syncthreads();
-    uint32_t q = *s_q;
-    int dv = load_desc(q);
-    if (q < nitems) {
+    rvn = load_run(*s_q);
+    if (table) {
+        __syncthreads();
+        if (tid == 0) *s_q = atomicAdd(queue_head, 1u);
+        __syncthreads();
+        rvn2 = load_run(*s_q);
+    }
+    int kpos = next_entry(rvn, -1);
+    uint32_t e = kpos >= 0 ? (uint32_t)__builtin_amdgcn_readlane((int)rvn, kpos) : kRunNone;
+    bool first = true;
+    int dv = load_desc(e);
+    if (e != kRunNone) {
         stage_head(dv);
         if (dword(dv, kDCnt) > 0) load_x(dv);
     }
     __syncthreads();
 
-    while (q < nitems) {
+    while (e != kRunNone) {
         const char* yprep = dptr(dv, kDYprep);
         const char* yrs = dptr(dv, kDYrs);
         const int nchunks = (dword(dv, kDYrows) + kBN - 1) / kBN;
         const bool active = dword(dv, kDCnt) > 0;
-        if (tid == 0) *s_q = atomicAdd(queue_head, 1u);
+        if (first && tid == 0) *s_q = atomicAdd(queue_head, 1u);
 
         i32x4 acc[2][2];
         auto insert = [&](int xt, int code) __attribute__((always_inline)) {
@@ -266,8 +303,21 @@
         YFrag y0, y1;
         asm volatile("s_waitcnt vmcnt(0)" ::: "memory");
         __syncthreads();
-        const uint32_t qn = *s_q;
-        const int dvn = load_desc(qn);
+        if (first) {
+            rv = rvn;
+            if (table) {
+                rvn = rvn2;
+                rvn2 = load_run(*s_q);
+            } else {
+                rvn = load_run(*s_q);
+            }
+        }
+        int kn = next_entry(rv, kpos);
+        const bool same_run = kn >= 0;
+        if (!same_run) kn = next_entry(rvn, -1);
+        const uint32_t en = kn < 0 ? kRunNone : (uint32_t)__builtin_amdgcn_readlane((int)(same_run ? rv : rvn), kn);
+        const bool keep_x = MODE == 0 && same_run && (en & kRunSameX) != 0;
+        const int dvn = load_desc(en);
 #ifdef AMC_SCAN_STAMPS
         {
             const uint32_t now = AMC_STAMP();
@@ -277,9 +327,15 @@
                 st_sum[2] += now - st_first;
                 st_sum[3] += 1;
                 st_sum[4] += st_prev_active ? 1 : 0;
+                if (st_keep_x) {
+                    st_kept[0] += now - st_end;
+                    st_kept[1] += 1;
+                }
                 if (lane == 0) {
 #pragma unroll
                     for (int k = 0; k < 5; ++k) st_slot[k] = st_sum[k];
+                    st_slot[8] = st_kept[0];
+                    st_slot[9] = st_kept[1];
                 }
             }
             st_a = 0;
@@ -390,9 +446,12 @@
             asm volatile("v_mov_b32 %0, %1" : "=v"(et[xt]) : "v"(btile[xt]));
             ex[xt] = xterm[xt];
         }
-        if (qn < nitems) {
+        if (en != kRunNone) {
             stage_head(dvn);
-            if (dword(dvn, kDCnt) > 0) load_x(dvn);
+            if (dword(dvn, kDCnt) > 0) {
+                if (keep_x) reset_x();
+                else load_x(dvn);
+            }
         }
         if (active) {
             const int cnt = dword(dv, kDCnt);
@@ -437,13 +496,18 @@
             }
         }
 #ifdef AMC_SCAN_STAMPS
-        if (qn >= nitems && lane == 0) {
+        if (en == kRunNone && lane == 0) {
             st_slot[5] = st_a;
             st_slot[6] = AMC_STAMP() - st_first;
             st_slot[7] = 1;
         }
 #endif
-        q = qn;
+#ifdef AMC_SCAN_STAMPS
+        st_keep_x = keep_x;
+#endif
+        e = en;
+        kpos = kn;
+        first = !same_run;
         dv = dvn;
     }
 }
@@ -602,9 +666,111 @@
     return hipGetLastError();
 }
 
+constexpr uint32_t kRunTailBlocks = 8;
+__device__ __forceinline__ bool run_block_is_single(uint32_t b, uint32_t nblocks) {
+    return nblocks >= kRunTailBlocks && b + 1 == nblocks;
+}
+__global__ __launch_bounds__(1024) void run_scan_kernel(const uint32_t* __restrict__ grp_segs, uint32_t ngroups, uint32_t R,
+                                                        uint32_t* __restrict__ run_base, uint32_t* __restrict__ nruns_out) {
+    __shared__ uint32_t wsum[16];
+    const uint32_t tid = threadIdx.x, lane = tid & 63, wid = tid >> 6;
+    const uint32_t nblocks = (ngroups + R - 1) / R;
+    uint32_t running = 0;
+    for (uint32_t base = 0; base < nblocks; base += 1024) {
+        const uint32_t b = base + tid;
+        uint32_t s = 0;
+        if (b < nblocks)
+            for (uint32_t g = b * R; g < min(b * R + R, ngroups); ++g) {
+                const uint32_t n = (grp_segs[g] + kSegsPerItem - 1) / kSegsPerItem;
+                s = run_block_is_single(b, nblocks) ? s + n : max(s, n);
+            }
+        uint32_t inc = s;
+#pragma unroll
+        for (int m = 1; m < 64; m <<= 1) {
+            const uint32_t o = __shfl_up(inc, m);
+            if (lane >= (uint32_t)m) inc += o;
+        }
+        if (lane == 63) wsum[wid] = inc;
+        __syncthreads();
+        uint32_t wbase = 0, total = 0;
+        for (uint32_t k = 0; k < 16; ++k) {
+            if (k < wid) wbase += wsum[k];
+            total += wsum[k];
+        }
+        if (b < nblocks) run_base[b] = running + wbase + inc - s;
+        running += total;
+        __syncthreads();
+    }
+    if (tid == 0) *nruns_out = running;
+}
+
+__device__ __forceinline__ bool items_share_x(const SegDesc* __restrict__ a, const SegDesc* __restrict__ b) {
+    bool same = true;
+    for (int w = 0; w < kSegsPerItem; ++w)
+        same = same && a[w].xprep == b[w].xprep && a[w].xrs == b[w].xrs && a[w].cnt == b[w].cnt && a[w].list == nullptr &&
+               b[w].list == nullptr;
+    return same;
+}
+
+constexpr uint32_t kRunMax = 8;
+__global__ __launch_bounds__(256) void run_fill_kernel(const SegDesc* __restrict__ segs, const uint32_t* __restrict__ grp_segs,
+                                                       const uint32_t* __restrict__ grp_item_base, uint32_t ngroups,
+                                                       uint32_t R, const uint32_t* __restrict__ run_base,
+                                                       uint32_t* __restrict__ run_items) {
+    __shared__ uint32_t s_items[kRunMax], s_base[kRunMax];
+    const uint32_t b = blockIdx.x, tid = threadIdx.x;
+    if (tid < R) {
+        const uint32_t g = b * R + tid;
+        s_items[tid] = g < ngroups ? (grp_segs[g] + kSegsPerItem - 1) / kSegsPerItem : 0u;
+        s_base[tid] = g < ngroups ? grp_item_base[g] : 0u;
+    }
+    __syncthreads();
+    uint32_t m = 0;
+    for (uint32_t p = 0; p < R; ++p) m = max(m, s_items[p]);
+    uint32_t* out = run_items + (size_t)run_base[b] * R;
+    if (run_block_is_single(b, gridDim.x)) {
+        uint32_t total = 0;
+        for (uint32_t p = 0; p < R; ++p) total += s_items[p];
+        for (uint32_t idx = blockIdx.y * 256 + tid; idx < total * R; idx += 256 * gridDim.y) {
+            uint32_t t = idx / R, p = 0;
+            const uint32_t pos = idx - t * R;
+            while (t >= s_items[p]) t -= s_items[p++];
+            out[idx] = pos == 0 ? s_base[p] + t : kRunNone;
+        }
+        return;
+    }
+    for (uint32_t idx = blockIdx.y * 256 + tid; idx < m * R; idx += 256 * gridDim.y) {
+        const uint32_t t = idx / R, p = idx - t * R;
+        uint32_t entry = kRunNone;
+        if (t < s_items[p]) {
+            entry = s_base[p] + t;
+            int pp = (int)p - 1;
+            while (pp >= 0 && t >= s_items[pp]) --pp;
+            if (pp >= 0 && items_share_x(segs + (size_t)entry * kSegsPerItem, segs + (size_t)(s_base[pp] + t) * kSegsPerItem))
+                entry |= kRunSameX;
+        }
+        out[idx] = entry;
+    }
+}
+
+hipError_t launch_build_runs(const SegDesc* segs, const uint32_t* grp_segs, const uint32_t* grp_item_base, uint32_t ngroups,
+                             uint32_t R, uint32_t* run_base, uint32_t* run_items, uint32_t* nruns_dev, hipStream_t s) {
+    if (R < 2 || R > kRunMax) return hipErrorInvalidValue;
+    if (ngroups == 0) return memset_async(nruns_dev, 0, sizeof(uint32_t), s);
+    const uint32_t nblocks = (ngroups + R - 1) / R;
+    hipLaunchKernelGGL(run_scan_kernel, dim3(1), dim3(1024), 0, s, grp_segs, ngroups, R, run_base, nruns_dev);
+    hipLaunchKernelGGL(run_fill_kernel, dim3(nblocks, kFillY), dim3(256), 0, s, segs, grp_segs, grp_item_base, ngroups, R,
+                       run_base, run_items);
+    return hipGetLastError();
+}
+
 hipError_t launch_match_mfma(int mode, const SegDesc* segs, const uint32_t* nitems_dev, uint32_t max_items,
                              uint32_t* queue_head, uint32_t* accmask, const ScanAccept* accept_dev, hipStream_t s,
-                             const CopyJob& job_in, uint32_t* copy_head) {
+                             const CopyJob& job_in, uint32_t* copy_head, const uint32_t* run_items, uint32_t run_len,
+                             const uint32_t* nruns_dev) {
+    if (run_items && (mode != 0 || run_len < 2 || run_len > kRunMax || !nruns_dev)) return hipErrorInvalidValue;
+    const uint32_t* const ntickets = run_items ? nruns_dev : nitems_dev;
+    const int rl = run_items ? (int)run_len : 1;
     if (max_items == 0) return hipSuccess;
     CopyJob job = (mode == 0 && copy_head) ? job_in : CopyJob();
     hipError_t e = job.parts ? memset_async(copy_head, 0, sizeof(uint32_t), s) : hipSuccess;
@@ -630,11 +796,11 @@
     if (job.parts > grid) job.parts = grid;
     if ((e = memset_async(queue_head, 0, sizeof(uint32_t), s)) != hipSuccess) return e;
     if (mode == 0)
-        hipLaunchKernelGGL((match_mfma_kernel<0>), dim3(grid), dim3(64 * kW), 0, s, segs, nitems_dev, queue_head,
-                           accmask, accept_dev, job, copy_head);
+        hipLaunchKernelGGL((match_mfma_kernel<0>), dim3(grid), dim3(64 * kW), 0, s, segs, ntickets, queue_head,
+                           accmask, accept_dev, job, copy_head, run_items, rl);
     else
-        hipLaunchKernelGGL((match_mfma_kernel<1>), dim3(grid), dim3(64 * kW), 0, s, segs, nitems_dev, queue_head,
-                           accmask, accept_dev, job, copy_head);
+        hipLaunchKernelGGL((match_mfma_kernel<1>), dim3(grid), dim3(64 * kW), 0, s, segs, ntickets, queue_head,
+                           accmask, accept_dev, job, copy_head, run_items, rl);
     return hipGetLastError();
 }
 
diff --git a/pycolmap_amd/csrc/scan_run.h b/pycolmap_amd/csrc/scan_run.h
--- /dev/null
+++ b/pycolmap_amd/csrc/scan_run.h
@@ -0,0 +1,31 @@
+#pragma once
+#include <cstddef>
+#include <cstdint>
+
+namespace amc {
+
+constexpr int kScanRunAuto = 4;
+constexpr size_t kScanRunMinPerWorkgroup = 64;
+
+template <class Slot1At>
+inline int choose_scan_run_by(Slot1At slot1_at, const uint32_t* grp, size_t ngrp, size_t items, size_t workgroups,
+                              int forced) {
+    if (forced == 1 || forced == 2 || forced == 4 || forced == 8) return forced;
+    if (ngrp < 2 || items < kScanRunMinPerWorkgroup * kScanRunAuto * workgroups) return 1;
+    const size_t cuts = ngrp - 1, allowed = cuts / 4;
+    size_t bad = 0;
+    for (size_t g = 0; g + 1 < ngrp; ++g) {
+        const size_t a = grp[g], b = grp[g + 1], e = grp[g + 2];
+        const size_t n = b - a < e - b ? b - a : e - b;
+        size_t k = 0;
+        while (k < n && slot1_at(a + k) == slot1_at(b + k)) ++k;
+        if ((k < n || n == 0) && ++bad > allowed) return 1;
+    }
+    return kScanRunAuto;
+}
+inline int choose_scan_run(const uint32_t* slot1, const uint32_t* grp, size_t ngrp, size_t items, size_t workgroups,
+                           int forced) {
+    return choose_scan_run_by([slot1](size_t q) { return slot1[q]; }, grp, ngrp, items, workgroups, forced);
+}
+
+}
```

Result: faster. 13800 billion distances/s, median of 6 (+1.3%).
